# celliern/triflow

Measured on AMD Instinct MI355X. Metric: implicit time-steps/s, 1e6-node 3-var system (member-steps/s over all GPUs), higher is better.
Workload: dtype f64; 1 GPU; BASELINE config 3: M3_film, N=1000000 nodes, periodic, fixed dt=0.001, ROS2; members_per_gpu=1, parallelism=ensemble members sharded by rank, no data-path collective

## Files before the change

### include/triflow_hip.h

```cpp
#ifndef TRIFLOW_HIP_H
#define TRIFLOW_HIP_H

#include <stddef.h>
#include <stdint.h>

#ifdef __cplusplus
extern "C" {
#endif

typedef struct tf_model tf_model;
typedef struct tf_solver tf_solver;

typedef struct tf_model_spec {
    int32_t nvar;
    int32_t nh;
    int32_t npar;
    int32_t mp;
    int32_t nnz;
    int32_t seg;
    int32_t sweep_block;
    int32_t uses_x;
    uint32_t parvec_mask;
} tf_model_spec;

typedef struct tf_solver_opts {
    int32_t m1;
    int32_t m_upper;
    int32_t nstate;
    int32_t refine;
    int32_t device;
    int32_t berr_every;
    int32_t reserved;
} tf_solver_opts;

const char* tf_last_error(void);
int tf_runtime_info(int32_t* is_device_build, int32_t* device_count);
int tf_set_device(int32_t ordinal);

int tf_model_create(const tf_model_spec* spec, const void* code_object, size_t code_size,
                    tf_model** out);
int tf_model_add_alternate(tf_model* model, const void* code_object, size_t code_size,
                           uint64_t kernel_mask);
void tf_model_destroy(tf_model* model);

int tf_solver_create(tf_model* model, int64_t N, int32_t nsys, int32_t periodic,
                     const tf_solver_opts* opts, tf_solver** out);
void tf_solver_destroy(tf_solver* solver);
int tf_solver_describe(tf_solver* solver, int32_t* nlevels, int32_t* chunks ,
                       int32_t max_levels, int64_t* device_bytes);

int tf_set_state(tf_solver*, int32_t slot, int32_t first_var, int32_t nvars, const double* host);
int tf_get_state(tf_solver*, int32_t slot, int32_t first_var, int32_t nvars, double* host);
int tf_set_state_flat(tf_solver*, int32_t slot, const double* uflat );
int tf_get_state_flat(tf_solver*, int32_t slot, double* uflat);
int tf_copy_state(tf_solver*, int32_t src_slot, int32_t dst_slot);
int tf_set_helpers(tf_solver*, int32_t first, int32_t count, const double* host);
int tf_set_param_scalar(tf_solver*, int32_t k, const double* values );
int tf_set_param_vector(tf_solver*, int32_t k, const double* host );
int tf_set_dx(tf_solver*, const double* dx );
int tf_set_x(tf_solver*, const double* x );
int tf_set_dirichlet(tf_solver*, int32_t n, const int32_t* var, const int64_t* node,
                     const double* value);

int tf_set_dirichlet_values(tf_solver*, const double* before, const double* after);
int tf_poke(tf_solver*, int32_t slot, int32_t n, const int32_t* var, const int64_t* node,
            const double* value);
int tf_peek(tf_solver*, int32_t slot, int32_t n, const int32_t* var, const int64_t* node,
            double* out);

int tf_eval(tf_solver*, int32_t slot, int32_t with_j);
int tf_eval_repeat(tf_solver*, int32_t slot, int32_t with_j, int32_t reps, double* total_ms);
int tf_get_F(tf_solver*, double* F );
int tf_get_J(tf_solver*, double* Jvals );

int tf_set_csc_map(tf_solver*, const int32_t* map, int64_t n);
int tf_get_J_mapped(tf_solver*, double* out );

int tf_set_constant_jacobian(tf_solver*, int32_t on);

int tf_factor(tf_solver*, double c);
int tf_solve(tf_solver*, const double* rhs_flat , double* x_flat);
int tf_matvec(tf_solver*, const double* v_flat, double* y_flat);

int tf_step_theta(tf_solver*, int32_t src, int32_t dst, double dt, double theta);
int tf_step_row(tf_solver*, int32_t src, int32_t dst, double dt, int32_t s,
                const double* alpha, const double* gamma, const double* b,
                const double* b_pred, int32_t hook_after, double* err_out);
int tf_step_bdf2(tf_solver*, int32_t src, int32_t dst, double dt);
int tf_bdf2_reset(tf_solver*);
int tf_step_bdf2_owned(tf_solver*, int32_t src, int32_t dst, double dt, int64_t owner,
                       int32_t continuing);
int tf_bdf2_release(tf_solver*, int64_t owner);
int tf_step_bdf2_from(tf_solver*, int32_t src, int32_t dst, int32_t prev, double dt);
int tf_step_row_queued(tf_solver*, int32_t src, int32_t dst, double dt, int32_t stages,
                       const double* alpha, const double* gamma, const double* b,
                       const double* b_pred, int32_t hook_after, int32_t err_slot);
int tf_read_err(tf_solver*, int32_t err_slot, double* err_out);
enum { TF_SCHEME_THETA = 0, TF_SCHEME_ROW = 1 };
typedef struct tf_scheme {
    int32_t kind;
    int32_t stages;
    double theta;
    const double* alpha;
    const double* gamma;
    const double* b;
    int32_t hook_after;
    int32_t reserved;
} tf_scheme;
int tf_step_doubling(tf_solver*, int32_t src, int32_t dst, int32_t tmp, int32_t coarse, double dt,
                     int32_t m, int32_t nfine, const tf_scheme* scheme, int32_t ord, double* err_out);
int tf_diff_norm(tf_solver*, int32_t slot_a, int32_t slot_b, int32_t ord, double* out);

int tf_backward_error(tf_solver*, double* omega, int32_t* refined);

int tf_monitor_error(tf_solver*, double* worst);
int tf_solver_counters(tf_solver*, int64_t* factorisations, int64_t* checks, int64_t* replans);
int tf_solver_kernel_block(tf_solver*, int32_t kernel, int32_t* block);
int tf_sync(tf_solver*);

int tf_timing_enable(tf_solver*, int64_t mask);
int tf_timing_reset(tf_solver*);
int tf_timing_get(tf_solver*, int32_t kernel, double* total_ms, int64_t* launches);
int tf_debug_stamps(tf_solver*, uint64_t* out, int32_t max_levels);
int tf_kernel_count(void);
const char* tf_kernel_name(int32_t kernel);

typedef struct tf_probe tf_probe;
int tf_probe_create(tf_solver*, const void* code_object, size_t code_size, int32_t nprobe,
                    const int32_t* kinds, int32_t nconst, int32_t capacity, tf_probe** out);
void tf_probe_destroy(tf_probe* probe);
int tf_probe_set_consts(tf_probe*, const double* values , int32_t nconst);
int tf_probe_set_x(tf_probe*, const double* x );
int tf_probe_record(tf_probe*, int32_t slot);
int tf_probe_fetch(tf_probe*, double* out, int64_t max_rows, int64_t* rows);
int tf_probe_pending(tf_probe*, int64_t* rows);

typedef struct tf_record tf_record;
int tf_record_create(tf_solver*, const void* code_object, size_t code_size, int32_t nrec,
                     const int32_t* geometry, int32_t nconst, tf_record** out);
void tf_record_destroy(tf_record* record);
int tf_record_set_consts(tf_record*, const double* values , int32_t nconst);
int tf_record_set_x(tf_record*, const double* x );
int tf_record_record(tf_record*, int32_t which, int32_t slot);
int tf_record_fetch(tf_record*, int32_t which, double* out, int64_t max_rows, int64_t* rows);
int tf_record_pending(tf_record*, int32_t which, int64_t* rows);

#ifdef __cplusplus
}
#endif
#endif
```

### triflow_amd/_capi.py

```python

import ctypes as C
import os

import numpy as np

c_double_p = C.POINTER(C.c_double)
c_int32_p = C.POINTER(C.c_int32)
c_int64_p = C.POINTER(C.c_int64)


class ModelSpec(C.Structure):
    _fields_ = [("nvar", C.c_int32), ("nh", C.c_int32), ("npar", C.c_int32),
                ("mp", C.c_int32), ("nnz", C.c_int32), ("seg", C.c_int32),
                ("sweep_block", C.c_int32), ("uses_x", C.c_int32),
                ("parvec_mask", C.c_uint32)]


class SolverOpts(C.Structure):
    _fields_ = [("m1", C.c_int32), ("m_upper", C.c_int32), ("nstate", C.c_int32),
                ("refine", C.c_int32), ("device", C.c_int32), ("berr_every", C.c_int32),
                ("reserved", C.c_int32)]


class Scheme(C.Structure):
    _fields_ = [("kind", C.c_int32), ("stages", C.c_int32), ("theta", C.c_double),
                ("alpha", c_double_p), ("gamma", c_double_p), ("b", c_double_p),
                ("hook_after", C.c_int32), ("reserved", C.c_int32)]


SIGNATURES = {
    "tf_last_error": (C.c_char_p, []),
    "tf_runtime_info": (C.c_int, [c_int32_p, c_int32_p]),
    "tf_set_device": (C.c_int, [C.c_int32]),
    "tf_model_create": (C.c_int, [C.POINTER(ModelSpec), C.c_void_p, C.c_size_t,
                                  C.POINTER(C.c_void_p)]),
    "tf_model_add_alternate": (C.c_int, [C.c_void_p, C.c_void_p, C.c_size_t, C.c_uint64]),
    "tf_model_destroy": (None, [C.c_void_p]),
    "tf_solver_create": (C.c_int, [C.c_void_p, C.c_int64, C.c_int32, C.c_int32,
                                   C.POINTER(SolverOpts), C.POINTER(C.c_void_p)]),
    "tf_solver_destroy": (None, [C.c_void_p]),
    "tf_solver_describe": (C.c_int, [C.c_void_p, c_int32_p, c_int32_p, C.c_int32, c_int64_p]),
    "tf_set_state": (C.c_int, [C.c_void_p, C.c_int32, C.c_int32, C.c_int32, c_double_p]),
    "tf_get_state": (C.c_int, [C.c_void_p, C.c_int32, C.c_int32, C.c_int32, c_double_p]),
    "tf_set_state_flat": (C.c_int, [C.c_void_p, C.c_int32, c_double_p]),
    "tf_get_state_flat": (C.c_int, [C.c_void_p, C.c_int32, c_double_p]),
    "tf_copy_state": (C.c_int, [C.c_void_p, C.c_int32, C.c_int32]),
    "tf_set_helpers": (C.c_int, [C.c_void_p, C.c_int32, C.c_int32, c_double_p]),
    "tf_set_param_scalar": (C.c_int, [C.c_void_p, C.c_int32, c_double_p]),
    "tf_set_param_vector": (C.c_int, [C.c_void_p, C.c_int32, c_double_p]),
    "tf_set_dx": (C.c_int, [C.c_void_p, c_double_p]),
    "tf_set_x": (C.c_int, [C.c_void_p, c_double_p]),
    "tf_set_dirichlet": (C.c_int, [C.c_void_p, C.c_int32, c_int32_p, c_int64_p, c_double_p]),
    "tf_set_dirichlet_values": (C.c_int, [C.c_void_p, c_double_p, c_double_p]),
    "tf_poke": (C.c_int, [C.c_void_p, C.c_int32, C.c_int32, c_int32_p, c_int64_p, c_double_p]),
    "tf_peek": (C.c_int, [C.c_void_p, C.c_int32, C.c_int32, c_int32_p, c_int64_p, c_double_p]),
    "tf_eval": (C.c_int, [C.c_void_p, C.c_int32, C.c_int32]),
    "tf_eval_repeat": (C.c_int, [C.c_void_p, C.c_int32, C.c_int32, C.c_int32, c_double_p]),
    "tf_get_F": (C.c_int, [C.c_void_p, c_double_p]),
    "tf_get_J": (C.c_int, [C.c_void_p, c_double_p]),
    "tf_set_csc_map": (C.c_int, [C.c_void_p, c_int32_p, C.c_int64]),
    "tf_set_constant_jacobian": (C.c_int, [C.c_void_p, C.c_int32]),
    "tf_get_J_mapped": (C.c_int, [C.c_void_p, c_double_p]),
    "tf_factor": (C.c_int, [C.c_void_p, C.c_double]),
    "tf_solve": (C.c_int, [C.c_void_p, c_double_p, c_double_p]),
    "tf_matvec": (C.c_int, [C.c_void_p, c_double_p, c_double_p]),
    "tf_step_theta": (C.c_int, [C.c_void_p, C.c_int32, C.c_int32, C.c_double, C.c_double]),
    "tf_step_row": (C.c_int, [C.c_void_p, C.c_int32, C.c_int32, C.c_double, C.c_int32,
                              c_double_p, c_double_p, c_double_p, c_double_p, C.c_int32,
                              c_double_p]),
    "tf_step_row_queued": (C.c_int, [C.c_void_p, C.c_int32, C.c_int32, C.c_double, C.c_int32,
                                     c_double_p, c_double_p, c_double_p, c_double_p, C.c_int32, C.c_int32]),
    "tf_read_err": (C.c_int, [C.c_void_p, C.c_int32, c_double_p]),
    "tf_step_bdf2": (C.c_int, [C.c_void_p, C.c_int32, C.c_int32, C.c_double]),
    "tf_bdf2_reset": (C.c_int, [C.c_void_p]),
    "tf_step_bdf2_from": (C.c_int, [C.c_void_p, C.c_int32, C.c_int32, C.c_int32, C.c_double]),
    "tf_step_bdf2_owned": (C.c_int, [C.c_void_p, C.c_int32, C.c_int32, C.c_double, C.c_int64,
                                     C.c_int32]),
    "tf_bdf2_release": (C.c_int, [C.c_void_p, C.c_int64]),
    "tf_diff_norm": (C.c_int, [C.c_void_p, C.c_int32, C.c_int32, C.c_int32, c_double_p]),
    "tf_step_doubling": (C.c_int, [C.c_void_p, C.c_int32, C.c_int32, C.c_int32, C.c_int32, C.c_double,
                                   C.c_int32, C.c_int32, C.POINTER(Scheme), C.c_int32, c_double_p]),
    "tf_backward_error": (C.c_int, [C.c_void_p, c_double_p, c_int32_p]),
    "tf_monitor_error": (C.c_int, [C.c_void_p, c_double_p]),
    "tf_solver_counters": (C.c_int, [C.c_void_p, c_int64_p, c_int64_p, c_int64_p]),
    "tf_sync": (C.c_int, [C.c_void_p]),
    "tf_timing_enable": (C.c_int, [C.c_void_p, C.c_int64]),
    "tf_timing_reset": (C.c_int, [C.c_void_p]),
    "tf_timing_get": (C.c_int, [C.c_void_p, C.c_int32, c_double_p, c_int64_p]),
    "tf_debug_stamps": (C.c_int, [C.c_void_p, C.POINTER(C.c_uint64), C.c_int32]),
    "tf_solver_kernel_block": (C.c_int, [C.c_void_p, C.c_int32, C.POINTER(C.c_int32)]),
    "tf_kernel_count": (C.c_int, []),
    "tf_kernel_name": (C.c_char_p, [C.c_int32]),
    "tf_probe_create": (C.c_int, [C.c_void_p, C.c_void_p, C.c_size_t, C.c_int32, c_int32_p, C.c_int32,
                                  C.c_int32, C.POINTER(C.c_void_p)]),
    "tf_probe_destroy": (None, [C.c_void_p]),
    "tf_probe_set_consts": (C.c_int, [C.c_void_p, c_double_p, C.c_int32]),
    "tf_probe_set_x": (C.c_int, [C.c_void_p, c_double_p]),
    "tf_probe_record": (C.c_int, [C.c_void_p, C.c_int32]),
    "tf_probe_fetch": (C.c_int, [C.c_void_p, c_double_p, C.c_int64, c_int64_p]),
    "tf_probe_pending": (C.c_int, [C.c_void_p, c_int64_p]),
    "tf_record_create": (C.c_int, [C.c_void_p, C.c_void_p, C.c_size_t, C.c_int32, c_int32_p, C.c_int32,
                                   C.POINTER(C.c_void_p)]),
    "tf_record_destroy": (None, [C.c_void_p]),
    "tf_record_set_consts": (C.c_int, [C.c_void_p, c_double_p, C.c_int32]),
    "tf_record_set_x": (C.c_int, [C.c_void_p, c_double_p]),
    "tf_record_record": (C.c_int, [C.c_void_p, C.c_int32, C.c_int32]),
    "tf_record_fetch": (C.c_int, [C.c_void_p, C.c_int32, c_double_p, C.c_int64, c_int64_p]),
    "tf_record_pending": (C.c_int, [C.c_void_p, C.c_int32, c_int64_p]),
}


def _dptr(arr):
    return arr.ctypes.data_as(c_double_p)


def _f64(a, shape=None):
    out = np.ascontiguousarray(a, dtype=np.float64)
    if shape is not None and out.shape != tuple(shape):
        raise ValueError("expected array of shape %r, got %r" % (tuple(shape), out.shape))
    return out


class Library:

    def __init__(self, path):
        if not os.path.exists(path):
            raise RuntimeError(
                "HIP runtime library %s is missing -- build it with "
                "`python -c 'import __graft_entry__ as g; g.build()'` "
                "(there is no CPU fallback)" % path)
        self.path = path
        self.dll = C.CDLL(path)
        for name, (restype, argtypes) in SIGNATURES.items():
            fn = getattr(self.dll, name)
            fn.restype = restype
            fn.argtypes = argtypes

    def call(self, name, *args):
        rc = getattr(self.dll, name)(*args)
        if rc != 0:
            raise RuntimeError("%s: %s" % (name, self.dll.tf_last_error().decode()))

    def runtime_info(self):
        dev, cnt = C.c_int32(0), C.c_int32(0)
        self.call("tf_runtime_info", C.byref(dev), C.byref(cnt))
        return bool(dev.value), cnt.value

    def set_device(self, ordinal):
        self.call("tf_set_device", int(ordinal))

    def kernel_names(self):
        return [self.dll.tf_kernel_name(k).decode() for k in range(self.dll.tf_kernel_count())]


class DeviceModel:

    def __init__(self, lib, spec, code, alt_code=None, alt_kernels=()):
        self.lib = lib
        self.spec = dict(spec)
        cs = ModelSpec(spec["nvar"], spec["nh"], spec["npar"], spec["mp"], spec["nnz"],
                       spec["seg"], spec["sweep_block"], spec["uses_x"], spec["parvec_mask"])
        self._code = C.create_string_buffer(code, len(code)) if code else None
        handle = C.c_void_p()
        lib.call("tf_model_create", C.byref(cs),
                 C.cast(self._code, C.c_void_p) if self._code is not None else None,
                 len(code) if code else 0, C.byref(handle))
        self.handle = handle
        self._alt = None
        if alt_code and alt_kernels:
            names = lib.kernel_names()
            mask = 0
            for k in alt_kernels:
                mask |= 1 << names.index(k)
            self._alt = C.create_string_buffer(alt_code, len(alt_code))
            lib.call("tf_model_add_alternate", handle, C.cast(self._alt, C.c_void_p), len(alt_code), mask)

    def close(self):
        if self.handle:
            self.lib.dll.tf_model_destroy(self.handle)
            self.handle = None

    def __del__(self):
        try:
            self.close()
        except Exception:
            pass


class DeviceSolver:

    def __init__(self, model, N, nsys=1, periodic=False, m1=0, m_upper=0, nstate=0,
                 refine=-1, device=-1, berr_every=0):
        self.model = model
        self.lib = model.lib
        self.N, self.nsys, self.periodic = int(N), int(nsys), bool(periodic)
        self.nvar, self.nh = model.spec["nvar"], model.spec["nh"]
        self.npar, self.nnz = model.spec["npar"], model.spec["nnz"]
        m1 = m1 or int(os.environ.get("TRIFLOW_M1", "0"))
        m_upper = m_upper or int(os.environ.get("TRIFLOW_M_UPPER", "0"))
        opts = SolverOpts(m1, m_upper, nstate, refine, device, berr_every, 0)
        handle = C.c_void_p()
        self.lib.call("tf_solver_create", model.handle, self.N, self.nsys,
                      int(self.periodic), C.byref(opts), C.byref(handle))
        self.handle = handle
        self.nstate = nstate if nstate > 0 else 3
        ju = model.spec.get("j_uniform") or []
        self.constant_jacobian = bool(ju) and all(ju) and os.environ.get("TRIFLOW_REUSE_FACTOR", "1") != "0"
        if self.constant_jacobian:
            self.lib.call("tf_set_constant_jacobian", self.handle, 1)

    def close(self):
        if self.handle:
            self.lib.dll.tf_solver_destroy(self.handle)
            self.handle = None

    def __del__(self):
        try:
            self.close()
        except Exception:
            pass

    def describe(self):
        nl, nbytes = C.c_int32(0), C.c_int64(0)
        chunks = (C.c_int32 * 32)()
        self.lib.call("tf_solver_describe", self.handle, C.byref(nl), chunks, 32, C.byref(nbytes))
        return dict(levels=nl.value, chunks=list(chunks[:nl.value]), device_bytes=nbytes.value)

    def set_state(self, slot, arrays, first=0):
        a = _f64(arrays).reshape(-1, self.nsys, self.N)
        self.lib.call("tf_set_state", self.handle, slot, first, a.shape[0], _dptr(a))

    def get_state(self, slot, first=0, nvars=None):
        nvars = self.nvar - first if nvars is None else nvars
        out = np.empty((nvars, self.nsys, self.N))
        self.lib.call("tf_get_state", self.handle, slot, first, nvars, _dptr(out))
        return out

    def set_state_flat(self, slot, uflat):
        a = _f64(uflat).reshape(self.nsys, self.N * self.nvar)
        self.lib.call("tf_set_state_flat", self.handle, slot, _dptr(a))

    def get_state_flat(self, slot):
        out = np.empty((self.nsys, self.N * self.nvar))
        self.lib.call("tf_get_state_flat", self.handle, slot, _dptr(out))
        return out

    def copy_state(self, src, dst):
        self.lib.call("tf_copy_state", self.handle, src, dst)

    def set_helpers(self, arrays, first=0):
        a = _f64(arrays).reshape(-1, self.nsys, self.N)
        self.lib.call("tf_set_helpers", self.handle, first, a.shape[0], _dptr(a))

    def set_param(self, k, value):
        if (self.model.spec["parvec_mask"] >> k) & 1:
            a = _f64(np.broadcast_to(np.asarray(value, dtype=float), (self.nsys, self.N)))
            self.lib.call("tf_set_param_vector", self.handle, k, _dptr(a))
        else:
            a = _f64(np.broadcast_to(np.asarray(value, dtype=float), (self.nsys,)))
            self.lib.call("tf_set_param_scalar", self.handle, k, _dptr(a))

    def set_dx(self, dx):
        a = _f64(np.broadcast_to(np.asarray(dx, dtype=float), (self.nsys,)))
        self.lib.call("tf_set_dx", self.handle, _dptr(a))

    def set_x(self, x):
        a = _f64(np.broadcast_to(np.asarray(x, dtype=float), (self.nsys, self.N)))
        self.lib.call("tf_set_x", self.handle, _dptr(a))

    def set_dirichlet(self, entries):
        entries = list(entries)
        n = len(entries)
        var = np.array([e[0] for e in entries], dtype=np.int32)
        node = np.array([e[1] for e in entries], dtype=np.int64)
        val = np.array([e[2] for e in entries], dtype=np.float64)
        self.lib.call("tf_set_dirichlet", self.handle, n,
                      var.ctypes.data_as(c_int32_p), node.ctypes.data_as(c_int64_p), _dptr(val))

    def poke(self, slot, entries):
        entries = list(entries)
        if not entries:
            return
        var = np.array([e[0] for e in entries], dtype=np.int32)
        node = np.array([e[1] for e in entries], dtype=np.int64)
        val = np.array([e[2] for e in entries], dtype=np.float64)
        self.lib.call("tf_poke", self.handle, slot, len(entries),
                      var.ctypes.data_as(c_int32_p), node.ctypes.data_as(c_int64_p), _dptr(val))

    def peek(self, slot, var, node):
        v = np.array([var], dtype=np.int32)
        n = np.array([node], dtype=np.int64)
        out = np.empty((1, self.nsys))
        self.lib.call("tf_peek", self.handle, slot, 1, v.ctypes.data_as(c_int32_p),
                      n.ctypes.data_as(c_int64_p), _dptr(out))
        return out[0]

    def set_dirichlet_values(self, before=None, after=None):
        b = _f64(before) if before is not None else None
        a = _f64(after) if after is not None else None
        self.lib.call("tf_set_dirichlet_values", self.handle,
                      _dptr(b) if b is not None else None, _dptr(a) if a is not None else None)

    def eval(self, slot=0, with_j=False):
        self.lib.call("tf_eval", self.handle, slot, int(with_j))

    def eval_repeat(self, slot=0, with_j=True, reps=20):
        ms = C.c_double(0.0)
        self.lib.call("tf_eval_repeat", self.handle, slot, int(with_j), reps, C.byref(ms))
        return ms.value / reps

    def get_F(self):
        out = np.empty((self.nsys, self.N * self.nvar))
        self.lib.call("tf_get_F", self.handle, _dptr(out))
        return out

    def get_J(self):
        out = np.empty((self.nsys, self.N, max(self.nnz, 1)))
        self.lib.call("tf_get_J", self.handle, _dptr(out))
        return out[:, :, :self.nnz]

    def set_csc_map(self, index_list):
        m = np.ascontiguousarray(index_list, dtype=np.int32)
        self.lib.call("tf_set_csc_map", self.handle, m.ctypes.data_as(c_int32_p), m.size)
        self._csc_n = m.size

    def get_J_mapped(self):
        out = np.empty(self._csc_n)
        self.lib.call("tf_get_J_mapped", self.handle, _dptr(out))
        return out

    def factor(self, c):
        self.lib.call("tf_factor", self.handle, float(c))

    def solve(self, rhs_flat):
        rhs = _f64(rhs_flat).reshape(self.nsys, self.N * self.nvar)
        out = np.empty_like(rhs)
        self.lib.call("tf_solve", self.handle, _dptr(rhs), _dptr(out))
        return out

    def matvec(self, v_flat):
        v = _f64(v_flat).reshape(self.nsys, self.N * self.nvar)
        out = np.empty_like(v)
        self.lib.call("tf_matvec", self.handle, _dptr(v), _dptr(out))
        return out

    def step_theta(self, src, dst, dt, theta=1.0):
        self.lib.call("tf_step_theta", self.handle, src, dst, float(dt), float(theta))

    def step_row(self, src, dst, dt, alpha, gamma, b, b_pred=None, hook_after=False,
                 want_err=True):
        alpha, gamma = _f64(alpha), _f64(gamma)
        b = _f64(b)
        s = b.size
        bp = _f64(b_pred) if b_pred is not None else None
        err = C.c_double(0.0)
        self.lib.call("tf_step_row", self.handle, src, dst, float(dt), s, _dptr(alpha),
                      _dptr(gamma), _dptr(b), _dptr(bp) if bp is not None else None,
                      int(hook_after), C.byref(err) if want_err else None)
        return np.float64(err.value) if (want_err and bp is not None) else None

    def step_row_queued(self, src, dst, dt, alpha, gamma, b, b_pred, hook_after=False, err_slot=1):
        alpha, gamma, b, bp = _f64(alpha), _f64(gamma), _f64(b), _f64(b_pred)
        self.lib.call("tf_step_row_queued", self.handle, src, dst, float(dt), b.size, _dptr(alpha),
                      _dptr(gamma), _dptr(b), _dptr(bp), int(hook_after), int(err_slot))

    def read_err(self, err_slot):
        err = C.c_double(0.0)
        self.lib.call("tf_read_err", self.handle, int(err_slot), C.byref(err))
        return np.float64(err.value)

    def step_bdf2(self, src, dst, dt, owner=0, continuing=True):
        if owner:
            self.lib.call("tf_step_bdf2_owned", self.handle, src, dst, float(dt), int(owner),
                          int(bool(continuing)))
        else:
            self.lib.call("tf_step_bdf2", self.handle, src, dst, float(dt))

    def step_bdf2_from(self, src, dst, prev, dt):
        self.lib.call("tf_step_bdf2_from", self.handle, src, dst, int(prev), float(dt))

    def bdf2_release(self, owner):
        if self.handle:
            self.lib.call("tf_bdf2_release", self.handle, int(owner))

    def bdf2_reset(self):
        self.lib.call("tf_bdf2_reset", self.handle)

    def step_doubling(self, src, dst, tmp, coarse, dt, m, desc, ord=2, nfine=10):
        keep = []
        if desc["kind"] == "theta":
            sch = Scheme(0, 0, float(desc["theta"]), None, None, None, 0, 0)
        else:
            arrs = [_f64(desc[k]) for k in ("alpha", "gamma", "b")]
            keep.extend(arrs)
            sch = Scheme(1, arrs[2].size, 0.0, _dptr(arrs[0]), _dptr(arrs[1]), _dptr(arrs[2]),
                         int(bool(desc.get("hook_after", True))), 0)
        err = np.empty(self.nsys)
        self.lib.call("tf_step_doubling", self.handle, src, dst, tmp, coarse, float(dt), int(m),
                      int(nfine), C.byref(sch), 0 if ord in (0, np.inf, "inf") else int(ord), _dptr(err))
        return err

    def diff_norms(self, slot_a, slot_b, ord=2):
        out = np.empty((self.nsys, self.nvar))
        self.lib.call("tf_diff_norm", self.handle, slot_a, slot_b,
                      0 if ord in (0, np.inf, "inf") else int(ord), _dptr(out))
        return out

    def backward_error(self):
        om, flag = C.c_double(0.0), C.c_int32(0)
        self.lib.call("tf_backward_error", self.handle, C.byref(om), C.byref(flag))
        return om.value, bool(flag.value)

    def counters(self):
        f, c, r = C.c_int64(0), C.c_int64(0), C.c_int64(0)
        self.lib.call("tf_solver_counters", self.handle, C.byref(f), C.byref(c), C.byref(r))
        return dict(factorisations=f.value, checks=c.value, replans=r.value)

    def kernel_block(self, name):
        b = C.c_int32(0)
        self.lib.call("tf_solver_kernel_block", self.handle, self.lib.kernel_names().index(name), C.byref(b))
        return b.value

    def monitor_error(self):
        w = C.c_double(0.0)
        self.lib.call("tf_monitor_error", self.handle, C.byref(w))
        return w.value

    def sync(self):
        self.lib.call("tf_sync", self.handle)
        if not getattr(self, "_warned_replan", False) and self.counters()["replans"]:
            import warnings
            self._warned_replan = True
            warnings.warn("banded solver: the default partition lost accuracy on this matrix and the "
                          "factorisations go through the rescue plan (8 x longer chunks, every solve "
                          "checked): several times slower; see DESIGN.md section 4.5", RuntimeWarning,
                          stacklevel=2)

    def debug_stamps(self, levels=8):
        out = np.zeros((levels, 64), dtype=np.uint64)
        self.lib.call("tf_debug_stamps", self.handle, out.ctypes.data_as(C.POINTER(C.c_uint64)), levels)
        return out

    def timing(self, on=True, kernels=None):
        if kernels is not None:
            names = self.lib.kernel_names()
            mask = 0
            for k in kernels:
                mask |= 1 << names.index(k)
        else:
            mask = -1 if on else 0
        self.lib.call("tf_timing_enable", self.handle, mask)

    def timing_reset(self):
        self.lib.call("tf_timing_reset", self.handle)

    def timing_report(self):
        out = {}
        for k, name in enumerate(self.lib.kernel_names()):
            ms, n = C.c_double(0.0), C.c_int64(0)
            self.lib.call("tf_timing_get", self.handle, k, C.byref(ms), C.byref(n))
            if n.value:
                out[name] = (ms.value, n.value)
        return out


class DeviceProbe:

    def __init__(self, solver, code, kinds, nconst, capacity=1024):
        self.solver, self.lib = solver, solver.lib
        self.nprobe, self.nconst, self.capacity = len(kinds), int(nconst), int(capacity)
        self._code = C.create_string_buffer(code, len(code))
        k = np.ascontiguousarray(kinds, dtype=np.int32)
        handle = C.c_void_p()
        self.lib.call("tf_probe_create", solver.handle, C.cast(self._code, C.c_void_p), len(code),
                      self.nprobe, k.ctypes.data_as(c_int32_p), self.nconst, self.capacity, C.byref(handle))
        self.handle = handle

    def close(self):
        if self.handle:
            self.lib.dll.tf_probe_destroy(self.handle)
            self.handle = None

    def __del__(self):
        try:
            self.close()
        except Exception:
            pass

    def _check_open(self):
        if not self.solver.handle:
            raise RuntimeError("the solver of this probe set was closed (rows not fetched before are lost)")

    def set_consts(self, values):
        self._check_open()
        v = _f64(values).reshape(self.solver.nsys, self.nconst)
        self.lib.call("tf_probe_set_consts", self.handle, _dptr(v) if v.size else None, self.nconst)

    def set_x(self, x):
        self._check_open()
        a = _f64(np.broadcast_to(np.asarray(x, dtype=float), (self.solver.nsys, self.solver.N)))
        self.lib.call("tf_probe_set_x", self.handle, _dptr(a))

    def record(self, slot):
        self._check_open()
        self.lib.call("tf_probe_record", self.handle, int(slot))

    def pending(self):
        self._check_open()
        n = C.c_int64(0)
        self.lib.call("tf_probe_pending", self.handle, C.byref(n))
        return n.value

    def fetch(self):
        n = self.pending()
        out = np.empty((n, self.solver.nsys, self.nprobe))
        got = C.c_int64(0)
        self.lib.call("tf_probe_fetch", self.handle, _dptr(out), n, C.byref(got))
        return out[:got.value]


class DeviceRecord:

    def __init__(self, solver, code, geometry, nconst):
        self.solver, self.lib = solver, solver.lib
        self.nconst = int(nconst)
        g = np.ascontiguousarray(geometry, dtype=np.int32).reshape(-1, 6)
        self.ncols = [-(-(int(r[3]) - int(r[2])) // int(r[4])) for r in g]
        self._code = C.create_string_buffer(code, len(code))
        handle = C.c_void_p()
# ... 46 lines not shown
```

### triflow_amd/csrc/tf_args.h

```cpp
#pragma once
#include <stdint.h>

#define TF_MAX_FIELDS 16
#define TF_MAX_PARS 16
#define TF_MAX_TERMS 8

struct TfLayout {
    int nsys;
    int N;
    int P;
    int mbase;
    int rem;
    int M;
    int Ptot;
    int periodic;
    int64_t plane;
};

struct TfSweepArgs {
    TfLayout L;
    const double* fields;
    const double* helpers;
    const double* parvec;
    const double* parsca;
    const double* dx;
    const double* xcoord;
    double* F;
    double* Jv;
    int with_j;
    int nterms;
    const double* kx[TF_MAX_TERMS];
    double kc[TF_MAX_TERMS];
    double fscale;
    double* theta_rhs;
    double theta, theta_dt;
    double* bdf_rhs;
    const double* bdf_prev;
    double* bdf_prev_out;
    double bdf_c0, bdf_c1;
    int bdf_two_step;
    double* stage_rhs;
    double gc[TF_MAX_TERMS];
    double cF, cA;
};

struct TfSpmvArgs {
    TfLayout L;
    const double* parsca;
    const double* dx;
    const double* Jv;
    const double* v;
    double* y;
    double scale;
    int absval;
    int nterms;
    const double* vx[TF_MAX_TERMS];
    double vc[TF_MAX_TERMS];
    const double* addF;
    double cF, cA;
};

struct TfNormArgs {
    TfLayout L;
    const double* a;
    const double* b;
    double* partial;
    int nblocks;
    int ord;
    const int* status;
    const double* mon;
};

struct TfBerrArgs {
    TfLayout L;
    const double* parsca;
    const double* dx;
    const double* Jv;
    const double* x;
    const double* rhs;
    double c;
    double* red;
    int one_node;
    int reserved_;
    const double* xbase;
};

struct TfStageMonArgs { TfSweepArgs s; TfBerrArgs b; };

struct TfVecArgs {
    int64_t n;
    int nterms;
    int op;
    double* out;
    const double* base;
    const double* x[TF_MAX_TERMS];
    double c[TF_MAX_TERMS];
    double* red;
    double c2[TF_MAX_TERMS];
};

struct TfPermArgs {
    TfLayout L;
    const double* src;
    double* dst;
    int ncomp;
    int mode;
};

struct TfGatherArgs {
    TfLayout L;
    const double* Jv;
    const int* map;
    double* out;
    int64_t n;
    int nnz;
};

struct TfDirichletArgs {
    TfLayout L;
    double* fields;
    int n;
    const int* var;
    const int* node;
    const double* value;
};

#define TF_POKE_MAX 8
struct TfPokeArgs {
    TfLayout L;
    double* fields;
    int n;
    int var[TF_POKE_MAX];
    int node[TF_POKE_MAX];
    double value[TF_POKE_MAX];
};

struct TfLevelArgs {
    TfLayout L;
    const double* Jv;
    const double* parsca;
    const double* dx;
    double c;
    const double* Ablk;
    const double* rhs;
    double* x;
    double* Ut;
    double* Et;
    double* yt;
    double* Dinv;
    double* Unup;
    double* tips_dn;
    double* tips_up;
    TfLayout Lnext;
    double* Anext;
    double* rhsnext;
    const double* xnext;
    int* status;
    int lu_cols;
    int next_aos;
    int cr_rhs;
    double* crf;
    double* zt;
    unsigned* perm;
    int fold_top;
    int respike;
    int twist;
    int ylds_rows;
    int fuse_asm;
    double* upd_out;
    const double* upd_base;
    const double* upd_k0;
    double upd_c0, upd_c1;
    int upd_n;
    double* topAinv;
    double* topx;
    unsigned long long* stamps;
};

struct TfTinyArgs {
    TfLayout L;
    const double* Jv;
    const double* parsca;
    const double* dx;
    double c;
    double* lu;
    int* piv;
    const double* rhs;
    double* x;
    int* status;
};

struct TfTailArgs {
    TfLevelArgs lv[2];
};

struct TfScalarArgs {
    TfLevelArgs lv[3];
    unsigned* counter;
};

struct TfTopArgs {
    int nsys;
    const double* A;
    const double* rhs;
    double* Ainv;
    double* x;
    int* status;
    int aos;
};

#define TF_RESPIKE_MODEL(mp, nvar) ((mp) * (nvar) * (nvar) >= 8)
#define TF_RESPIKE_MIN_NODES 750000
#define TF_TWIST_MAX_CHUNKS 65536

#ifndef TF_L1_SPLIT_LDS
#define TF_L1_SPLIT_LDS (40 * 1024)
#endif
#define TF_L1_SPLIT_MODEL(mp, nvar) ((nvar) >= 2 && 2 * (1 + (mp)) * (nvar) * (nvar) * 64 * 8 <= TF_L1_SPLIT_LDS)

#define TF_STAGE_SEG 8

#define TF_CR_MAXLEN 16
#define TF_CRS_MAXLEN 256
#define TF_CRS_TOPLEN(b) ((b) == 1 ? 512 : 256)

#define TF_PROBE_SUM 0
#define TF_PROBE_MEAN 1
#define TF_PROBE_INTEGRAL 2
#define TF_PROBE_MAX 3
#define TF_PROBE_MIN 4
#define TF_PROBE_ARGMAX 5
#define TF_PROBE_ARGMIN 6
#define TF_PROBE_KINDS 7
#define TF_PROBE_SEG 8
struct TfProbeArgs {
    TfLayout L;
    const double* fields;
    const double* helpers;
    const double* parvec;
    const double* parsca;
    const double* dx;
    const double* xcoord;
    const double* hc;
    double* partial;
    double* ends;
    int nblk;
    int nseg;
    int capacity;
    int* cursor;
    double* ring;
};

#define TF_REC_SAMPLE 0
#define TF_REC_MAX 1
#define TF_REC_MIN 2
#define TF_REC_MEAN 3
#define TF_REC_BLOCK 256
struct TfRecordArgs {
    TfLayout L;
    const double* fields;
    const double* helpers;
    const double* parvec;
    const double* parsca;
    const double* dx;
    const double* xcoord;
    const double* hc;
    int which;
    int pool;
    int start, stop, step;
    int ncols;
    int split;
    int part;
    int nblk;
    int capacity;
    int* cursor;
    double* ring;
};

enum TfKernel {
    TFK_SWEEP_F = 0, TFK_SWEEP_FJ, TFK_SPMV, TFK_VEC, TFK_VEC_MAXABS, TFK_PERM, TFK_DIRICHLET,
    TFK_L1_FACTOR, TFK_L1_SOLVE, TFK_L1_ASM_MAT, TFK_L1_ASM_RHS, TFK_L1_BACKSUB,
    TFK_BT_LU, TFK_BT_SPIKE, TFK_BT_RHS, TFK_BT_ASM_MAT, TFK_BT_ASM_RHS, TFK_BT_BACKSUB,
    TFK_TOP_FACTOR, TFK_TOP_SOLVE, TFK_BERR, TFK_DIFFNORM, TFK_L1_FACTOR_RHS, TFK_SWEEP_F_STAGE,
    TFK_CR_FACTOR, TFK_CR_FWD, TFK_CR_BWD, TFK_POKE, TFK_SWEEP_FJ_THETA, TFK_SWEEP_FJ_BDF2, TFK_GATHER,
    TFK_SWEEP_F_STAGE_RHS, TFK_L1_FWD2, TFK_L1_BACKSUB_U, TFK_CR_TAIL, TFK_L1_FWD2_BACKSUB, TFK_TINY_FACTOR, TFK_TINY_SOLVE,
    TFK_S_FWD, TFK_S_BWD, TFK_SWEEP_F_STAGE_RHS_N, TFK_L1_SOLVE_CR, TFK_L1_FWD2_BACKSUB_CR, TFK_SWEEP_F_STAGE_RHS_MON,
    TFK_PROBE_PARTIAL, TFK_PROBE_FINAL,
    TFK_RECORD, TFK_COUNT
};
#define TF_KERNEL_NAMES { \
    "tfk_sweep_f", "tfk_sweep_fj", "tfk_spmv", "tfk_vec", "tfk_vec_maxabs", "tfk_perm", "tfk_dirichlet", \
    "tfk_l1_factor", "tfk_l1_solve", "tfk_l1_asm_mat", "tfk_l1_asm_rhs", "tfk_l1_backsub", \
    "tfk_bt_lu", "tfk_bt_spike", "tfk_bt_rhs", "tfk_bt_asm_mat", "tfk_bt_asm_rhs", "tfk_bt_backsub", \
    "tfk_top_factor", "tfk_top_solve", "tfk_berr", "tfk_diffnorm", "tfk_l1_factor_rhs", "tfk_sweep_f_stage", \
    "tfk_cr_factor", "tfk_cr_fwd", "tfk_cr_bwd", "tfk_poke", "tfk_sweep_fj_theta", "tfk_sweep_fj_bdf2", \
    "tfk_gather", "tfk_sweep_f_stage_rhs", "tfk_l1_fwd2", "tfk_l1_backsub_u", "tfk_cr_tail", \
    "tfk_l1_fwd2_backsub", "tfk_tiny_factor", "tfk_tiny_solve", "tfk_s_fwd", "tfk_s_bwd", "tfk_sweep_f_stage_rhs_n", \
    "tfk_l1_solve_cr", "tfk_l1_fwd2_backsub_cr", "tfk_sweep_f_stage_rhs_mon", \
    "tfk_probe_partial", "tfk_probe_final" }
#define TF_KERNEL_NAMES_RECORD { "tfk_record" }
static inline const char* tf_kernel_entry(int kernel) {
    static const char* const base[] = TF_KERNEL_NAMES;
    static const char* const rec[] = TF_KERNEL_NAMES_RECORD;
    static_assert(sizeof(base) / sizeof(base[0]) == TFK_RECORD, "TF_KERNEL_NAMES and TfKernel differ");
    static_assert(sizeof(rec) / sizeof(rec[0]) == TFK_COUNT - TFK_RECORD, "TF_KERNEL_NAMES_RECORD and TfKernel differ");
    if (kernel < 0 || kernel >= TFK_COUNT) return "";
    return kernel < TFK_RECORD ? base[kernel] : rec[kernel - TFK_RECORD];
}
```

### triflow_amd/csrc/tf_backend_hip.cpp

```cpp
#include "tf_backend.h"
#include "tf_args.h"

#include <hip/hip_runtime.h>
#include <hip/hip_ext.h>

#include <algorithm>
#include <cstdio>
#include <cstdlib>
#include <cstring>
#include <map>
#include <thread>
#include <stdexcept>
#include <string>

namespace tfb {

static void check(hipError_t err, const char* what) {
    if (err != hipSuccess)
        throw std::runtime_error(std::string("HIP error in ") + what + ": " + hipGetErrorString(err));
}
#define TF_HIP(call) check((call), #call)

struct Module { hipModule_t mod; hipFunction_t fn[TFK_COUNT]; hipModule_t alt = nullptr; };
struct Stream { hipStream_t s; };
struct Event { hipEvent_t e; };

bool is_device_build() { return true; }
int coop_group(int b) { return b <= 2 ? 1 : (b <= 8 ? 8 : (b <= 16 ? 16 : 1)); }

bool cyclic_reduction(int b) {
    const char* mode = getenv("TRIFLOW_REDUCED");
    if (mode && std::string(mode) == "walk") return false;
    return b >= 1 && b <= 8;
}

int device_count() {
    int n = 0;
    if (hipGetDeviceCount(&n) != hipSuccess) return 0;
    return n;
}

void set_device(int ordinal) { TF_HIP(hipSetDevice(ordinal)); }

void* dev_alloc(size_t bytes) {
    void* p = nullptr;
    if (bytes == 0) bytes = 8;
    TF_HIP(hipMalloc(&p, bytes));
    TF_HIP(hipMemset(p, 0, bytes));
    TF_HIP(hipDeviceSynchronize());
    return p;
}
void dev_free(void* p) { if (p) (void)hipFree(p); }
void memset0(void* p, size_t bytes, Stream* s) { TF_HIP(hipMemsetAsync(p, 0, bytes, s->s)); }
namespace {
constexpr size_t kStageChunk = 8u << 20;
constexpr size_t kStageMin = 4u << 20;
struct Bounce {
    void* buf[2] = {nullptr, nullptr};
    hipEvent_t ev[2];
    bool ok = false;
    Bounce() {
        if (hipHostMalloc(&buf[0], kStageChunk, hipHostMallocDefault) != hipSuccess) return;
        if (hipHostMalloc(&buf[1], kStageChunk, hipHostMallocDefault) != hipSuccess) return;
        if (hipEventCreateWithFlags(&ev[0], hipEventDisableTiming) != hipSuccess) return;
        if (hipEventCreateWithFlags(&ev[1], hipEventDisableTiming) != hipSuccess) return;
        ok = true;
    }
};
struct BounceSet {
    std::map<int, Bounce*> by_device;
    ~BounceSet() {
        for (auto& kv : by_device) {
            Bounce* b = kv.second;
            if (b->ok) { (void)hipEventDestroy(b->ev[0]); (void)hipEventDestroy(b->ev[1]); }
            if (b->buf[0]) (void)hipHostFree(b->buf[0]);
            if (b->buf[1]) (void)hipHostFree(b->buf[1]);
            delete b;
        }
    }
};
Bounce& bounce() {
    static thread_local BounceSet set;
    int dev = 0;
    (void)hipGetDevice(&dev);
    Bounce*& b = set.by_device[dev];
    if (!b) b = new Bounce();
    return *b;
}
void parallel_copy(void* dst, const void* src, size_t n) {
    constexpr int NT = 4;
    if (n < (1u << 20)) { std::memcpy(dst, src, n); return; }
    std::thread th[NT - 1];
    const size_t part = (n / NT + 63) & ~(size_t)63;
    for (int t = 1; t < NT; ++t) {
        const size_t lo = std::min(n, part * t), hi = std::min(n, part * (t + 1));
        th[t - 1] = std::thread([=] { if (hi > lo) std::memcpy((char*)dst + lo, (const char*)src + lo, hi - lo); });
    }
    std::memcpy(dst, src, std::min(n, part));
    for (int t = 1; t < NT; ++t) th[t - 1].join();
}
}
void h2d(void* dst, const void* src, size_t bytes, Stream* s) {
    Bounce& b = bounce();
    if (bytes < kStageMin || !b.ok) {
        TF_HIP(hipMemcpyAsync(dst, src, bytes, hipMemcpyHostToDevice, s->s));
        TF_HIP(hipStreamSynchronize(s->s));
        return;
    }
    size_t off = 0;
    for (int k = 0; off < bytes; ++k) {
        const int i = k & 1;
        const size_t n = std::min(kStageChunk, bytes - off);
        if (k >= 2) TF_HIP(hipEventSynchronize(b.ev[i]));
        parallel_copy(b.buf[i], (const char*)src + off, n);
        TF_HIP(hipMemcpyAsync((char*)dst + off, b.buf[i], n, hipMemcpyHostToDevice, s->s));
        TF_HIP(hipEventRecord(b.ev[i], s->s));
        off += n;
    }
    TF_HIP(hipStreamSynchronize(s->s));
}
void d2h(void* dst, const void* src, size_t bytes, Stream* s) {
    Bounce& b = bounce();
    if (bytes < kStageMin || !b.ok) {
        TF_HIP(hipMemcpyAsync(dst, src, bytes, hipMemcpyDeviceToHost, s->s));
        TF_HIP(hipStreamSynchronize(s->s));
        return;
    }
    size_t off = 0, done = 0;
    int k = 0;
    for (; off < bytes; ++k) {
        const int i = k & 1;
        const size_t n = std::min(kStageChunk, bytes - off);
        if (k >= 2) {
            TF_HIP(hipEventSynchronize(b.ev[i]));
            const size_t m = std::min(kStageChunk, bytes - done);
            parallel_copy((char*)dst + done, b.buf[i], m);
            done += m;
        }
        TF_HIP(hipMemcpyAsync(b.buf[i], (const char*)src + off, n, hipMemcpyDeviceToHost, s->s));
        TF_HIP(hipEventRecord(b.ev[i], s->s));
        off += n;
    }
    for (int j = (k >= 2 ? k - 2 : 0); j < k; ++j) {
        const int i = j & 1;
        TF_HIP(hipEventSynchronize(b.ev[i]));
        const size_t m = std::min(kStageChunk, bytes - done);
        parallel_copy((char*)dst + done, b.buf[i], m);
        done += m;
    }
}
void d2d(void* dst, const void* src, size_t bytes, Stream* s) {
    TF_HIP(hipMemcpyAsync(dst, src, bytes, hipMemcpyDeviceToDevice, s->s));
}

Module* module_load(const void* image, size_t) {
    Module* m = new Module();
    hipError_t err = hipModuleLoadData(&m->mod, image);
    if (err != hipSuccess) {
        delete m;
        check(err, "hipModuleLoadData (is the code object built for this GPU, gfx950?)");
    }
    for (int k = 0; k < TFK_COUNT; ++k) {
        err = hipModuleGetFunction(&m->fn[k], m->mod, tf_kernel_entry(k));
        if (err != hipSuccess) {
            (void)hipModuleUnload(m->mod);
            delete m;
            throw std::runtime_error(std::string("kernel missing from code object: ") + tf_kernel_entry(k));
        }
    }
    if (const char* alt = getenv("TF_ALT_HSACO")) {
        const char* mask_s = getenv("TF_ALT_MASK");
        unsigned long mask = mask_s ? strtoul(mask_s, nullptr, 0) : 0;
        FILE* f = fopen(alt, "rb");
        if (f && mask) {
            fseek(f, 0, SEEK_END); long n = ftell(f); fseek(f, 0, SEEK_SET);
            std::string img(n, '\0');
            if (fread(&img[0], 1, n, f) == (size_t)n) {
                hipModule_t am;
                if (hipModuleLoadData(&am, img.data()) == hipSuccess)
                    for (int k = 0; k < TFK_COUNT; ++k)
                        if ((mask >> k) & 1ul) (void)hipModuleGetFunction(&m->fn[k], am, tf_kernel_entry(k));
            }
        }
        if (f) fclose(f);
    }
    return m;
}
void module_add_alternate(Module* m, const void* image, size_t, uint64_t mask) {
    if (!m || !mask) return;
    if (m->alt) throw std::runtime_error("module_add_alternate: one alternate build per model");
    check(hipModuleLoadData(&m->alt, image), "hipModuleLoadData (alternate build)");
    for (int k = 0; k < TFK_COUNT; ++k)
        if ((mask >> k) & 1ull) {
            if (hipModuleGetFunction(&m->fn[k], m->alt, tf_kernel_entry(k)) != hipSuccess)
                throw std::runtime_error(std::string("kernel missing from the alternate code object: ") + tf_kernel_entry(k));
        }
}
void module_unload(Module* m) {
    if (!m) return;
    if (m->alt) (void)hipModuleUnload(m->alt);
    (void)hipModuleUnload(m->mod);
    delete m;
}

Stream* stream_create() {
    Stream* s = new Stream();
    TF_HIP(hipStreamCreateWithFlags(&s->s, hipStreamNonBlocking));
    return s;
}
void stream_destroy(Stream* s) { if (s) { (void)hipStreamDestroy(s->s); delete s; } }
void stream_sync(Stream* s) { TF_HIP(hipStreamSynchronize(s->s)); }

unsigned kernel_block(Module* m, int kernel) {
    int v = 0;
    TF_HIP(hipFuncGetAttribute(&v, HIP_FUNC_ATTRIBUTE_MAX_THREADS_PER_BLOCK, m->fn[kernel]));
    return (unsigned)v;
}

void launch(Module* m, int kernel, unsigned gx, unsigned gy, unsigned block,
            const void* args, size_t arg_bytes, Stream* s, unsigned lds_bytes) {
    size_t size = arg_bytes;
    void* config[] = {HIP_LAUNCH_PARAM_BUFFER_POINTER, const_cast<void*>(args),
                      HIP_LAUNCH_PARAM_BUFFER_SIZE, &size, HIP_LAUNCH_PARAM_END};
    TF_HIP(hipModuleLaunchKernel(m->fn[kernel], gx, gy, 1, block, 1, 1, lds_bytes, s->s, nullptr, config));
}

void launch_timed(Module* m, int kernel, unsigned gx, unsigned gy, unsigned block,
                  const void* args, size_t arg_bytes, Stream* s, Event* start, Event* stop,
                  unsigned lds_bytes) {
    size_t size = arg_bytes;
    void* config[] = {HIP_LAUNCH_PARAM_BUFFER_POINTER, const_cast<void*>(args),
                      HIP_LAUNCH_PARAM_BUFFER_SIZE, &size, HIP_LAUNCH_PARAM_END};
    TF_HIP(hipExtModuleLaunchKernel(m->fn[kernel], gx * block, gy, 1, block, 1, 1, lds_bytes, s->s,
                                    nullptr, config, start->e, stop->e, 0));
}

struct Graph { hipGraph_t graph; hipGraphExec_t exec; };
bool graphs_supported() { return true; }
void capture_begin(Stream* s) { TF_HIP(hipStreamBeginCapture(s->s, hipStreamCaptureModeThreadLocal)); }
Graph* capture_end(Stream* s) {
    hipGraph_t graph = nullptr;
    TF_HIP(hipStreamEndCapture(s->s, &graph));
    hipGraphExec_t exec = nullptr;
    hipError_t err = hipGraphInstantiate(&exec, graph, nullptr, nullptr, 0);
    if (err != hipSuccess) { (void)hipGraphDestroy(graph); check(err, "hipGraphInstantiate"); }
    return new Graph{graph, exec};
}
void capture_abort(Stream* s) {
    hipGraph_t graph = nullptr;
    (void)hipStreamEndCapture(s->s, &graph);
    if (graph) (void)hipGraphDestroy(graph);
}
void graph_launch(Graph* g, Stream* s) { TF_HIP(hipGraphLaunch(g->exec, s->s)); }
void graph_destroy(Graph* g) {
    if (!g) return;
    (void)hipGraphExecDestroy(g->exec);
    (void)hipGraphDestroy(g->graph);
    delete g;
}

struct Mailbox { char* host = nullptr; hipEvent_t ev; };
Mailbox* mailbox_create() {
    Mailbox* m = new Mailbox();
    TF_HIP(hipHostMalloc((void**)&m->host, 64, hipHostMallocDefault));
    std::memset(m->host, 0, 64);
    TF_HIP(hipEventCreateWithFlags(&m->ev, hipEventDisableTiming));
    return m;
}
void mailbox_destroy(Mailbox* m) {
    if (!m) return;
    (void)hipEventDestroy(m->ev);
    (void)hipHostFree(m->host);
    delete m;
}
void mailbox_post(Mailbox* m, int at, const void* dev_src, size_t bytes, Stream* s) {
    TF_HIP(hipMemcpyAsync(m->host + at, dev_src, bytes, hipMemcpyDeviceToHost, s->s));
}
void mailbox_mark(Mailbox* m, Stream* s) { TF_HIP(hipEventRecord(m->ev, s->s)); }
void mailbox_wait(Mailbox* m, void* dst, size_t bytes) {
    TF_HIP(hipEventSynchronize(m->ev));
    std::memcpy(dst, m->host, bytes);
}

Event* event_create() {
    Event* e = new Event();
    TF_HIP(hipEventCreate(&e->e));
    return e;
}
void event_destroy(Event* e) { if (e) { (void)hipEventDestroy(e->e); delete e; } }
void event_record(Event* e, Stream* s) { TF_HIP(hipEventRecord(e->e, s->s)); }
float event_elapsed_ms(Event* a, Event* b) {
    float ms = 0.f;
    TF_HIP(hipEventElapsedTime(&ms, a->e, b->e));
    return ms;
}

void* host_alloc(size_t bytes) {
    void* p = nullptr;
    TF_HIP(hipHostMalloc(&p, bytes ? bytes : 8, hipHostMallocDefault));
    return p;
}
void host_free(void* p) { if (p) (void)hipHostFree(p); }
void d2h_async(void* dst, const void* src, size_t bytes, Stream* s) {
    TF_HIP(hipMemcpyAsync(dst, src, bytes, hipMemcpyDeviceToHost, s->s));
}
void stream_wait_event(Stream* s, Event* e) { TF_HIP(hipStreamWaitEvent(s->s, e->e, 0)); }
void event_sync(Event* e) { TF_HIP(hipEventSynchronize(e->e)); }

}
```

### triflow_amd/csrc/tf_coop_hip.h

```cpp
#pragma once
#include "tf_crs.h"

template <int BB> struct TfCoop {
    static constexpr int G = BB <= 2 ? 1 : (BB <= 8 ? 8 : (BB <= 16 ? 16 : 1));
    static constexpr int NGRP = G > 1 ? 64 / G : 64;
};

template <int BB>
__device__ __forceinline__ void tfk_bt_lu_coop(const TfLevelArgs& a, int dir) {
    typedef TfTips<BB, 1> Tip;
    constexpr int G = TfCoop<BB>::G, NGRP = TfCoop<BB>::NGRP;
    const TfLayout& L = a.L;
    const int grp = threadIdx.x / G, g = threadIdx.x % G;
    const int pg = blockIdx.x * NGRP + grp;
    const bool lane_on = pg < L.Ptot && g < BB;
    const int e = lane_on ? pg / L.P : 0, p = lane_on ? pg - e * L.P : 0;
    const int len = tf_len(L, p), mI = len - 1, start = tf_start(L, p);
    const int di = dir > 0 ? 0 : 1;
    const int behind = dir > 0 ? 0 : 2, ahead = dir > 0 ? 2 : 0;

    __shared__ double sUn[NGRP][BB][BB];
    __shared__ double sAh[NGRP][BB][BB];
    __shared__ double sAll[2][NGRP][G][2 * BB + 1];
    __shared__ double sE[NGRP][BB][BB + 1];
// ... 322 lines not shown
            double sub = 0.0, dia = 0.0, sup = 0.0;
#pragma unroll
            for (int k = 0; k < BB; ++k) {
                sub = tf_fma(-H[k], tdn(Tip::V(0, 0, k, c)), sub);
                dia = tf_fma(-H[k], tdn(Tip::W(0, 0, k, c)), dia);
            }
            dia += D[c];
            if (has_next) {
#pragma unroll
                for (int k = 0; k < BB; ++k) {
                    dia = tf_fma(-K[k], tup(Tip::V(0, 0, k, c)), dia);
                    sup = tf_fma(-K[k], tup(Tip::W(0, 0, k, c)), sup);
                }
            }
            a.Anext[tf_next_A(a, e, p, s2, 0, g, c, BB)] = sub;
            a.Anext[tf_next_A(a, e, p, s2, 1, g, c, BB)] = dia;
            a.Anext[tf_next_A(a, e, p, s2, 2, g, c, BB)] = sup;
        }
    }
}

template <int BB> struct TfCr {
    static constexpr int MAXLEN = TF_CR_MAXLEN;
    static constexpr int NPOS = MAXLEN + 1;
    static constexpr int G = 8, NGRP = 8;
};

template <int BB, int G>
__device__ __forceinline__ int tf_gj_coop(double (&S)[BB], double (&INV)[BB], bool on, int g,
                                          double* xch, bool& ok) {
    constexpr int RS = 2 * BB + 1;
    int myk = -1;
#pragma unroll
    for (int c = 0; c < BB; ++c) INV[c] = c == g ? 1.0 : 0.0;
    auto publish = [&](int kk) {
        double* dst = xch + ((kk & 1) * G + g) * RS;
#pragma unroll
        for (int c = 0; c < BB; ++c) { dst[c] = S[c]; dst[BB + c] = INV[c]; }
        dst[2 * BB] = (on && myk < 0) ? tf_abs(S[kk]) : -1.0;
    };
    publish(0);
    __syncthreads();
#pragma unroll
    for (int kk = 0; kk < BB; ++kk) {
        const double* buf = xch + (kk & 1) * G * RS;
        int piv = 0;
        double best = -2.0;
#pragma unroll
        for (int r = 0; r < BB; ++r) {
            const double v = buf[r * RS + 2 * BB];
            if (v > best) { best = v; piv = r; }
        }
        const double* prow = buf + piv * RS;
        const double pv = prow[kk];
        if (on) ok = ok && (pv != 0.0) && tf_finite(pv);
        const double rp = 1.0 / pv;
        const bool mine = g == piv;
        if (mine) myk = kk;
        const double f2 = mine ? 0.0 : -S[kk] * rp;
#pragma unroll
        for (int c = 0; c < BB; ++c) {
            S[c] = tf_fma(f2, prow[c], S[c]);
            INV[c] = tf_fma(f2, prow[BB + c], INV[c]);
        }
        if (mine) {
#pragma unroll
            for (int c = 0; c < BB; ++c) { S[c] *= rp; INV[c] *= rp; }
        }
        if (kk + 1 < BB) publish(kk + 1);
        __syncthreads();
    }
    return myk;
}


template <int BB>
__device__ __forceinline__ void tf_load_row(const double* p, double (&dst)[BB]) {
    if constexpr (BB % 2 == 0) {
        const double2* q = reinterpret_cast<const double2*>(__builtin_assume_aligned(p, 16));
#pragma unroll
        for (int m = 0; m < BB / 2; ++m) {
            const double2 v = q[m];
            dst[2 * m] = v.x;
            dst[2 * m + 1] = v.y;
        }
    } else {
#pragma unroll
        for (int m = 0; m < BB; ++m) dst[m] = p[m];
    }
}

__device__ __forceinline__ void tf_wave_sync() {
    __builtin_amdgcn_fence(__ATOMIC_RELEASE, "wavefront");
    __builtin_amdgcn_wave_barrier();
    __builtin_amdgcn_fence(__ATOMIC_ACQUIRE, "wavefront");
}
template <int BB> struct TfCrSolveLds {
    static constexpr int NPOS = TF_CR_MAXLEN + 1;
    double sYr[NPOS * 2 * BB], sY[NPOS][BB], sZ[NPOS][BB];
};

template <int BB> struct TfCrIo {
    const double* ys;
    const double* crf0;
    double* next_own;
    double* next_prev;
    double* xmirror;
    bool has_mirror;
    const double* xn_own;
    const double* xn_prev;
    bool has_xprev;
    __device__ __forceinline__ TfCrIo(const TfLevelArgs& a, const TfCrChunk<BB>& ch) {
        ys = a.rhs + (ch.nbase + ch.start) * 2 * BB;
        crf0 = a.crf + (ch.nbase + ch.start) * 5 * BB * BB;
        next_own = a.rhsnext ? a.rhsnext + ((int64_t)ch.e * a.Lnext.N + ch.p) * 2 * BB : nullptr;
        next_prev = a.rhsnext ? a.rhsnext + ((int64_t)ch.e * a.Lnext.N + ch.pprev) * 2 * BB + BB : nullptr;
        xmirror = nullptr; has_mirror = false;
        xn_own = a.xnext ? a.xnext + ((int64_t)ch.e * a.Lnext.N + ch.p) * BB : nullptr;
        xn_prev = a.xnext ? a.xnext + ((int64_t)ch.e * a.Lnext.N + ch.pprev) * BB : nullptr;
        has_xprev = ch.has_prev;
    }
};

template <int BB> struct TfCrFwdRows { double Di[4][BB], Lb[4][BB], Ua[4][BB]; };
template <int BB>
__device__ __forceinline__ void tfk_cr_fwd_load(const TfCrChunk<BB>& ch, int tid, const TfCrIo<BB>& io, TfCrFwdRows<BB>& rows) {
    constexpr int G = TfCr<BB>::G, B2 = BB * BB, MAXR = 4;
    const int grp = tid / G, g = tid % G;
    const bool row_on = g < BB;
    const int mI = ch.mI;
#pragma unroll
    for (int r = 0; r < MAXR; ++r) {
        const int s = 1 << r;
        const int nA = ((mI >> r) + 1) >> 1, nB = mI >> (r + 1), nq = mI >> r;
        const bool onA = s <= mI && grp < nA && row_on;
        const bool onB = s <= mI && grp <= nB && row_on;
        const bool ends = grp == nB;
        const int aa = 2 * s * (grp + 1);
        const bool vL = onB && (ends ? (nq & 1) != 0 : true);
        const bool vR = onB && (ends ? true : aa + s <= mI);
        const int k = s * (2 * grp + 1), kL = ends ? nq * s : aa - s, kR = ends ? s : aa + s;
        const double* rk = io.crf0 + ((onA ? k : 1) - 1) * 5 * B2 + g * BB;
        const double* rl = io.crf0 + ((vL ? kL : 1) - 1) * 5 * B2 + 4 * B2 + g * BB;
        const double* rr = io.crf0 + ((vR ? kR : 1) - 1) * 5 * B2 + 3 * B2 + g * BB;
        tf_load_row<BB>(rk, rows.Di[r]);
        tf_load_row<BB>(rl, rows.Lb[r]);
        tf_load_row<BB>(rr, rows.Ua[r]);
    }
}
#define TF_CR_NYS(b) ((TF_CR_MAXLEN * 2 * (b) + 63) / 64)
template <int BB>
__device__ __forceinline__ void tfk_cr_fwd_load_ys(const TfCrChunk<BB>& ch, int tid, const TfCrIo<BB>& io, double (&ysv)[TF_CR_NYS(BB)]) {
#pragma unroll
    for (int q = 0; q < TF_CR_NYS(BB); ++q) ysv[q] = tid + 64 * q < ch.len * 2 * BB ? io.ys[tid + 64 * q] : 0.0;
}

template <int BB, bool KEEPZ = false, bool PRE = false>
__device__ __forceinline__ void tfk_cr_fwd_chunk(const TfLevelArgs& a, const TfCrChunk<BB>& ch, int tid,
                                                 TfCrSolveLds<BB>& sh, const TfCrIo<BB>& io,
                                                 double* zkeep = nullptr, const TfCrFwdRows<BB>* pre = nullptr,
                                                 const double* ysv = nullptr) {
    typedef TfCr<BB> C;
    constexpr int G = C::G, B2 = BB * BB, MAXR = 4;
    static_assert(C::MAXLEN <= 16, "round count");
    const TfLayout& L = a.L;
    const int grp = tid / G, g = tid % G;
    const bool row_on = g < BB;
    const int mI = ch.mI, pe = ch.pe, len = ch.len;
    double (&sY)[TfCrSolveLds<BB>::NPOS][BB] = sh.sY;
    double (&sZ)[TfCrSolveLds<BB>::NPOS][BB] = sh.sZ;
    double* sYr = sh.sYr;

    double* const zt0 = a.zt + (ch.nbase + ch.start - 1) * BB + (row_on ? g : 0);
    tf_wave_sync();
    TfCrFwdRows<BB> own;
    if constexpr (PRE) {
#pragma unroll
        for (int q = 0; q < TF_CR_NYS(BB); ++q)
            if (tid + 64 * q < len * 2 * BB) sYr[2 * BB + tid + 64 * q] = ysv[q];
    } else {
        for (int i = tid; i < len * 2 * BB; i += 64) sYr[2 * BB + i] = io.ys[i];
        tfk_cr_fwd_load<BB>(ch, tid, io, own);
    }
    const TfCrFwdRows<BB>& rw = PRE ? *pre : own;
    const double (&Di)[4][BB] = rw.Di;
    const double (&Lb)[4][BB] = rw.Lb;
    const double (&Ua)[4][BB] = rw.Ua;
    tf_wave_sync();
    if (PRE && (ch.p & 3) == 0) TF_STAMP(a, 42);
    for (int i = tid; i < (len + 1) * BB; i += 64) {
        const int pos = i / BB, r = i - pos * BB;
        sY[pos][r] = pos > 0 ? sYr[pos * 2 * BB + r] + sYr[pos * 2 * BB + BB + r] : 0.0;
    }
    tf_wave_sync();
#pragma unroll
    for (int r = 0; r < MAXR; ++r) {
        const int s = 1 << r;
        if (s <= mI) {
            const int nA = ((mI >> r) + 1) >> 1, nB = mI >> (r + 1), nq = mI >> r;
            if (grp < nA && row_on) {
                const int k = s * (2 * grp + 1);
                double z = 0.0;
#pragma unroll
                for (int m = 0; m < BB; ++m) z = tf_fma(Di[r][m], sY[k][m], z);
                sZ[k][g] = z;
                zt0[k * BB] = z;
                if (KEEPZ) zkeep[r] = z;
            }
            tf_wave_sync();
            if (grp <= nB && row_on) {
                const bool ends = grp == nB;
                const int aa = 2 * s * (grp + 1);
                const int aL = ends ? pe : aa, aU = ends ? 0 : aa;
                const bool vL = ends ? (nq & 1) != 0 : true;
                const bool vR = ends ? true : aa + s <= mI;
                const int kL = vL ? (ends ? nq * s : aa - s) : 1, kR = vR ? (ends ? s : aa + s) : 1;
                double yl = 0.0, yu = 0.0;
#pragma unroll
                for (int m = 0; m < BB; ++m) {
                    yl = tf_fma(-Lb[r][m], sZ[kL][m], yl);
                    yu = tf_fma(-Ua[r][m], sZ[kR][m], yu);
                }
                if (vL) sY[aL][g] += yl;
                if (vR) sY[aU][g] += yu;
            }
            tf_wave_sync();
        }
    }
    if (PRE && (ch.p & 3) == 0) TF_STAMP(a, 43);
    if (a.fold_top) {
        double x = 0.0;
        if (row_on && grp == 0) {
            const int nsys = L.Ptot;
#pragma unroll
            for (int c = 0; c < BB; ++c)
                x = tf_fma(a.topAinv[(int64_t)(g * BB + c) * nsys + ch.e], sY[pe][c] + sY[0][c], x);
        }
        tf_wave_sync();
        if (row_on && grp == 0) {
            a.topx[(int64_t)ch.e * BB + g] = x;
            a.x[(ch.nbase + ch.node(pe)) * BB + g] = x;
            if (io.has_mirror) io.xmirror[(pe - 1) * BB + g] = x;
            sY[pe][g] = x;
            sY[0][g] = ch.has_prev ? x : 0.0;
        }
        tf_wave_sync();
#pragma unroll
        for (int r = MAXR - 1; r >= 0; --r) {
            const int s = 1 << r;
            if (s <= mI) {
                const int nA = ((mI >> r) + 1) >> 1;
                if (grp < nA && row_on) {
                    const int k = s * (2 * grp + 1);
                    const int kl = k - s, kr = k + s <= mI ? k + s : pe;
                    const double* rec = io.crf0 + (k - 1) * 5 * B2 + g * BB;
                    double xk = sZ[k][g];
#pragma unroll
                    for (int m = 0; m < BB; ++m) {
                        xk = tf_fma(-rec[1 * B2 + m], sY[kl][m], xk);
                        xk = tf_fma(-rec[2 * B2 + m], sY[kr][m], xk);
                    }
                    sY[k][g] = xk;
                    a.x[(ch.nbase + ch.node(k)) * BB + g] = xk;
                    if (io.has_mirror) io.xmirror[(k - 1) * BB + g] = xk;
                }
                tf_wave_sync();
            }
        }
    } else if (row_on && grp < 2) {
        if (grp == 0) io.next_own[g] = sY[pe][g]; else io.next_prev[g] = sY[0][g];
    }
}

template <int BB> struct TfCrBwdRows { double Er[4][BB], Fr[4][BB], zk[4]; };

template <int BB>
__device__ __forceinline__ void tfk_cr_bwd_load(const TfLevelArgs& a, const TfCrChunk<BB>& ch, int tid,
                                                const TfCrIo<BB>& io, TfCrBwdRows<BB>& rows, bool load_z) {
    constexpr int G = TfCr<BB>::G, B2 = BB * BB, MAXR = 4;
    const int grp = tid / G, g = tid % G;
    const bool row_on = g < BB;
    const int mI = ch.mI;
#pragma unroll
    for (int r = 0; r < MAXR; ++r) {
        const int s = 1 << r;
        const int nA = ((mI >> r) + 1) >> 1;
        const bool on = s <= mI && grp < nA && row_on;
        const int k = on ? s * (2 * grp + 1) : 1;
        const double* rec = io.crf0 + (k - 1) * 5 * B2 + g * BB;
        tf_load_row<BB>(rec + 1 * B2, rows.Er[r]);
        tf_load_row<BB>(rec + 2 * B2, rows.Fr[r]);
        if (load_z) rows.zk[r] = a.zt[(ch.nbase + ch.node(k)) * BB + (row_on ? g : 0)];
    }
}

template <int BB>
__device__ __forceinline__ double tfk_cr_bwd_sep(int tid, const TfCrIo<BB>& io) {
    constexpr int G = TfCr<BB>::G;
    const int grp = tid / G, g = tid % G;
    if (g < BB && grp == 0) return io.xn_own[g];
    if (g < BB && grp == 1 && io.has_xprev) return io.xn_prev[g];
    return 0.0;
}
template <int BB, bool USE_EF = false, bool PREX = false>
__device__ __forceinline__ void tfk_cr_bwd_run(const TfLevelArgs& a, const TfCrChunk<BB>& ch, int tid,
                                               TfCrSolveLds<BB>& sh, const TfCrIo<BB>& io,
                                               const TfCrBwdRows<BB>& rows, const double* ef = nullptr, double xsep = 0.0) {
    constexpr int G = TfCr<BB>::G, MAXR = 4, B2 = BB * BB;
    const int grp = tid / G, g = tid % G;
    const bool row_on = g < BB;
    const int mI = ch.mI, pe = ch.pe;
    double (&sX)[TfCrSolveLds<BB>::NPOS][BB] = sh.sY;
    double* const x0 = a.x + (ch.nbase + ch.start - 1) * BB + (row_on ? g : 0);
    tf_wave_sync();
    if (row_on && grp == 0) {
        const double xs = PREX ? xsep : io.xn_own[g];
        sX[pe][g] = xs;
        x0[pe * BB] = xs;
    }
    if (row_on && grp == 1) sX[0][g] = PREX ? xsep : (io.has_xprev ? io.xn_prev[g] : 0.0);
    tf_wave_sync();
#pragma unroll
    for (int r = MAXR - 1; r >= 0; --r) {
        const int s = 1 << r;
        if (s <= mI) {
            const int nA = ((mI >> r) + 1) >> 1;
            if (grp < nA && row_on) {
                const int k = s * (2 * grp + 1);
                const int kl = k - s, kr = k + s <= mI ? k + s : pe;
                double xk = rows.zk[r];
                if (USE_EF) {
                    const double* er = ef + (k - 1) * 2 * B2 + g * BB;
#pragma unroll
                    for (int m = 0; m < BB; ++m) {
                        xk = tf_fma(-er[m], sX[kl][m], xk);
                        xk = tf_fma(-er[B2 + m], sX[kr][m], xk);
                    }
                } else {
#pragma unroll
                    for (int m = 0; m < BB; ++m) {
                        xk = tf_fma(-rows.Er[r][m], sX[kl][m], xk);
                        xk = tf_fma(-rows.Fr[r][m], sX[kr][m], xk);
                    }
                }
                sX[k][g] = xk;
                x0[k * BB] = xk;
            }
            tf_wave_sync();
        }
    }
}

template <int BB>
__device__ __forceinline__ void tfk_cr_fwd_coop(const TfLevelArgs& a) {
    __shared__ TfCrSolveLds<BB> sh;
    const TfCrChunk<BB> ch(a.L, (int)blockIdx.x);
    tfk_cr_fwd_chunk<BB>(a, ch, (int)threadIdx.x, sh, TfCrIo<BB>(a, ch));
}
template <int BB>
__device__ __forceinline__ void tfk_cr_bwd_coop(const TfLevelArgs& a) {
    __shared__ TfCrSolveLds<BB> sh;
    const TfCrChunk<BB> ch(a.L, (int)blockIdx.x);
    const TfCrIo<BB> io(a, ch);
    TfCrBwdRows<BB> rows;
    tfk_cr_bwd_load<BB>(a, ch, (int)threadIdx.x, io, rows, true);
    tfk_cr_bwd_run<BB>(a, ch, (int)threadIdx.x, sh, io, rows);
}

#define TF_CR_TAIL_WAVES 8
#define TF_CR_TAIL_MAXB 6
template <int BB>
__device__ __forceinline__ void tfk_cr_tail_coop(const TfTailArgs& t) {
    constexpr int B2 = BB * BB, NW = TF_CR_TAIL_WAVES, MAXLEN = TF_CR_MAXLEN;
    __shared__ TfCrSolveLds<BB> sh[NW];
    __shared__ double sEF[NW][MAXLEN * 2 * B2];
    __shared__ double sCrfTop[NW * 5 * B2];
    __shared__ double sRhsTop[NW * 2 * BB];
    __shared__ double sXTop[NW * BB];
    const int w = __builtin_amdgcn_readfirstlane((int)threadIdx.x >> 6), lane = (int)threadIdx.x & 63, e = (int)blockIdx.x;
    const TfLevelArgs& la = t.lv[0];
    const TfLevelArgs& lb = t.lv[1];
    const int P = la.L.P;
    const TfCrChunk<BB> chb(lb.L, e);
    const TfCrChunk<BB> ch(la.L, e * P + (w < P ? w : 0));
    const bool mine = w < P;
    TF_STAMP(la, 50);
    constexpr int NTOP = (NW * 5 * B2 + 64 * NW - 1) / (64 * NW);
    double topv[NTOP];
    {
        const double* src = lb.crf + chb.nbase * 5 * B2;
#pragma unroll
        for (int q = 0; q < NTOP; ++q) {
            const int i = (int)threadIdx.x + 64 * NW * q, lim = P * 5 * B2 - 1;
            topv[q] = src[i < lim ? i : lim];
        }
    }
    TfCrIo<BB> io(la, ch);
    constexpr int NEF = (MAXLEN * 2 * B2 + 63) / 64;
    double ef[NEF];
#pragma unroll
    for (int q = 0; q < NEF; ++q) {
        const int i = lane + 64 * q;
        const int nd = i / (2 * B2), o = i - nd * 2 * B2;
        const int ndc = nd < ch.mI ? nd : (ch.mI > 0 ? ch.mI - 1 : 0);
        ef[q] = io.crf0[ndc * 5 * B2 + B2 + o];
    }
    TfCrBwdRows<BB> rows;
#pragma unroll
    for (int r = 0; r < 4; ++r) rows.zk[r] = 0.0;
    TF_STAMP(la, 51);
    if (mine) {
        io.next_own = sRhsTop + ch.p * 2 * BB;
        io.next_prev = sRhsTop + ch.pprev * 2 * BB + BB;
        tfk_cr_fwd_chunk<BB, true>(la, ch, lane, sh[w], io, rows.zk);
    }
    TF_STAMP(la, 52);
#pragma unroll
    for (int q = 0; q < NEF; ++q)
        if (lane + 64 * q < MAXLEN * 2 * B2) sEF[w][lane + 64 * q] = ef[q];
#pragma unroll
    for (int q = 0; q < NTOP; ++q) {
        const int i = (int)threadIdx.x + 64 * NW * q;
        if (i < NW * 5 * B2) sCrfTop[i] = topv[q];
    }
    __syncthreads();
    TF_STAMP(la, 53);
    if (w == 0) {
        TfCrIo<BB> iob(lb, chb);
        iob.ys = sRhsTop;
        iob.crf0 = sCrfTop;
        iob.xmirror = sXTop; iob.has_mirror = true;
        tfk_cr_fwd_chunk<BB>(lb, chb, lane, sh[0], iob);
    }
    TF_STAMP(la, 54);
    __syncthreads();
    TF_STAMP(la, 55);
    if (mine) {
        io.xn_own = sXTop + ch.p * BB;
        io.xn_prev = sXTop + ch.pprev * BB;
        tfk_cr_bwd_run<BB, true>(la, ch, lane, sh[w], io, rows, sEF[w]);
    }
    TF_STAMP(la, 56);
}

template <int BB>
__device__ __forceinline__ void tfk_top_factor_coop(const TfTopArgs& a) {
    constexpr int G = 8, NGRP = 8;
    const int grp = threadIdx.x / G, g = threadIdx.x % G;
    const int e = blockIdx.x * NGRP + grp;
    const bool on = e < a.nsys && g < BB;
    const int es = e < a.nsys ? e : 0, gq = g < BB ? g : 0;
    __shared__ double sX[NGRP * 2 * G * (2 * BB + 1)];
    double S[BB], INV[BB];
#pragma unroll
    for (int c = 0; c < BB; ++c) {
        if (a.aos) {
            const double* rec = a.A + (int64_t)es * 4 * BB * BB + gq * BB + c;
            S[c] = rec[0] + rec[BB * BB] + rec[2 * BB * BB] + rec[3 * BB * BB];
        } else {
            S[c] = a.A[(int64_t)((0 * BB + gq) * BB + c) * a.nsys + es]
                 + a.A[(int64_t)((1 * BB + gq) * BB + c) * a.nsys + es]
                 + a.A[(int64_t)((2 * BB + gq) * BB + c) * a.nsys + es];
        }
    }
    bool ok = true;
    const int myk = tf_gj_coop<BB, G>(S, INV, on, g, sX + grp * 2 * G * (2 * BB + 1), ok);
    if (on) {
#pragma unroll
        for (int c = 0; c < BB; ++c) a.Ainv[(int64_t)(myk * BB + c) * a.nsys + e] = INV[c];
        if (!ok) *a.status = 1;
    }
}
```

### triflow_amd/csrc/tf_cr3_hip.h

```cpp
#pragma once

template <int BB> struct TfCr3 {
    static constexpr int MAXLEN = TF_CR_MAXLEN, NPOS = MAXLEN + 1;
    static constexpr int oL = 0, oDL = BB, oU = 2 * BB, oYL = 3 * BB, oDR = 3 * BB + 1, oYR = 4 * BB + 1,
                         oZ = 4 * BB + 2;
    static constexpr int RS = (4 * BB + 3) | 1;
    static constexpr int PS = BB * RS;
    static constexpr int NC = 4 * BB + 1;
    static constexpr bool DUP = NC <= 32;
    static_assert(NC <= 64, "a wavefront holds the augmented columns");
};

__device__ __forceinline__ void tf_st_u(double* ubase, unsigned off8, double v) {
    *(double*)((char*)ubase + off8) = v;
}

template <int BB, int K>
__device__ __forceinline__ void tf_gj3_step(double (&val)[BB], int c, bool& grow) {
    constexpr int PL = BB + K;
    const double pv = tf_readlane_f64(val[K], PL);
    const double rp = tf_rcp_newton(pv);
    if constexpr (K + 1 < BB) {
        double mx = 0.0;
#pragma unroll
        for (int i = K + 1; i < BB; ++i) mx = __builtin_fmax(mx, tf_abs(val[i]));
        if (c == PL && !(mx <= TF_GJ_GROWTH * tf_abs(val[K]))) grow = true;
    }
    const double pr = val[K] * rp;
#pragma unroll
    for (int i = 0; i < BB; ++i) {
        if (i == K) continue;
        const double m = tf_readlane_f64(val[i], PL);
        val[i] = tf_fma(-m, pr, val[i]);
    }
    val[K] = pr;
    if constexpr (K + 1 < BB) tf_gj3_step<BB, K + 1>(val, c, grow);
}

template <int BB>
__device__ __forceinline__ void tfk_cr_factor_v4(const TfLevelArgs& a) {
    typedef TfCr3<BB> C;
    constexpr int NPOS = C::NPOS, B2 = BB * BB, REC = 4 * B2, NT_MIN = 256;
    constexpr int RS = C::RS, PS = C::PS, NC = C::NC;
    constexpr int oL = C::oL, oDL = C::oDL, oU = C::oU, oYL = C::oYL, oDR = C::oDR, oYR = C::oYR, oZ = C::oZ;
    constexpr int NO = 2 * BB + 1;
    constexpr int NQ = (2 * B2 + 63) / 64;
    const int NT = blockDim.x, nw = NT >> 6;
    const TfLayout& L = a.L;
    const TfCrChunk<BB> ch(L, (int)blockIdx.x);
    const int tid = threadIdx.x, w = __builtin_amdgcn_readfirstlane(tid >> 6), lane = tid & 63;
    constexpr bool DUP = C::DUP;
    const int half = DUP ? lane >> 5 : 0, c = DUP ? lane & 31 : lane;
    const int mI = ch.mI, pe = ch.pe, len = ch.len;
    const bool with_rhs = a.cr_rhs != 0;

    __shared__ double sRow[NPOS * PS];
    __shared__ unsigned sPerm[NPOS + 1];
    auto row = [&](int pos, int r) { return sRow + pos * PS + r * RS; };
    unsigned* const perm = a.perm + ch.nbase + ch.start;
    if (tid < len) sPerm[tid + 1] = perm[tid];
    unsigned* const perm_top = a.perm + (int64_t)L.nsys * L.N + ch.e;
    if (a.fold_top && tid == 64) sPerm[0] = *perm_top;

    const bool cL = c < BB, cD = c >= BB && c < 2 * BB, cU = c >= 2 * BB && c < 3 * BB, cY = c == 3 * BB,
               cI = c > 3 * BB && c < NC;
    const int off1 = cL ? oL + c : (cD ? oDL + c - BB : (cU ? oU + c - 2 * BB : (cY ? oYL : oZ)));
    const int off2 = cD ? oDR + c - BB : (cY ? oYR : oZ);
    const int idc = cI ? c - 3 * BB - 1 : -1;
    const bool keepE = half == 0 && (cL || cU), keepZ = half == 0 && cY;
    const bool grec = half == 0 && (cL || cU || cI);
    const unsigned goff = (unsigned)((cI ? idc : (cL ? B2 + c : 2 * B2 + c - 2 * BB)) * 8);
    const bool pvalid = cL || cU || cY;
    auto pacc_of = [&](int sd) { return sd == 0 ? (cL || cY) : (cU || cY); };
    auto pslot_of = [&](int sd) { return sd == 0 ? (cL ? oDR + c : (cU ? oU + c - 2 * BB : oYR))
                                                 : (cL ? oL + c : (cU ? oDL + c - 2 * BB : oYL)); };
    const int pslot0 = pslot_of(DUP ? half : 0), pslot1 = pslot_of(1);
    const bool pacc0 = pacc_of(DUP ? half : 0), pacc1 = pacc_of(1);
    const int opoff0 = (DUP ? half : 0) ? oL : oU;
    int crel[NQ];
    bool cside[NQ], cok[NQ];
#pragma unroll
    for (int q = 0; q < NQ; ++q) {
        const int e = lane + 64 * q, sd = e >= B2 ? 1 : 0, j = e - sd * B2;
        cok[q] = e < 2 * B2;
        cside[q] = sd != 0;
        crel[q] = cok[q] ? (j / BB) * RS + (sd ? oL : oU) + j % BB : 0;
    }

    TF_STAMP_REAL(a, 30);
    TF_STAMP(a, 0);
    {
        const double* src = a.Ablk + (ch.nbase + ch.start) * REC;
        const int n3 = len * 3 * B2;
        constexpr int NIT = (C::MAXLEN * 3 * B2 + NT_MIN - 1) / NT_MIN;
        double v[NIT], v2[NIT];
#pragma unroll
        for (int it = 0; it < NIT; ++it) {
            const int i = it * NT + tid;
            const int nd = i / (3 * B2), rem = i - nd * 3 * B2, blk = rem / B2, rc = rem - blk * B2;
            v[it] = i < n3 ? src[nd * REC + blk * B2 + rc] : 0.0;
            v2[it] = (i < n3 && blk == 1) ? src[nd * REC + 3 * B2 + rc] : 0.0;
        }
        const double* prev = a.Ablk + (ch.nbase + ch.gprev) * REC + 2 * B2;
        double p0 = 0.0, y0 = 0.0;
        if (tid < B2 && ch.has_prev) p0 = prev[tid];
        const double* ys = a.rhs + (ch.nbase + ch.start) * 2 * BB;
        if (with_rhs && tid < len * BB) y0 = ys[(tid / BB) * 2 * BB + tid % BB] + ys[(tid / BB) * 2 * BB + BB + tid % BB];
        for (int i = tid; i < (len + 1) * BB * (RS - 3 * BB); i += NT) {
            const int pr = i / (RS - 3 * BB), o = i - pr * (RS - 3 * BB);
            sRow[(pr / BB) * PS + (pr % BB) * RS + 3 * BB + o] = 0.0;
        }
        if (tid < 3 * B2) {
            const int blk = tid / B2, rc = tid - blk * B2, r = rc / BB, cc = rc - r * BB;
            row(0, r)[blk * BB + cc] = 0.0;
        }
#pragma unroll
        for (int it = 0; it < NIT; ++it) {
            const int i = it * NT + tid;
            const int nd = i / (3 * B2), rem = i - nd * 3 * B2, blk = rem / B2, rc = rem - blk * B2;
            const int r = rc / BB, cc = rc - r * BB;
            if (i < n3) row(nd + 1, r)[blk * BB + cc] = v[it] + v2[it];
        }
        __syncthreads();
        if (tid < B2) row(0, tid / BB)[oU + tid % BB] = p0;
        if (tid < len * BB) row(tid / BB + 1, tid % BB)[oYL] = y0;
        if (!L.periodic) {
            if (ch.start == 0 && tid < B2) row(1, tid / BB)[oL + tid % BB] = 0.0;
            if (ch.start + len == L.N && tid >= 64 && tid < 64 + B2) row(pe, (tid - 64) / BB)[oU + (tid - 64) % BB] = 0.0;
        }
    }
    __syncthreads();

    bool ok = true;
    TF_STAMP(a, 1);
    int stamp_i = 2;
    for (int r = 0; (1 << r) <= mI; ++r) {
        const int s = 1 << r;
        const int nA = ((mI >> r) + 1) >> 1;
        for (int t = w; t < nA; t += nw) {
            const int k = s * (2 * t + 1);
            const int ia = k - s, ib = k + s <= mI ? k + s : pe;
            const double* rk = row(k, 0);
            double* ra = row(ia, 0);
            double* rb = row(ib, 0);
            double* nb = (DUP && half) ? rb : ra;
            if (r == 1) TF_STAMP(a, 44);
            double old[BB], old1[DUP ? 1 : BB], cp[NQ];
#pragma unroll
            for (int i = 0; i < BB; ++i) old[i] = nb[i * RS + pslot0];
            if constexpr (!DUP) {
#pragma unroll
                for (int i = 0; i < BB; ++i) old1[i] = rb[i * RS + pslot1];
            }
#pragma unroll
            for (int q = 0; q < NQ; ++q) cp[q] = (cside[q] ? rb : ra)[crel[q]];
            unsigned code = (unsigned)__builtin_amdgcn_readfirstlane((int)sPerm[k]);
            double val[BB];
            bool done = false;
#pragma unroll 1
            for (int attempt = 0; attempt < 2 && !done; ++attempt) {
#pragma unroll
                for (int i = 0; i < BB; ++i) {
                    const int src = (int)(((code >> (3 * i)) & 7u) ^ (unsigned)i);
                    const double* rr = rk + src * RS;
                    const double v = rr[off1] + rr[off2];
                    val[i] = idc == src ? 1.0 : v;
                }
                bool grow = false;
                tf_gj3_step<BB, 0>(val, c, grow);
                double chk = 0.0;
#pragma unroll
                for (int i = 0; i < BB; ++i) chk += val[i] - val[i];
                if (c < NC && !(chk == 0.0)) grow = true;
                done = __builtin_amdgcn_ballot_w64(grow) == 0ull;
                TF_COUNT(a, 41);
                if (!done) {
                    if (attempt == 1) { ok = false; break; }
                    TF_COUNT(a, 40);
                    constexpr int NJ = (NC + 7) / 8;
                    const int g = lane & 7, h = lane >> 3;
                    double sv[NJ];
#pragma unroll
                    for (int j = 0; j < NJ; ++j) {
                        const int cc = h + 8 * j;
                        const double* rr = rk + (g < BB ? g : 0) * RS;
                        double v = 0.0;
                        if (g < BB) {
                            if (cc < BB) v = rr[oL + cc];
                            else if (cc < 2 * BB) v = rr[oDL + cc - BB] + rr[oDR + cc - BB];
                            else if (cc < 3 * BB) v = rr[oU + cc - 2 * BB];
                            else if (cc == 3 * BB) v = rr[oYL] + rr[oYR];
                            else if (cc < NC) v = cc - 3 * BB - 1 == g ? 1.0 : 0.0;
                        }
                        sv[j] = v;
                    }
                    const int myk = tf_gj_wave<BB, NC, BB>(sv, g, h, ok);
                    unsigned bits = 0;
                    if (g < BB && h == 0) {
                        if (myk >= 0) bits = ((unsigned)(g ^ myk)) << (3 * myk); else ok = false;
                    }
                    code = (unsigned)__builtin_amdgcn_readfirstlane((int)tf_group8_or(bits));
                    if (lane == 0) perm[k - 1] = code;
                }
            }
            if (r == 1) TF_STAMP(a, 45);
            {
                double* rec = a.crf + (ch.nbase + ch.node(k)) * 5 * B2;
                if (grec) {
#pragma unroll
                    for (int i = 0; i < BB; ++i) tf_st_u(rec, goff + (unsigned)(i * BB * 8), val[i]);
                }
#pragma unroll
                for (int q = 0; q < NQ; ++q)
                    if (cok[q]) tf_st_u(rec, (unsigned)((3 * B2 + lane + 64 * q) * 8), cp[q]);
                double* rkw = row(k, 0);
                if (keepZ || (keepE && a.fold_top)) {
#pragma unroll
                    for (int i = 0; i < BB; ++i) rkw[i * RS + off1] = val[i];
                }
            }
            if (r == 1) TF_STAMP(a, 46);
            auto update = [&](double* nbp, int opoff, int pslot, bool pacc, const double* oldv) {
                const double* opb = nbp + opoff;
                double out[BB];
#pragma unroll
                for (int i = 0; i < BB; ++i) {
                    double acc = 0.0;
#pragma unroll
                    for (int m = 0; m < BB; ++m) acc = tf_fma(-opb[i * RS + m], val[m], acc);
                    out[i] = acc;
                }
                if (pvalid) {
#pragma unroll
                    for (int i = 0; i < BB; ++i) nbp[i * RS + pslot] = (pacc ? oldv[i] : 0.0) + out[i];
                }
            };
            update(nb, opoff0, pslot0, pacc0, old);
            if (r == 1) TF_STAMP(a, 47);
            if constexpr (!DUP) update(rb, oL, pslot1, pacc1, old1);
            if (r == 1) TF_STAMP(a, 48);
        }
        TF_STAMP(a, stamp_i); ++stamp_i;
        __syncthreads();
        TF_STAMP(a, stamp_i); ++stamp_i;
    }

    if (with_rhs) {
        double* zt = a.zt + (ch.nbase + ch.start) * BB;
        for (int i = tid; i < mI * BB; i += NT) zt[i] = row(i / BB + 1, i % BB)[oYL];
    }
    for (int i = tid; i < 2 * BB * NO; i += NT) {
        const int side = i / (BB * NO), rem = i - side * BB * NO, r = rem / NO, o = rem - r * NO;
        const int nn = side == 0 ? ch.p : ch.pprev;
        double* rec = a.Anext + ((int64_t)ch.e * a.Lnext.N + nn) * REC;
        double* rr = a.rhsnext + ((int64_t)ch.e * a.Lnext.N + nn) * 2 * BB;
        const double* rs = row(side == 0 ? pe : 0, r);
        if (o < BB) rec[(side == 0 ? 0 : 2) * B2 + r * BB + o] = rs[(side == 0 ? oL : oU) + o];
        else if (o < 2 * BB) rec[(side == 0 ? 1 : 3) * B2 + r * BB + o - BB] = rs[oDL + o - BB] + rs[oDR + o - BB];
        else if (with_rhs) rr[(side == 0 ? 0 : BB) + r] = rs[oYL] + rs[oYR];
    }
    TF_STAMP(a, 20);
    if (a.fold_top) {
        __syncthreads();
        constexpr int NCT = 2 * BB + 1, NJT = (NCT + 7) / 8;
        const int g = lane & 7, h = lane >> 3;
        if (w == 0) {
            const double* r0 = row(0, 0);
            const double* rp = row(pe, 0);
            double val[NJT];
            unsigned code = sPerm[0];
            const unsigned code0 = code;
            const int myk = tf_gj_node<BB, NCT, 0>(val, g, h, code, ok, [&](int rr, int cc) {
                const int o = rr * RS;
                return rr < 0 ? 0.0 : (cc < BB ? rp[o + oL + cc] + (rp[o + oDL + cc] + rp[o + oDR + cc]) + r0[o + oU + cc]
                                                     + (r0[o + oDL + cc] + r0[o + oDR + cc])
                       : (cc == BB ? (rp[o + oYL] + rp[o + oYR]) + (r0[o + oYL] + r0[o + oYR])
                                   : ((cc < NCT && cc - BB - 1 == rr) ? 1.0 : 0.0))); });
            if (code != code0 && lane == 0) *perm_top = code;
            if (g < BB) {
                const int nsys = L.Ptot;
#pragma unroll
                for (int j = 0; j < NJT; ++j) {
                    const int cc = h + 8 * j;
                    if (cc > BB && cc < NCT) a.topAinv[(int64_t)(myk * BB + cc - BB - 1) * nsys + ch.e] = val[j];
                    if (cc == BB && with_rhs) {
                        const double x = val[j];
                        a.topx[(int64_t)ch.e * BB + myk] = x;
                        a.x[(ch.nbase + ch.node(pe)) * BB + myk] = x;
                        row(pe, myk)[oYL] = x;
                        row(0, myk)[oYL] = ch.has_prev ? x : 0.0;
                    }
                }
            }
        }
        if (with_rhs) {
            __syncthreads();
            int r = 0;
            while ((2 << r) <= mI) ++r;
            for (; r >= 0; --r) {
                const int s = 1 << r;
                const int nA = ((mI >> r) + 1) >> 1;
                for (int t = w; t < nA; t += nw) {
                    if (!(h == 0 && g < BB)) continue;
                    const int k = s * (2 * t + 1);
                    const int kl = k - s, kr = k + s <= mI ? k + s : pe;
                    double* rk = row(k, g);
                    double xk = rk[oYL];
#pragma unroll
                    for (int m = 0; m < BB; ++m) {
                        xk = tf_fma(-rk[oL + m], row(kl, m)[oYL], xk);
                        xk = tf_fma(-rk[oU + m], row(kr, m)[oYL], xk);
                    }
                    rk[oYL] = xk;
                    a.x[(ch.nbase + ch.node(k)) * BB + g] = xk;
                }
                __syncthreads();
            }
        }
    }
    if (!ok && lane == 0) *a.status = 1;
    TF_STAMP(a, 21);
    TF_STAMP_REAL(a, 31);
}
```

### triflow_amd/csrc/tf_entry_hip.h

```cpp
#pragma once

#include "tf_coop_hip.h"
#include "tf_cr2_hip.h"
#include "tf_cr3_hip.h"
#include "tf_probe.h"
#include "tf_record.h"

#define TF_GID ((int)(blockIdx.x * blockDim.x + threadIdx.x))

#define TF_ASM_HALF (2 * TF_B2 * TF_B2)
#define TF_ASM_SW (TF_ASM_HALF | 1)
#define TF_FUSE_ASM_OK (TF_ASM_SW * 64 * 8 <= 40 * 1024)
#ifndef TF_L1_SPLIT
#define TF_L1_SPLIT 1
#endif
#define TF_L1_SPLIT_ON (TF_L1_SPLIT && TF_L1_SPLIT_MODEL(TF_MP, TF_NVAR))
#define TF_L1_FACTOR_BLOCK (TF_L1_SPLIT_ON ? 128 : 64)
#define TF_L1_XCH (TF_L1_SPLIT_ON ? 2 * (1 + TF_MP) * TF_NVAR * TF_NVAR * 64 : 1)
#define TF_L1_STAGE (TF_FUSE_ASM_OK ? 64 * TF_ASM_SW : 1)
template <bool WITH_RHS>
__device__ __forceinline__ void tfk_l1_factor_any(const TfLevelArgs& a) {
    __shared__ double stage[TF_L1_STAGE > TF_L1_XCH ? TF_L1_STAGE : TF_L1_XCH];
    __shared__ int srec[64];
    const int lane = threadIdx.x & 63, role = threadIdx.x >> 6, pg = blockIdx.x * 64 + lane;
// ... 42 lines not shown
__global__ void __launch_bounds__(TF_SWEEP_BLOCK) tfk_sweep_f_stage_rhs(TfSweepArgs a) {
    if (a.nterms == 1) tfk_sweep_body<false, true, false, false, true, TF_STAGE_SEG, 1>(a, TF_GID, blockIdx.y);
    else tfk_sweep_body<false, true, false, false, true, TF_STAGE_SEG>(a, TF_GID, blockIdx.y);
}
__global__ void __launch_bounds__(TF_SWEEP_BLOCK) tfk_sweep_f_stage_rhs_n(TfSweepArgs a) {
    switch (a.nterms) {
    case 2: tfk_sweep_body<false, true, false, false, true, TF_STAGE_SEG, 2>(a, TF_GID, blockIdx.y); break;
    case 3: tfk_sweep_body<false, true, false, false, true, TF_STAGE_SEG, 3>(a, TF_GID, blockIdx.y); break;
    case 4: tfk_sweep_body<false, true, false, false, true, TF_STAGE_SEG, 4>(a, TF_GID, blockIdx.y); break;
    case 5: tfk_sweep_body<false, true, false, false, true, TF_STAGE_SEG, 5>(a, TF_GID, blockIdx.y); break;
    default: tfk_sweep_body<false, true, false, false, true, TF_STAGE_SEG>(a, TF_GID, blockIdx.y);
    }
}
__global__ void TF_SWEEP_ATTR __launch_bounds__(TF_SWEEP_BLOCK) tfk_sweep_fj(TfSweepArgs a) {
    tfk_sweep_body<true>(a, TF_GID, blockIdx.y);
}
__global__ void TF_SWEEP_ATTR __launch_bounds__(TF_SWEEP_BLOCK) tfk_sweep_fj_theta(TfSweepArgs a) {
    tfk_sweep_body<true, false, true>(a, TF_GID, blockIdx.y);
}
__global__ void TF_SWEEP_ATTR __launch_bounds__(TF_SWEEP_BLOCK) tfk_sweep_fj_bdf2(TfSweepArgs a) {
    tfk_sweep_body<true, false, false, true>(a, TF_GID, blockIdx.y);
}
__global__ void __launch_bounds__(TF_SWEEP_BLOCK) tfk_spmv(TfSpmvArgs a) {
    tfk_spmv_body(a, TF_GID, blockIdx.y);
}
__device__ __forceinline__ void tf_raise_max(unsigned long long* red, unsigned long long bits) {
    if (bits > __atomic_load_n(red, __ATOMIC_RELAXED)) atomicMax(red, bits);
}

__global__ void __launch_bounds__(256) tfk_vec(TfVecArgs a) {
    const int64_t stride = (int64_t)gridDim.x * blockDim.x;
    for (int64_t i = TF_GID; i < a.n; i += stride) tfk_vec_elem(a, i);
}

__global__ void __launch_bounds__(256) tfk_vec_maxabs(TfVecArgs a) {
    const int64_t stride = (int64_t)gridDim.x * blockDim.x;
    double m = 0.0;
    for (int64_t i = TF_GID; i < a.n; i += stride) {
        const double v = a.op == TF_VEC_MAXRATIO ? tf_vec_ratio(a, i) : (a.op == TF_VEC_SUM_ERR ? tf_vec_sum_err(a, i) : tf_vec_err(a, i));
        m = (v > m || v != v) ? v : m;
    }
    unsigned long long bits = (unsigned long long)__double_as_longlong(m);
    if (m != m) bits = 0x7ff8000000000000ull;
#pragma unroll
    for (int off = 32; off > 0; off >>= 1) {
        const unsigned long long o = __shfl_xor(bits, off, 64);
        bits = o > bits ? o : bits;
    }
    __shared__ unsigned long long part[4];
    const int lane = threadIdx.x & 63, wave = threadIdx.x >> 6;
    if (lane == 0) part[wave] = bits;
    __syncthreads();
    if (threadIdx.x == 0) {
        for (int w = 1; w < (int)(blockDim.x >> 6); ++w) bits = part[w] > bits ? part[w] : bits;
        tf_raise_max((unsigned long long*)a.red, bits);
    }
}

__device__ __forceinline__ void tf_berr_reduce(const TfBerrArgs& a, double m) {
    unsigned long long bits = (unsigned long long)__double_as_longlong(m);
    if (m != m) bits = 0x7ff8000000000000ull;
#pragma unroll
    for (int off = 32; off > 0; off >>= 1) {
        const unsigned long long o = __shfl_xor(bits, off, 64);
        bits = o > bits ? o : bits;
    }
    if ((threadIdx.x & 63) == 0) tf_raise_max((unsigned long long*)a.red, bits);
}
__global__ void __launch_bounds__(TF_SWEEP_BLOCK) tfk_berr(TfBerrArgs a) {
    tf_berr_reduce(a, tfk_berr_body(a, TF_GID, blockIdx.y));
}
__global__ void __launch_bounds__(TF_SWEEP_BLOCK) tfk_sweep_f_stage_rhs_mon(TfStageMonArgs a) {
    if (blockIdx.y + 1 == gridDim.y) { tf_berr_reduce(a.b, tfk_berr_body(a.b, TF_GID, 0)); return; }
    tfk_sweep_body<false, true, false, false, true, TF_STAGE_SEG, 1>(a.s, TF_GID, blockIdx.y);
}

__global__ void __launch_bounds__(256) tfk_diffnorm(TfNormArgs a) {
    double acc = tfk_diffnorm_partial(a, blockIdx.y, blockIdx.x, threadIdx.x, blockDim.x);
#pragma unroll
    for (int off = 32; off > 0; off >>= 1) {
        const double o = __shfl_xor(acc, off, 64);
        acc = a.ord == 2 ? acc + o : (o > acc ? o : acc);
    }
    __shared__ double part[4];
    if ((threadIdx.x & 63) == 0) part[threadIdx.x >> 6] = acc;
    __syncthreads();
    if (threadIdx.x == 0) {
        for (int w = 1; w < (int)(blockDim.x >> 6); ++w)
            acc = a.ord == 2 ? acc + part[w] : (part[w] > acc ? part[w] : acc);
        a.partial[(int64_t)blockIdx.y * a.nblocks + blockIdx.x] = acc;
        if (a.status && blockIdx.x == 0 && blockIdx.y == 0) {
            double* tail = a.partial + (int64_t)gridDim.y * a.nblocks;
            unsigned long long bits = (unsigned)*a.status;
            tail[0] = __longlong_as_double((long long)bits);
            tail[1] = *a.mon;
        }
    }
}

__device__ __forceinline__ TfProbeAcc tf_probe_wave(int kind, TfProbeAcc r) {
#pragma unroll
    for (int off = 32; off > 0; off >>= 1) {
        const TfProbeAcc o{__shfl_xor(r.v, off, 64), __shfl_xor(r.i, off, 64)};
        r = tf_probe_combine(kind, r, o);
    }
    return r;
}
__global__ void __launch_bounds__(256) tfk_probe_partial(TfProbeArgs a) {
    if constexpr (TF_NPROBE > 0) {
        const int e = blockIdx.x / a.nblk, blk = blockIdx.x - e * a.nblk, sg = blockIdx.y;
        const int p = blk * 256 + threadIdx.x;
        const int lane = threadIdx.x & 63, wave = threadIdx.x >> 6;
        TfProbeAcc acc[TF_NPROBE_A];
        if (p < a.L.P) tf_probe_walk(a, e, p, sg, acc);
        else {
#pragma unroll
            for (int k = 0; k < TF_NPROBE; ++k) acc[k] = tf_probe_identity(tf_probe_kind[k]);
        }
        __shared__ double lv[4][TF_NPROBE_A], li[4][TF_NPROBE_A];
#pragma unroll
        for (int k = 0; k < TF_NPROBE; ++k) {
            const TfProbeAcc r = tf_probe_wave(tf_probe_kind[k], acc[k]);
            if (lane == 0) { lv[wave][k] = r.v; li[wave][k] = r.i; }
        }
        __syncthreads();
        if (threadIdx.x < TF_NPROBE) {
            const int k = threadIdx.x, kind = tf_probe_kind[k];
            TfProbeAcc r{lv[0][k], li[0][k]};
            for (int w = 1; w < 4; ++w) r = tf_probe_combine(kind, r, TfProbeAcc{lv[w][k], li[w][k]});
            double* out = a.partial + (((int64_t)e * TF_NPROBE + k) * a.nseg * a.nblk + sg * a.nblk + blk) * 2;
            out[0] = r.v;
            out[1] = r.i;
        }
    }
}
__global__ void __launch_bounds__(256) tfk_probe_final(TfProbeArgs a) {
    if constexpr (TF_NPROBE > 0) {
        const int e = blockIdx.x, lane = threadIdx.x & 63, wave = threadIdx.x >> 6;
        const TfLayout& L = a.L;
        const int row = *(volatile int*)&a.cursor[0];
        const int nb = a.nblk * a.nseg;
        for (int k = wave; k < TF_NPROBE; k += 4) {
            const int kind = tf_probe_kind[k];
            const double* part = a.partial + ((int64_t)e * TF_NPROBE + k) * nb * 2;
            TfProbeAcc r = tf_probe_identity(kind);
            for (int b0 = lane; b0 < nb; b0 += 64 * 8) {
                TfProbeAcc v[8];
#pragma unroll
                for (int j = 0; j < 8; ++j) {
                    const int b = b0 + 64 * j;
                    v[j] = b < nb ? TfProbeAcc{part[2 * b], part[2 * b + 1]} : tf_probe_identity(kind);
                }
#pragma unroll
                for (int j = 0; j < 8; ++j)
                    if (b0 + 64 * j < nb) r = tf_probe_combine(kind, r, v[j]);
            }
            r = tf_probe_wave(kind, r);
            if (lane == 0) {
                double xnode = 0.0;
                if ((kind == TF_PROBE_ARGMAX || kind == TF_PROBE_ARGMIN) && r.i >= 0.0 && r.i < (double)L.N) {
                    int p, i;
                    tf_locate(L, (int)r.i, p, i);
                    xnode = a.xcoord[tf_idx(L, e * L.P + p, i)];
                }
                const double* end = a.ends + ((int64_t)e * TF_NPROBE + k) * 2;
                const double f0 = kind == TF_PROBE_INTEGRAL ? end[0] : 0.0;
                const double fN1 = kind == TF_PROBE_INTEGRAL ? end[1] : 0.0;
                const double val = tf_probe_finish(kind, r, L.N, L.periodic, a.dx[e], f0, fN1, xnode);
                if (row < a.capacity) a.ring[((int64_t)row * L.nsys + e) * TF_NPROBE + k] = val;
            }
        }
        __syncthreads();
        if (threadIdx.x == 0) {
            __threadfence();
            if (atomicAdd(&a.cursor[1], 1) == L.nsys - 1) {
                atomicExch(&a.cursor[1], 0);
                atomicExch(&a.cursor[0], row < a.capacity ? row + 1 : row);
            }
        }
    }
}

__global__ void __launch_bounds__(256) tfk_perm(TfPermArgs a) {
    tfk_perm_elem(a, (int64_t)blockIdx.x * blockDim.x + threadIdx.x);
}
__global__ void __launch_bounds__(256) tfk_gather(TfGatherArgs a) {
    tfk_gather_elem(a, (int64_t)blockIdx.x * blockDim.x + threadIdx.x);
}
__global__ void __launch_bounds__(64) tfk_dirichlet(TfDirichletArgs a) {
    tfk_dirichlet_elem(a, TF_GID);
}
__global__ void __launch_bounds__(64) tfk_poke(TfPokeArgs a) {
    tfk_poke_elem(a, TF_GID);
}

#define TF_L1_ATTR
#if TF_L1_SPLIT_ON
#define TF_L1_FACTOR_ATTR __attribute__((amdgpu_waves_per_eu(2)))
#else
#define TF_L1_FACTOR_ATTR
#endif
__global__ void TF_L1_FACTOR_ATTR __launch_bounds__(TF_L1_FACTOR_BLOCK) tfk_l1_factor(TfLevelArgs a) { tfk_l1_factor_any<false>(a); }
__global__ void TF_L1_FACTOR_ATTR __launch_bounds__(TF_L1_FACTOR_BLOCK) tfk_l1_factor_rhs(TfLevelArgs a) { tfk_l1_factor_any<true>(a); }
__global__ void __launch_bounds__(64) tfk_l1_solve(TfLevelArgs a) {
    TF_WGTRACE(a, 2, 0);
    if (blockIdx.y == 0) tfk_chunk_body<TfRowsL1, +1, false, false, true>(a, TF_GID);
    else tfk_chunk_body<TfRowsL1, -1, false, false, false>(a, TF_GID);
    TF_WGTRACE(a, 2, 1);
}
__global__ void __launch_bounds__(64) tfk_l1_fwd2(TfLevelArgs a) {
    if constexpr (TF_RESPIKE_MODEL(TF_MP, TF_NVAR)) {
        if (blockIdx.y == 0) tfk_chunk_body<TfRowsL1, +1, false, false, true, true>(a, TF_GID);
        else tfk_chunk_body<TfRowsL1, -1, false, false, true, true>(a, TF_GID);
    }
}
__global__ void TF_L1_ATTR __launch_bounds__(128) tfk_l1_fwd2_backsub(TfLevelArgs a) {
    if constexpr (TF_RESPIKE_MODEL(TF_MP, TF_NVAR)) {
        extern __shared__ double tf_dyn_lds[];
        TF_WGTRACE(a, 1, 0);
        const int lane = threadIdx.x & 63, dir = threadIdx.x >> 6, pg = blockIdx.x * 64 + lane;
        double* ydn = tf_dyn_lds + lane;
        double* yup = tf_dyn_lds + (size_t)a.ylds_rows * TF_NVAR * 64 + lane;
        if (dir == 0) tfk_chunk_body<TfRowsL1, +1, false, false, true, true, true>(a, pg, ydn);
        else tfk_chunk_body<TfRowsL1, -1, false, false, true, true, true>(a, pg, yup);
        __syncthreads();
        TF_STAMP(a, 3);
        tfk_backsub_twist_body<TfRowsL1, true>(a, pg, dir, ydn, yup);
        TF_STAMP(a, 8);
        TF_WGTRACE(a, 1, 1);
    }
}
__global__ void __launch_bounds__(64 * TF_MP) tfk_l1_asm_mat(TfLevelArgs a) {
    constexpr int NREC = 3 * TF_B2 * TF_B2, SW = NREC | 1;
    const int lane = threadIdx.x & 63, pg = blockIdx.x * 64 + lane;
    const int tsel = blockDim.x > 64 ? (int)(threadIdx.x >> 6) : -1;
    if constexpr (SW * 64 * 8 <= 64 * 1024) {
        if (a.next_aos) {
            __shared__ double stage[64 * SW];
            tfk_asm_body<TfRowsL1, true>(a, pg, stage + lane * SW, tsel);
            __syncthreads();
            const int pg0 = blockIdx.x * 64;
            const int nrec = a.L.Ptot - pg0 < 64 ? a.L.Ptot - pg0 : 64;
            double* dst = a.Anext + (int64_t)pg0 * 4 * TF_B2 * TF_B2;
            for (int idx = threadIdx.x; idx < nrec * NREC; idx += blockDim.x) {
                const int t = idx / NREC, off = idx - t * NREC;
                dst[(int64_t)t * 4 * TF_B2 * TF_B2 + off] = stage[t * SW + off];
            }
            return;
        }
    }
    tfk_asm_body<TfRowsL1, true>(a, pg, nullptr, tsel);
}
__global__ void __launch_bounds__(64 * TF_MP) tfk_l1_asm_rhs(TfLevelArgs a) {
    tfk_asm_body<TfRowsL1, false>(a, blockIdx.x * 64 + (threadIdx.x & 63), nullptr,
                                  blockDim.x > 64 ? (int)(threadIdx.x >> 6) : -1);
}
__global__ void TF_L1_ATTR __launch_bounds__(64) tfk_l1_backsub(TfLevelArgs a) { tfk_backsub_body<TfRowsL1, true>(a, TF_GID); }
__global__ void TF_L1_ATTR __launch_bounds__(64) tfk_l1_backsub_u(TfLevelArgs a) {
    if constexpr (TF_RESPIKE_MODEL(TF_MP, TF_NVAR)) tfk_backsub_twist_body<TfRowsL1>(a, TF_GID, (int)blockIdx.y);
}

typedef TfRowsBT<TF_B2> TfRowsUp;
__global__ void __launch_bounds__(64) tfk_bt_lu(TfLevelArgs a) {
    if constexpr (TfCoop<TF_B2>::G > 1) tfk_bt_lu_coop<TF_B2>(a, blockIdx.y == 0 ? +1 : -1);
    else tfk_bt_lu_body<TF_B2>(a, TF_GID, blockIdx.y == 0 ? +1 : -1);
}
__global__ void __launch_bounds__(64) tfk_bt_spike(TfLevelArgs a) {
    if constexpr (TfCoop<TF_B2>::G > 1)
        tfk_bt_col_coop<TF_B2>(a, (blockIdx.y & 1) == 0 ? +1 : -1, blockIdx.y >> 1);
    else tfk_bt_col_body<TF_B2>(a, TF_GID, (blockIdx.y & 1) == 0 ? +1 : -1, blockIdx.y >> 1);
}
__global__ void __launch_bounds__(64) tfk_bt_rhs(TfLevelArgs a) {
    if constexpr (TfCoop<TF_B2>::G > 1) tfk_bt_col_coop<TF_B2>(a, blockIdx.y == 0 ? +1 : -1, TF_B2);
    else tfk_bt_col_body<TF_B2>(a, TF_GID, blockIdx.y == 0 ? +1 : -1, TF_B2);
}
__global__ void __launch_bounds__(64) tfk_bt_asm_mat(TfLevelArgs a) {
    if constexpr (TfCoop<TF_B2>::G > 1) tfk_bt_asm_coop<TF_B2, true>(a);
    else tfk_asm_body<TfRowsUp, true>(a, TF_GID);
}
__global__ void __launch_bounds__(64) tfk_bt_asm_rhs(TfLevelArgs a) {
    if constexpr (TfCoop<TF_B2>::G > 1) tfk_bt_asm_coop<TF_B2, false>(a);
    else tfk_asm_body<TfRowsUp, false>(a, TF_GID);
}
__global__ void __launch_bounds__(64) tfk_bt_backsub(TfLevelArgs a) {
    if constexpr (TfCoop<TF_B2>::G > 1) tfk_bt_backsub_coop<TF_B2>(a);
    else tfk_backsub_body<TfRowsUp>(a, TF_GID);
}
__global__ void __launch_bounds__(64) tfk_top_factor(TfTopArgs a) {
    if constexpr (TfCoop<TF_B2>::G == 8) tfk_top_factor_coop<TF_B2>(a);
    else tfk_top_body<TF_B2, true>(a, TF_GID);
}
__global__ void __launch_bounds__(64) tfk_top_solve(TfTopArgs a) { tfk_top_body<TF_B2, false>(a, TF_GID); }
__global__ void __launch_bounds__(64) tfk_tiny_factor(TfTinyArgs a) { tfk_tiny_factor_body(a, TF_GID); }
__global__ void __launch_bounds__(64) tfk_tiny_solve(TfTinyArgs a) { tfk_tiny_solve_body(a, TF_GID); }

#define TF_CR_BLOCK (TF_B2 <= 2 ? 256 : 64)
#define TF_CR_FACTOR_BLOCK (TF_B2 <= 2 ? 256 : 512)
#ifndef TF_CR_FACTOR_WAVES
#define TF_CR_FACTOR_WAVES (TF_B2 >= 8 ? 2 : 4)
#endif
__global__ void __attribute__((amdgpu_waves_per_eu(TF_CR_FACTOR_WAVES))) __launch_bounds__(TF_CR_FACTOR_BLOCK)
tfk_cr_factor(TfLevelArgs a) {
    if constexpr (TF_B2 <= 2) tfk_crs_factor<TF_B2, 256>(a, (int)blockIdx.x, (int)threadIdx.x);
    else if constexpr (TF_B2 <= 8) tfk_cr_factor_v4<TF_B2>(a);
}
__global__ void __launch_bounds__(TF_CR_BLOCK) tfk_cr_fwd(TfLevelArgs a) {
    if constexpr (TF_B2 <= 2) tfk_crs_fwd<TF_B2, 256>(a, (int)blockIdx.x, (int)threadIdx.x);
    else if constexpr (TF_B2 <= 8) tfk_cr_fwd_coop<TF_B2>(a);
}
__global__ void __launch_bounds__(TF_CR_BLOCK) tfk_cr_bwd(TfLevelArgs a) {
    if constexpr (TF_B2 <= 2) tfk_crs_bwd<TF_B2, 256>(a, (int)blockIdx.x, (int)threadIdx.x);
    else if constexpr (TF_B2 <= 8) tfk_cr_bwd_coop<TF_B2>(a);
}
__device__ __forceinline__ void tf_own4(const TfLayout& L2, int blk, int& e, int& q0, int& nq, int& c0, int& cnt) {
    const int qps = (L2.P + 3) / 4;
    e = blk / qps;
    q0 = (blk - e * qps) * 4;
    nq = L2.P - q0 < 4 ? L2.P - q0 : 4;
    c0 = tf_start(L2, q0);
    cnt = tf_start(L2, q0 + nq - 1) + tf_len(L2, q0 + nq - 1) - c0;
}
__global__ void TF_L1_ATTR __launch_bounds__(128) tfk_l1_solve_cr(TfTailArgs t) {
    if constexpr (TF_B2 >= 3 && TF_B2 <= 6) {
        const TfLevelArgs& l1 = t.lv[0];
        const TfLevelArgs& l2 = t.lv[1];
        __shared__ TfCrSolveLds<TF_B2> sh[2];
        const int lane = threadIdx.x & 63, w = __builtin_amdgcn_readfirstlane((int)threadIdx.x >> 6);
        int e, q0, nq, c0, cnt;
        tf_own4(l2.L, (int)blockIdx.x, e, q0, nq, c0, cnt);
        const int P1 = l1.L.P;
        const TfCrChunk<TF_B2> cha(l2.L, e * l2.L.P + q0 + (w < nq ? w : 0));
        const TfCrChunk<TF_B2> chb(l2.L, e * l2.L.P + q0 + (w + 2 < nq ? w + 2 : 0));
        const TfCrIo<TF_B2> ioa(l2, cha), iob(l2, chb);
        TfCrFwdRows<TF_B2> ra, rb;
        TF_STAMP(l2, 57);
        tfk_cr_fwd_load<TF_B2>(cha, lane, ioa, ra);
        if (lane < cnt) {
            if (w == 0) tfk_chunk_body<TfRowsL1, +1, false, false, true>(l1, e * P1 + c0 + lane);
            else {
                int c = c0 + lane + 1;
                if (c == P1) c = l1.L.periodic ? 0 : -1;
                if (c >= 0) tfk_chunk_body<TfRowsL1, -1, false, false, false>(l1, e * P1 + c);
            }
        }
        TF_STAMP(l2, 58);
        __builtin_amdgcn_fence(__ATOMIC_RELEASE, "workgroup");
        __syncthreads();
        __builtin_amdgcn_fence(__ATOMIC_ACQUIRE, "workgroup");
        TF_STAMP(l2, 59);
        double ya[TF_CR_NYS(TF_B2)], yb[TF_CR_NYS(TF_B2)];
        tfk_cr_fwd_load_ys<TF_B2>(cha, lane, ioa, ya);
        tfk_cr_fwd_load_ys<TF_B2>(chb, lane, iob, yb);
        tfk_cr_fwd_load<TF_B2>(chb, lane, iob, rb);
        if (w < nq) tfk_cr_fwd_chunk<TF_B2, false, true>(l2, cha, lane, sh[w], ioa, nullptr, &ra, ya);
        TF_STAMP(l2, 60);
        if (w + 2 < nq) tfk_cr_fwd_chunk<TF_B2, false, true>(l2, chb, lane, sh[w], iob, nullptr, &rb, yb);
        TF_STAMP(l2, 61);
    }
}
__global__ void TF_L1_ATTR __launch_bounds__(128) tfk_l1_fwd2_backsub_cr(TfTailArgs t) {
    if constexpr (TF_RESPIKE_MODEL(TF_MP, TF_NVAR) && TF_B2 >= 3 && TF_B2 <= 6) {
        extern __shared__ double tf_dyn_lds[];
        const TfLevelArgs& a = t.lv[0];
        const TfLevelArgs& l2 = t.lv[1];
        __shared__ TfCrSolveLds<TF_B2> sh[2];
        const int lane = threadIdx.x & 63, dir = __builtin_amdgcn_readfirstlane((int)threadIdx.x >> 6);
        int e, q0, nq, c0, cnt;
        tf_own4(l2.L, (int)blockIdx.x, e, q0, nq, c0, cnt);
        const TfCrChunk<TF_B2> cha(l2.L, e * l2.L.P + q0 + (dir < nq ? dir : 0));
        const TfCrChunk<TF_B2> chb(l2.L, e * l2.L.P + q0 + (dir + 2 < nq ? dir + 2 : 0));
        const TfCrIo<TF_B2> ioa(l2, cha), iob(l2, chb);
        TfCrBwdRows<TF_B2> ra, rb;
        TF_STAMP(l2, 62);
        tfk_cr_bwd_load<TF_B2>(l2, cha, lane, ioa, ra, true);
        const double xa = tfk_cr_bwd_sep<TF_B2>(lane, ioa);
        tfk_cr_bwd_load<TF_B2>(l2, chb, lane, iob, rb, true);
        const double xb = tfk_cr_bwd_sep<TF_B2>(lane, iob);
        if (dir < nq) {
            if (dir == 0 && cha.has_prev && lane >= TfCr<TF_B2>::G && lane < TfCr<TF_B2>::G + TF_B2)
                l2.x[(cha.nbase + cha.gprev) * TF_B2 + lane - TfCr<TF_B2>::G] = xa;
            tfk_cr_bwd_run<TF_B2, false, true>(l2, cha, lane, sh[dir], ioa, ra, nullptr, xa);
        }
        if (dir + 2 < nq) tfk_cr_bwd_run<TF_B2, false, true>(l2, chb, lane, sh[dir], iob, rb, nullptr, xb);
        TF_STAMP(l2, 63);
        __builtin_amdgcn_fence(__ATOMIC_RELEASE, "workgroup");
        __syncthreads();
        __builtin_amdgcn_fence(__ATOMIC_ACQUIRE, "workgroup");
        const int pg = lane < cnt ? e * a.L.P + c0 + lane : a.L.Ptot;
        double* ydn = tf_dyn_lds + lane;
        double* yup = tf_dyn_lds + (size_t)a.ylds_rows * TF_NVAR * 64 + lane;
        if (dir == 0) tfk_chunk_body<TfRowsL1, +1, false, false, true, true, true>(a, pg, ydn);
        else tfk_chunk_body<TfRowsL1, -1, false, false, true, true, true>(a, pg, yup);
        __syncthreads();
        tfk_backsub_twist_body<TfRowsL1, true>(a, pg, dir, ydn, yup);
    }
}

__global__ void __launch_bounds__(512) tfk_s_fwd(TfScalarArgs t) {
    if constexpr (TF_B2 <= 2) {
        const TfLevelArgs& l1 = t.lv[0];
        const TfLevelArgs& l2 = t.lv[1];
        const int tid = threadIdx.x;
        const TfCrChunk<TF_B2> ch(l2.L, (int)blockIdx.x);
        const int P1 = l1.L.P;
        __shared__ double sF2[(TF_CRS_MAXLEN + 1) * 5 * TF_B2 * TF_B2], sF3[TfCrs<TF_B2>::FSIZE];
        TF_STAMP(l2, 57);
        TF_STAMP_REAL(l2, 30);
        TfCrsStaged<TF_B2, 512, TF_CRS_MAXLEN> rF2;
        TfCrsStaged<TF_B2, 512, TF_CRS_TOPLEN(TF_B2)> rF3;
        tfk_crs_stage_request<TF_B2, 512>(l2, (int)blockIdx.x, tid, rF2);
        tfk_crs_stage_request<TF_B2, 512>(t.lv[2], ch.e, tid, rF3);
        double topv[TF_B2 * TF_B2];
#pragma unroll
        for (int i = 0; i < TF_B2 * TF_B2; ++i) topv[i] = tid == 0 ? t.lv[2].topAinv[(int64_t)i * t.lv[2].L.Ptot + ch.e] : 0.0;
        TF_STAMP(l2, 58);
        __shared__ double sRhs[TF_CRS_MAXLEN * 2 * TF_B2];
        TfLevelArgs l1w = l1;
        l1w.rhsnext = (double*)sRhs - ((int64_t)ch.e * l1.Lnext.N + ch.start) * 2 * TF_B2;
        if (tid < 256) {
            if (tid < ch.len) tfk_chunk_body<TfRowsL1, +1, false, false, true>(l1w, ch.e * P1 + ch.start + tid);
        } else if (tid - 256 < ch.len) {
            int c = ch.start + tid - 256 + 1;
            if (c == P1) c = l1.L.periodic ? 0 : -1;
            if (c >= 0) tfk_chunk_body<TfRowsL1, -1, false, false, false>(l1w, ch.e * P1 + c);
            else if (TF_B2 > 0) {
#pragma unroll
                for (int r = 0; r < TF_B2; ++r) sRhs[(tid - 256) * 2 * TF_B2 + TF_B2 + r] = 0.0;
            }
        }
        tfk_crs_stage_put<TF_B2, 512>(l2, (int)blockIdx.x, tid, rF2, sF2);
        tfk_crs_stage_put<TF_B2, 512>(t.lv[2], ch.e, tid, rF3, sF3);
        TF_STAMP(l2, 59);
        __syncthreads();
        TF_STAMP(l2, 60);
        tfk_crs_fwd<TF_B2, 512, true, true>(l2, (int)blockIdx.x, tid, sF2, sRhs);
        TF_STAMP(l2, 61);
        __shared__ int last;
        if (tid < 64) {
            asm volatile("s_waitcnt vmcnt(0)" ::: "memory");
            if (tid == 0) {
                const unsigned seen = __hip_atomic_fetch_add(t.counter + ch.e, 1u, __ATOMIC_RELAXED, __HIP_MEMORY_SCOPE_AGENT);
                const int is_last = seen == (unsigned)l2.L.P - 1u;
                if (is_last) __hip_atomic_store(t.counter + ch.e, 0u, __ATOMIC_RELAXED, __HIP_MEMORY_SCOPE_AGENT);
                last = is_last;
            }
        }
        __syncthreads();
        TF_STAMP(l2, 62);
        TF_STAMP_IF(l2, 55, last);
        TF_STAMP_REAL_IF(l2, 32, last);
        if (last) tfk_crs_fwd<TF_B2, 512, true, false, true, true>(t.lv[2], ch.e, tid, sF3, nullptr, topv);
        TF_STAMP_IF(l2, 56, last);
        TF_STAMP_REAL_IF(l2, 31, last);
    }
}
__global__ void __launch_bounds__(512) tfk_s_bwd(TfScalarArgs t) {
    if constexpr (TF_B2 <= 2) {
        const TfLevelArgs& l1 = t.lv[0];
        const TfLevelArgs& l2 = t.lv[1];
        const int tid = threadIdx.x;
        const TfCrChunk<TF_B2> ch(l2.L, (int)blockIdx.x);
        TF_STAMP(l2, 50);
        tfk_crs_bwd<TF_B2, 512>(l2, (int)blockIdx.x, tid, true);
        TF_STAMP(l2, 51);
        __builtin_amdgcn_fence(__ATOMIC_RELEASE, "workgroup");
        __syncthreads();
        __builtin_amdgcn_fence(__ATOMIC_ACQUIRE, "workgroup");
        TF_STAMP(l2, 52);
        if (tid < ch.len) tfk_backsub_body<TfRowsL1, true>(l1, ch.e * l1.L.P + ch.start + tid);
        TF_STAMP(l2, 53);
    }
}
__global__ void __launch_bounds__(64 * TF_CR_TAIL_WAVES) tfk_cr_tail(TfTailArgs t) {
    if constexpr (TF_B2 >= 3 && TF_B2 <= TF_CR_TAIL_MAXB) tfk_cr_tail_coop<TF_B2>(t);
}

}
```

### triflow_amd/csrc/tf_rt_diag.cpp

```cpp
#include "tf_solver.h"

extern "C" {

int tf_backward_error(tf_solver* s, double* omega, int32_t* refined) {
    TF_API_BEGIN
    require(s, "null solver");
    if (omega) *omega = s->last_omega;
    if (refined) *refined = s->fact_needs_refine ? 1 : 0;
    TF_API_END
}

int tf_debug_stamps(tf_solver* s, uint64_t* out, int32_t max_levels) {
    TF_API_BEGIN
    require(s && out, "null argument");
    const size_t regions = std::max<size_t>(std::max<size_t>(s->levels.size(), 1), (size_t)std::max(max_levels, 0));
    const size_t need = 64 * regions;
    if (s->stamp_buf.n < need) { s->drop_graphs(); s->stamp_buf.alloc(need, s->bytes); return 0; }
    const size_t n = 64 * std::min<size_t>(s->stamp_buf.n / 64, (size_t)std::max(max_levels, 0));
    tfb::d2h(out, s->stamp_buf.p, n * sizeof(uint64_t), s->stream);
    TF_API_END
}

int tf_monitor_error(tf_solver* s, double* worst) {
    TF_API_BEGIN
    require(s && worst, "null argument");
    *worst = 0.0;
    if (s->monitored) tfb::d2h(worst, s->red.p + 4, sizeof(double), s->stream);
    TF_API_END
}

int tf_solver_counters(tf_solver* s, int64_t* factorisations, int64_t* checks, int64_t* replans) {
    TF_API_BEGIN
    require(s, "null solver");
    if (factorisations) *factorisations = s->n_factor;
    if (checks) *checks = s->n_checks;
    if (replans) *replans = s->n_replans;
    TF_API_END
}

int tf_solver_kernel_block(tf_solver* s, int32_t kernel, int32_t* block) {
    TF_API_BEGIN
    require(s && block, "null argument");
    require(kernel >= 0 && kernel < TFK_COUNT, "no such kernel");
    *block = (int32_t)tfb::kernel_block(s->model->module, kernel);
    TF_API_END
}

int tf_sync(tf_solver* s) {
    TF_API_BEGIN
    require(s, "null solver");
    tfb::stream_sync(s->stream);
    s->check_status();
    TF_API_END
}

int tf_timing_enable(tf_solver* s, int64_t on) {
    TF_API_BEGIN
    require(s, "null solver");
    s->collect_timing();
    s->timing = on < 0 ? ~0ull : (uint64_t)on;
    TF_API_END
}
int tf_timing_reset(tf_solver* s) {
    TF_API_BEGIN
    require(s, "null solver");
    s->collect_timing();
    for (int k = 0; k < TFK_COUNT; ++k) { s->time_ms[k] = 0; s->time_n[k] = 0; }
    TF_API_END
}
int tf_timing_get(tf_solver* s, int32_t kernel, double* total_ms, int64_t* launches) {
    TF_API_BEGIN
    require(s, "null solver");
    require(kernel >= 0 && kernel < TFK_COUNT, "tf_timing_get: kernel index");
    s->collect_timing();
    if (total_ms) *total_ms = s->time_ms[kernel];
    if (launches) *launches = s->time_n[kernel];
    TF_API_END
}

}
```

### triflow_amd/csrc/tf_rt_plan.cpp

```cpp
#include "tf_solver.h"

namespace tfrt { thread_local std::string g_last_error; }

extern "C" {

const char* tf_last_error(void) { return g_last_error.c_str(); }

int tf_runtime_info(int32_t* is_device_build, int32_t* device_count) {
    TF_API_BEGIN
    if (is_device_build) *is_device_build = tfb::is_device_build() ? 1 : 0;
    if (device_count) *device_count = tfb::device_count();
    TF_API_END
}

int tf_set_device(int32_t ordinal) {
    TF_API_BEGIN
    tfb::set_device(ordinal);
    TF_API_END
}

int tf_kernel_count(void) { return TFK_COUNT; }
const char* tf_kernel_name(int32_t kernel) {
    return tf_kernel_entry(kernel);
}

int tf_model_create(const tf_model_spec* spec, const void* code, size_t size, tf_model** out) {
    TF_API_BEGIN
    require(spec && out, "tf_model_create: null argument");
    require(spec->nvar >= 1 && spec->nvar + spec->nh <= TF_MAX_FIELDS, "tf_model_create: bad field count");
    require(spec->npar >= 0 && spec->npar <= TF_MAX_PARS, "tf_model_create: bad parameter count");
    require(spec->mp >= 1 && spec->seg >= 1 && spec->sweep_block >= 64, "tf_model_create: bad stencil constants");
    std::unique_ptr<tf_model> m(new tf_model());
    m->spec = *spec;
    m->module = tfb::module_load(code, size);
    *out = m.release();
    TF_API_END
}

int tf_model_add_alternate(tf_model* model, const void* code, size_t size, uint64_t kernel_mask) {
    TF_API_BEGIN
    require(model && code, "tf_model_add_alternate: null argument");
    tfb::module_add_alternate(model->module, code, size, kernel_mask);
    TF_API_END
}

void tf_model_destroy(tf_model* model) { delete model; }

}
namespace {
tf_solver* make_solver(tf_model* model, int64_t N, int32_t nsys, int32_t periodic,
                       const tf_solver_opts* opts, tfb::Stream* shared) {
    require(model != nullptr, "tf_solver_create: null argument");
    const tf_model_spec& sp = model->spec;
    require(nsys >= 1, "tf_solver_create: nsys must be >= 1");
    require(N >= (periodic ? sp.mp : 1), "tf_solver_create: a periodic grid needs at least mp nodes");
    require(N * (int64_t)nsys < (int64_t)1 << 31, "tf_solver_create: too many nodes for 32-bit chunk indices");
    std::unique_ptr<tf_solver> s(new tf_solver());
    s->model = model; s->spec = sp; s->N = N; s->nsys = nsys; s->periodic = periodic ? 1 : 0;
    int m1 = opts && opts->m1 > 0 ? opts->m1 : 0;
    int mup = opts && opts->m_upper > 0 ? opts->m_upper : 6;
    s->nstate = opts && opts->nstate > 0 ? opts->nstate : 3;
    s->refine = opts ? opts->refine : -1;
    if (opts && opts->berr_every > 0) { s->berr_every = s->berr_cur = opts->berr_every; s->berr_adaptive = false; }
    if (opts && opts->device >= 0) tfb::set_device(opts->device);
    mup = std::max(mup, 2);
    if (shared) { s->stream = shared; s->owns_stream = false; }
    else s->stream = tfb::stream_create();
    if (const char* v = getenv("TRIFLOW_REPLAN")) s->replan_on = atoi(v) != 0;
    s->graphs_on = tfb::graphs_supported() && (int64_t)N * nsys <= 50000;
    if (const char* v = getenv("TRIFLOW_GRAPHS")) s->graphs_on = tfb::graphs_supported() && atoi(v) != 0;
    if (const char* v = getenv("TRIFLOW_FUSE_STAGE")) s->fuse_stage = atoi(v) != 0;
    if (const char* v = getenv("TRIFLOW_S_FUSE")) s->s_fuse = atoi(v) != 0;
    if (const char* v = getenv("TRIFLOW_L1CR_FUSE")) s->l1cr_fuse = atoi(v) != 0;
    if (const char* v = getenv("TRIFLOW_L1_FUSE_BACKSUB")) s->l1_fuse_backsub = atoi(v) != 0;
    if (const char* v = getenv("TRIFLOW_L1_FUSE_ASM")) s->l1_fuse_asm = atoi(v) != 0;
    if (const char* v = getenv("TRIFLOW_FUSE_UPDATE")) s->upd_fuse = atoi(v) != 0;
    if (const char* v = getenv("TRIFLOW_HOOK_IN_PLACE")) s->hook_in_place = atoi(v) != 0;
    s->l1_respike = TF_RESPIKE_MODEL(sp.mp, sp.nvar) && (int64_t)N * nsys >= TF_RESPIKE_MIN_NODES;
    if (const char* v = getenv("TRIFLOW_L1_TWIST")) s->l1_twist = atoi(v) != 0 ? 1 : 0;
    if (const char* v = getenv("TRIFLOW_L1_RESPIKE"))
        s->l1_respike = TF_RESPIKE_MODEL(sp.mp, sp.nvar) && atoi(v) != 0;

    const int b2 = sp.mp * sp.nvar;
    s->use_cr = tfb::cyclic_reduction(b2);
    if (m1 == 0) {
        const int64_t total = (int64_t)N * nsys;
        m1 = 32;
        const bool dispersive_capable = sp.nvar == 1 && sp.mp >= 2;
        if (s->use_cr && !dispersive_capable)
            m1 = total <= 30000 ? 4 : (total <= 200000 ? 8 : (total <= 600000 ? 16 : 32));
        if (s->use_cr && !dispersive_capable && b2 <= 2 && total > 600000) {
            m1 = 16;
            while (N / m1 > TF_CRS_MAXLEN * TF_CRS_TOPLEN(b2)) m1 *= 2;
        }
    }
    m1 = std::max(m1, 2 * sp.mp);
    s->m1_used = m1; s->mup_used = mup;
    s->tiny = N < 2 * sp.mp + 1;
    {
        const int cr_cap = b2 <= 2 ? TF_CRS_MAXLEN : TF_CR_MAXLEN;
        const int cr_len = opts && opts->m_upper > 0 ? std::min(std::max(opts->m_upper, 2), cr_cap) : cr_cap;
        int64_t cr_max_nodes = (int64_t)1 << 40;
        if (const char* v = getenv("TRIFLOW_CR_MAX_NODES")) cr_max_nodes = atoll(v);
        int n = (int)N, B = sp.nvar, MP = sp.mp, m = m1;
        bool first = true;
        while (true) {
            const bool cr = !first && s->use_cr && (int64_t)n * nsys <= cr_max_nodes;
            int P = std::max(1, n / m);
            if (cr) P = (n + cr_len - 1) / cr_len;
            if (cr && b2 <= 2 && cr_len == cr_cap && n <= TF_CRS_TOPLEN(b2)) P = 1;
            std::unique_ptr<Level> lv(new Level());
            lv->L = make_layout(nsys, n, P, s->periodic);
            lv->B = B; lv->MP = MP; lv->cr = cr;
            s->levels.push_back(std::move(lv));
            if (P == 1) break;
            n = P; B = b2; MP = 1; m = mup; first = false;
        }
        s->top.L = make_layout(nsys, 1, 1, s->periodic);
        s->top.B = b2; s->top.MP = 1;
    }
    s->L1 = s->levels[0]->L;
    const int64_t plane = s->L1.plane;
    require(plane < ((int64_t)1 << 29), "tf_solver_create: more than 2^29 nodes per solver (a plane is addressed with 32-bit byte offsets)");

    int64_t& tot = s->bytes;
    for (int i = 0; i < s->nstate; ++i) {
        s->state.emplace_back(new DevBuf());
        s->state.back()->alloc((size_t)sp.nvar * plane, tot);
    }
    s->helpers.alloc((size_t)sp.nh * plane, tot);
    if (sp.parvec_mask) s->parvec.alloc((size_t)sp.npar * plane, tot); else s->parvec.alloc(1, tot);
    s->parsca.alloc((size_t)std::max(sp.npar, 1) * nsys, tot);
    s->dx.alloc(nsys, tot);
    if (sp.uses_x) s->xcoord.alloc(plane, tot); else s->xcoord.alloc(1, tot);
    s->F.alloc((size_t)sp.nvar * plane, tot);
    s->Jv.alloc((size_t)std::max(sp.nnz, 1) * plane, tot);
    DevBuf* work[] = {&s->Wstage, &s->Wsum, &s->Wjv, &s->Wrhs, &s->Wres, &s->Wdel};
    for (DevBuf* w : work) w->alloc((size_t)sp.nvar * plane, tot);
    for (int i = 0; i < TF_MAX_TERMS; ++i) s->K[i].alloc(i < 6 ? (size_t)sp.nvar * plane : 1, tot);
    s->red.alloc(8, tot);
    s->status = (int*)tfb::dev_alloc(sizeof(int));
    if (b2 <= 2) s->sfuse_counter = (unsigned*)tfb::dev_alloc((size_t)nsys * sizeof(unsigned));
    for (size_t l = 0; l < s->levels.size(); ++l) s->levels[l]->alloc(l, nsys, s->l1_respike, tot);
    s->top.alloc_top(b2, nsys, tot);
    s->topAinv.alloc((size_t)b2 * b2 * nsys, tot);
    if (s->tiny) {
        const size_t n = (size_t)N * sp.nvar;
        s->tiny_lu.alloc(n * n * nsys, tot);
        s->tiny_piv = (int*)tfb::dev_alloc(n * nsys * sizeof(int));
    }
    return s.release();
}
}

tf_solver* tf_solver::ensure_fallback() {
    if (fallback) return fallback;
    tf_solver_opts o;
    std::memset(&o, 0, sizeof(o));
    o.m1 = (int32_t)std::min<int64_t>(N, std::max<int64_t>(64, 8 * (int64_t)m1_used));
    o.m_upper = 0; o.nstate = 1; o.refine = -1; o.device = -1;
    o.berr_every = 1;
    fallback = make_solver(model, N, nsys, periodic, &o, stream);
    fallback->refine_trigger = 1e-14;
    bytes += fallback->bytes;
    return fallback;
}

extern "C" {
int tf_solver_create(tf_model* model, int64_t N, int32_t nsys, int32_t periodic,
                     const tf_solver_opts* opts, tf_solver** out) {
    TF_API_BEGIN
    require(model && out, "tf_solver_create: null argument");
    *out = make_solver(model, N, nsys, periodic, opts, nullptr);
    TF_API_END
}

void tf_solver_destroy(tf_solver* solver) {
    if (!solver) return;
    try { tfb::stream_sync(solver->stream); } catch (...) {}
    delete solver;
}

int tf_solver_describe(tf_solver* s, int32_t* nlevels, int32_t* chunks, int32_t max_levels,
                       int64_t* device_bytes) {
    TF_API_BEGIN
    require(s, "null solver");
    if (nlevels) *nlevels = (int32_t)s->levels.size();
    if (chunks)
        for (size_t l = 0; l < s->levels.size() && (int)l < max_levels; ++l) chunks[l] = s->levels[l]->L.P;
    if (device_bytes) *device_bytes = s->bytes;
    TF_API_END
}
}
```

### triflow_amd/csrc/tf_solver.h

```cpp
#pragma once
#include "../../include/triflow_hip.h"
#include "tf_args.h"
#include "tf_backend.h"

#include <algorithm>
#include <cmath>
#include <cstdio>
#include <cstdlib>
#include <cstring>
#include <map>
#include <memory>
#include <stdexcept>
#include <string>
#include <vector>

namespace tfrt {

extern thread_local std::string g_last_error;

#define TF_API_BEGIN try {
#define TF_API_END                                               \
    return 0;                                                    \
    }                                                            \
    catch (const std::exception& ex) { g_last_error = ex.what(); return 1; } \
    catch (...) { g_last_error = "unknown error"; return 1; }

inline void require(bool cond, const char* msg) {
    if (!cond) throw std::invalid_argument(msg);
}

inline TfLayout make_layout(int nsys, int N, int P, int periodic) {
    TfLayout L;
    L.nsys = nsys; L.N = N; L.P = P;
    L.mbase = N / P; L.rem = N % P;
    L.M = L.mbase + (L.rem > 0 ? 1 : 0);
    L.Ptot = nsys * P;
    L.periodic = periodic;
    L.plane = (int64_t)L.M * L.Ptot;
    return L;
}

struct DevBuf {
    double* p = nullptr;
    size_t n = 0;
    void alloc(size_t count, int64_t& total) {
        release();
        n = count;
        p = (double*)tfb::dev_alloc(std::max<size_t>(count, 1) * sizeof(double));
        total += (int64_t)(std::max<size_t>(count, 1) * sizeof(double));
    }
    void release() { if (p) tfb::dev_free(p); p = nullptr; n = 0; }
    void swap(DevBuf& o) { std::swap(p, o.p); std::swap(n, o.n); }
    ~DevBuf() { release(); }
    DevBuf() = default;
    DevBuf(const DevBuf&) = delete;
    DevBuf& operator=(const DevBuf&) = delete;
};

struct Level {
    TfLayout L;
    int B = 0, MP = 0;
    bool cr = false;
    DevBuf Ablk, rhs, x, Ut, Et, yt, tips_dn, tips_up, Dinv, Unup;
    DevBuf crf, zt;
    unsigned* perm = nullptr;
    ~Level() { if (perm) tfb::dev_free(perm); }
    Level() = default;
    Level(const Level&) = delete;
    Level& operator=(const Level&) = delete;
    void swap(Level& o) {
        std::swap(L, o.L); std::swap(B, o.B); std::swap(MP, o.MP); std::swap(cr, o.cr); std::swap(perm, o.perm);
        DevBuf* mine[] = {&Ablk, &rhs, &x, &Ut, &Et, &yt, &tips_dn, &tips_up, &Dinv, &Unup, &crf, &zt};
        DevBuf* theirs[] = {&o.Ablk, &o.rhs, &o.x, &o.Ut, &o.Et, &o.yt, &o.tips_dn, &o.tips_up, &o.Dinv, &o.Unup, &o.crf, &o.zt};
        for (int i = 0; i < 12; ++i) mine[i]->swap(*theirs[i]);
    }
    void alloc(size_t l, int nsys, bool l1_respike, int64_t& tot) {
        const int64_t pl = L.plane;
        if (cr) {
            const size_t nodes = (size_t)L.N * nsys;
            Ablk.alloc(nodes * 4 * B * B, tot);
            rhs.alloc(nodes * 2 * B, tot);
            x.alloc(nodes * B, tot);
            crf.alloc(nodes * 5 * B * B, tot);
            zt.alloc(nodes * B, tot);
            perm = (unsigned*)tfb::dev_alloc((nodes + nsys) * sizeof(unsigned));
            tot += (int64_t)((nodes + nsys) * sizeof(unsigned));
            return;
        }
        const int UW = (l == 0 && B == 1) ? 2 * MP : MP;
        Ut.alloc((size_t)UW * B * B * pl, tot);
        if (l == 0 && l1_respike) Et.alloc(1, tot);
        else Et.alloc((size_t)MP * B * B * pl, tot);
        yt.alloc((size_t)B * pl, tot);
        const size_t tipsz = (size_t)(MP * B + 2 * MP * MP * B * B) * L.Ptot;
        tips_dn.alloc(tipsz, tot);
        tips_up.alloc(tipsz, tot);
        if (l > 0) {
            Ablk.alloc((size_t)3 * B * B * pl, tot);
            Dinv.alloc((size_t)2 * B * B * pl, tot);
            Unup.alloc((size_t)B * B * pl, tot);
            rhs.alloc((size_t)B * pl, tot);
            x.alloc((size_t)B * pl, tot);
        }
    }
    void alloc_top(int b2, int nsys, int64_t& tot) {
        Ablk.alloc((size_t)4 * b2 * b2 * nsys, tot);
        rhs.alloc((size_t)2 * b2 * nsys, tot);
        x.alloc((size_t)b2 * nsys, tot);
    }
};

}
using namespace tfrt;

enum {
    TF_VEC_SUM = 0, TF_VEC_LIN2 = 1, TF_VEC_THETA_RHS = 2, TF_VEC_MAXABS = 3, TF_VEC_COPY = 4,
    TF_VEC_BDF2_RHS = 5, TF_VEC_ADD = 6, TF_VEC_RESID = 7, TF_VEC_MAXRATIO = 8, TF_VEC_SUM_ERR = 9
};

struct tf_model {
    tf_model_spec spec;
    tfb::Module* module = nullptr;
    ~tf_model() { tfb::module_unload(module); }
};

struct tf_solver {
    tf_model* model = nullptr;
    tf_model_spec spec;
    int64_t N = 0;
    int nsys = 1, periodic = 0, nstate = 3, refine = 0;
    TfLayout L1;
    bool use_cr = false;
    unsigned cr_block() const { return top.B <= 2 ? 256u : 64u; }
    unsigned cr_factor_block(int64_t chunks) const {
        if (top.B <= 2) return 256u;
        const char* v = getenv("TRIFLOW_CR_FACTOR_BLOCK");
        if (v) return atoi(v) >= 512 ? 512u : 256u;
        return chunks > 1024 ? 256u : 512u;
    }
    bool fold_top() const { return levels.size() > 1 && levels.back()->cr; }
    bool level_cr(size_t l) const { return l < levels.size() && levels[l]->cr; }
    bool next_aos(size_t l) const { return l + 1 < levels.size() ? levels[l + 1]->cr : levels.back()->cr; }
    tfb::Stream* stream = nullptr;
    int64_t bytes = 0;

    std::vector<std::unique_ptr<DevBuf>> state;
    DevBuf helpers, parvec, parsca, dx, xcoord;
    DevBuf F, Jv, Wstage, Wsum, Wjv, Wrhs, Wres, Wdel, K[TF_MAX_TERMS];
    DevBuf staging, normbuf;
    DevBuf red;
    int* status = nullptr;
    tfb::Mailbox* err_box[4] = {nullptr, nullptr, nullptr, nullptr};
    std::vector<std::unique_ptr<Level>> levels;
    Level top;
    DevBuf topAinv;
    double factor_c = 0.0;
    bool have_factor = false, have_jac = false;
    std::vector<std::unique_ptr<Level>> levels_alt;
    Level top_alt;
    DevBuf topAinv_alt;
    bool alt_allocated = false;
    int slot_id = 0;
    struct SlotMeta {
        double factor_c = 0.0, cf_c = 0.0;
        bool have_factor = false, cf_valid = false, fact_checked = false, fact_needs_refine = false,
             check_now = true, delegated = false;
        uint64_t cf_ver = 0;
        int sweeps_needed = 0;
    } meta_alt;
    bool fact_checked = false, fact_needs_refine = false;
    double last_omega = 0.0, refine_trigger = 1e-11, monitor_omega = 0.0;
    int berr_every = 8;
    int berr_cur = 8, berr_max = 64;
    bool berr_adaptive = true;
    int64_t n_factor = 0, n_checks = 0, n_replans = 0;
    bool check_now = true;
    struct Checked { double c; int sweeps; int64_t at; bool replan; };
    std::vector<Checked> checked;
    Checked* checked_like(double c) {
        for (auto& e : checked)
            if (std::fabs(c - e.c) <= 0.1 * std::fabs(e.c)) return &e;
        return nullptr;
    }

    int ndir = 0;
    int *dir_var = nullptr, *dir_node = nullptr;
    DevBuf dir_val, dir_val_post;

    DevBuf stamp_buf;
    int* csc_map = nullptr;
    int64_t csc_n = 0;
    char* poke_buf = nullptr;
    size_t poke_bytes = 0;

    struct BdfHist { DevBuf Uprev; bool have_prev = false; double dt_prev = 0.0; };
    BdfHist bdf0;
    std::map<int64_t, std::unique_ptr<BdfHist>> bdf_owned;

    enum LaunchMode { TF_EAGER = 0, TF_CAPTURE, TF_DRY };
    LaunchMode mode = TF_EAGER;
    bool graphs_on = false;
    struct GraphEntry { tfb::Graph* graph; int64_t used; };
    std::map<std::string, GraphEntry> graphs;
    int64_t graph_clock = 0, graph_replays = 0;
    void drop_graphs() {
        if (!graphs.empty()) { try { tfb::stream_sync(stream); } catch (...) {} }
        for (auto& kv : graphs) tfb::graph_destroy(kv.second.graph);
        graphs.clear();
    }
    std::map<std::string, int64_t> seen_once;
    template <class Fn> void run_graphed(const std::string& key, bool graphable, Fn fn) {
        if (!graphs_on || !graphable || timing != 0) { fn(); return; }
        auto it = graphs.find(key);
        if (it == graphs.end()) {
            auto seen = seen_once.find(key);
            if (seen == seen_once.end()) {
                if (seen_once.size() >= 64) seen_once.clear();
                seen_once.emplace(key, ++graph_clock);
                fn();
                return;
            }
            seen_once.erase(seen);
            tfb::capture_begin(stream);
            mode = TF_CAPTURE;
            try { fn(); } catch (...) { mode = TF_EAGER; tfb::capture_abort(stream); throw; }
            mode = TF_EAGER;
            tfb::Graph* g = tfb::capture_end(stream);
            if (graphs.size() >= 8) {
                auto victim = graphs.begin();
                for (auto jt = graphs.begin(); jt != graphs.end(); ++jt)
                    if (jt->second.used < victim->second.used) victim = jt;
                tfb::stream_sync(stream);
                tfb::graph_destroy(victim->second.graph);
                graphs.erase(victim);
            }
            it = graphs.emplace(key, GraphEntry{g, 0}).first;
        } else {
            mode = TF_DRY;
            try { fn(); } catch (...) { mode = TF_EAGER; throw; }
            mode = TF_EAGER;
            ++graph_replays;
        }
        it->second.used = ++graph_clock;
        tfb::graph_launch(it->second.graph, stream);
    }
    bool step_graphable(double c) {
        if (const Checked* like = checked_like(c); like && like->replan) return false;
        if (reuse_ok(c)) return refine != -1 || fact_checked;
        if (alt_ok(c)) return refine != -1 || meta_alt.fact_checked;
        return !check_due(c);
    }
    void prepare_step(double c) { if (wants_alt(c)) ensure_alt(); }
    bool check_due(double c) {
        if (refine != -1) return false;
        const Checked* like = checked_like(c);
        return n_factor + 1 <= 4 || !like || n_factor + 1 - like->at >= berr_cur;
    }
    int sweeps_for(double c) { const Checked* like = checked_like(c); return like ? like->sweeps : -1; }
    void zero(void* p, size_t nbytes) { if (mode != TF_DRY) tfb::memset0(p, nbytes, stream); }
    void copy(void* dst, const void* src, size_t nbytes) { if (mode != TF_DRY) tfb::d2d(dst, src, nbytes, stream); }

    uint64_t timing = 0;
    struct Stamp { int kernel; tfb::Event *a, *b; };
    std::vector<Stamp> stamps;
    std::vector<tfb::Event*> event_pool;
    double time_ms[TFK_COUNT] = {0};
    int64_t time_n[TFK_COUNT] = {0};

    ~tf_solver() {
        for (auto& st : stamps) { tfb::event_destroy(st.a); tfb::event_destroy(st.b); }
        for (auto* e : event_pool) tfb::event_destroy(e);
        drop_graphs();
        if (poke_buf) tfb::dev_free(poke_buf);
        if (csc_map) tfb::dev_free(csc_map);
        if (status) tfb::dev_free(status);
        if (sfuse_counter) tfb::dev_free(sfuse_counter);
        for (auto* m : err_box) tfb::mailbox_destroy(m);
        if (dir_var) tfb::dev_free(dir_var);
        if (dir_node) tfb::dev_free(dir_node);
        delete fallback;
        if (tiny_piv) tfb::dev_free(tiny_piv);
        if (owns_stream) tfb::stream_destroy(stream);
    }

    int64_t plane() const { return L1.plane; }
    int64_t vecn() const { return (int64_t)spec.nvar * L1.plane; }
    double* st(int slot) {
        if (slot < 0 || slot >= nstate) throw std::invalid_argument("state slot out of range");
        return state[slot]->p;
    }

    tfb::Event* get_event() {
        if (!event_pool.empty()) { auto* e = event_pool.back(); event_pool.pop_back(); return e; }
        return tfb::event_create();
    }
    void launch(int kernel, unsigned gx, unsigned gy, unsigned block, const void* args, size_t sz,
                unsigned lds_bytes = 0) {
        if (mode == TF_DRY) return;
        if ((timing >> kernel) & 1ull) {
            Stamp stp{kernel, get_event(), get_event()};
            tfb::launch_timed(model->module, kernel, gx, gy, block, args, sz, stream, stp.a, stp.b, lds_bytes);
            stamps.push_back(stp);
        } else {
            tfb::launch(model->module, kernel, gx, gy, block, args, sz, stream, lds_bytes);
        }
    }
    void collect_timing() {
        if (stamps.empty()) return;
        tfb::stream_sync(stream);
        for (auto& stp : stamps) {
            time_ms[stp.kernel] += tfb::event_elapsed_ms(stp.a, stp.b);
            time_n[stp.kernel] += 1;
            event_pool.push_back(stp.a);
            event_pool.push_back(stp.b);
        }
        stamps.clear();
    }
    static unsigned cdiv(int64_t a, int64_t b) { return (unsigned)((a + b - 1) / b); }
    unsigned sweep_gx() const {
        const unsigned gx = cdiv(L1.Ptot, spec.sweep_block);
        return gx > 8 ? (gx + 7u) / 8u * 8u : gx;
    }

    void vec(int op, double* out, const double* base, int nterms, const double* const* xs, const double* cs, int64_t n = -1, int red_slot = 0, const double* cs2 = nullptr);

    void perm(int mode, const double* src, double* dst, int ncomp);
    void ensure_staging(size_t count);
    void upload_planes(const double* host, double* planes, int ncomp);
    void download_planes(const double* planes, double* host, int ncomp);
    void upload_aos(const double* host, double* planes, int ncomp);
    void download_aos(const double* planes, double* host, int ncomp);

    void apply_dirichlet(double* fields, bool post = false);

    void sweep(const double* fields, bool with_j, int nterms = 0, const double* const* kx = nullptr, const double* kc = nullptr, double fscale = 1.0, double* Fout = nullptr);
    void sweep_bdf2(const double* fields, bool two_step, double c0, double c1, double* rhs, const double* prev, double* prev_out);
    void sweep_theta(const double* fields, double dt, double theta, double* rhs);
    void spmv(const double* v, double* y, double scale, bool absval = false);

    bool fuse_stage = true;
    bool jconst = false, cf_valid = false, reused = false;
    double cf_c = 0.0;
    uint64_t par_ver = 0, cf_ver = 0;
    static bool same_c(double a, double b) { return a == b || std::fabs(a - b) <= 1e-15 * std::fabs(b); }
    bool reuse_ok(double c) const { return jconst && cf_valid && have_jac && same_c(cf_c, c) && cf_ver == par_ver; }
    bool alt_ok(double c) const;
    bool wants_alt(double c) const;
    bool two_slots = true;
    void ensure_alt();
    void swap_slots();
    std::string slot_key(double c) const;
    bool l1_respike = false;
    int l1_twist = -1;
    bool l1_fuse_asm = true;
    bool fuse_asm_ok() const;
    unsigned l1_factor_block_ = 0;
    unsigned l1_factor_block();
    bool tiny = false;
    DevBuf tiny_lu;
    int* tiny_piv = nullptr;
    TfTinyArgs tiny_args(const double* rhs1, double* x1);
    bool l1_fuse_backsub = true;
    void stage_rhs(const double* Uin, int nterms, const double* const* ks, const double* ac, const double* gc, double dt, double* y,
                   const TfBerrArgs* probe = nullptr);
    void spmv_stage(int nterms, const double* const* vx, const double* vc, const double* Fp, double cF, double cA, double* y);

    std::vector<std::vector<double>> slot_hook;
    std::vector<double> dir_h, dir_post_h;
    bool hook_in_place = true;
    void slot_written(int slot) { if (slot >= 0 && (size_t)slot < slot_hook.size()) slot_hook[slot].clear(); }
    void mark_hooked(int slot, bool post = true);
    bool input_is_hooked(int src) const;
    const double* stage_input(int src, double* U);

    unsigned asm_block() const { return tfb::is_device_build() ? 64u * (unsigned)spec.mp : 64u; }
    Level& next_of(size_t l) { return l + 1 < levels.size() ? *levels[l + 1] : top; }
    unsigned l1_twist_lds(TfLevelArgs& a) const;
    TfLevelArgs level_args(size_t l, const double* rhs1, double* x1);
    TfTopArgs top_args();
    void factor(double c, const double* rhs1 = nullptr, double* x1 = nullptr);
    void factor_step(double c, const double* rhs1, double* x1);
    struct Update { double* out; const double* base; const double* k0; double c0, c1; int n; };
    Update upd_req{};
    bool upd_req_on = false, upd_done = false;
    bool upd_fuse = true;
    void request_update(double* out, const double* base, const double* k0, double c0, double c1, int n);
    bool take_update_done() { const bool d = upd_done; upd_done = false; upd_req_on = false; return d; }
    bool update_allowed() const;
    void backsub_chain(const double* rhs1, double* x1, int skip);
    bool s_fuse = true;
    unsigned* sfuse_counter = nullptr;
    bool l1cr_fuse = true;
    bool l1cr_ok() const;
    bool scalar_fused_ok() const;
    TfScalarArgs scalar_args(const double* rhs1, double* x1);
    bool cr_tail = true;
    bool tail_ok() const;
    void solve_once(const double* rhs1, double* x1);
    void refine_sweep(const double* rhs1, double* x1);
    double backward_error(const double* rhs1, const double* x1);
    unsigned mon_phase = 0;
    bool sampled_monitor_due() const;
    void monitor_sampled(const double* rhs1, const double* x1, const double* xbase);
    TfBerrArgs probe_args(const double* rhs1, const double* x1, const double* xbase);
    void solve(const double* rhs1, double* x1);
    int sweeps_needed = 0;
    bool unstable = false;

    tf_solver* fallback = nullptr;
    bool owns_stream = true;
    int m1_used = 0, mup_used = 0;
    bool delegated = false;
    bool replan_on = true;
    bool can_replan() const { return replan_on && refine == -1 && !tiny && !levels.empty() && levels[0]->L.P > 1; }
    tf_solver* ensure_fallback();
    void transfer_to(tf_solver* dst, const double* src_planes, double* dst_planes, int ncomp);
    double fb_c = 0.0;
    uint64_t fb_ver = 0;
    bool fb_valid = false;
    bool fb_touched = false;
    void delegate_factor(double c);
    void delegate_solve(const double* rhs1, double* x1);
    void polish(const double* rhs1, double* x1);

    bool monitored = false;
    void check_status(const int* have_flag = nullptr, const double* have_worst = nullptr);
};
```

### triflow_amd/csrc/tf_solver_linear.cpp

```cpp
#include "tf_solver.h"

unsigned tf_solver::l1_twist_lds(TfLevelArgs& a) const {
    if (!(l1_respike && a.twist && l1_fuse_backsub && tfb::is_device_build())) return 0;
    auto half = [&](int mI) { return (spec.mp * spec.nvar <= 6 && mI >= 4 * spec.mp) ? (mI + 1) / 2 : mI; };
    const int mI_max = a.L.M - spec.mp;
    a.ylds_rows = std::max(half(mI_max), a.L.rem > 0 ? half(mI_max - 1) : 0);
    const size_t lds = (size_t)2 * a.ylds_rows * spec.nvar * 64 * sizeof(double);
    return lds <= 80u * 1024u ? (unsigned)lds : 0u;
}

TfLevelArgs tf_solver::level_args(size_t l, const double* rhs1, double* x1) {
    Level& lv = *levels[l];
    Level& nx = next_of(l);
    TfLevelArgs a;
    std::memset(&a, 0, sizeof(a));
    a.L = lv.L; a.Jv = Jv.p; a.parsca = parsca.p; a.dx = dx.p; a.c = factor_c; a.Ablk = lv.Ablk.p;
    a.rhs = l == 0 ? rhs1 : lv.rhs.p;
    a.x = l == 0 ? x1 : lv.x.p;
    a.Ut = lv.Ut.p; a.Et = lv.Et.p; a.yt = lv.yt.p; a.Dinv = lv.Dinv.p; a.Unup = lv.Unup.p;
    a.tips_dn = lv.tips_dn.p; a.tips_up = lv.tips_up.p;
    a.Lnext = nx.L; a.Anext = nx.Ablk.p; a.rhsnext = nx.rhs.p; a.xnext = nx.x.p;
    a.status = status;
    a.next_aos = next_aos(l) ? 1 : 0; a.crf = lv.crf.p; a.zt = lv.zt.p; a.perm = lv.perm;
    a.fold_top = fold_top() && l + 1 == levels.size() ? 1 : 0;
    a.respike = l == 0 && l1_respike ? 1 : 0;
    a.fuse_asm = l == 0 && fuse_asm_ok() ? 1 : 0;
    a.twist = a.respike && (l1_twist < 0 ? lv.L.Ptot <= TF_TWIST_MAX_CHUNKS : l1_twist > 0) ? 1 : 0;
    if (a.respike && l1_twist < 0 && !a.twist) { a.twist = 1; if (!l1_twist_lds(a)) a.twist = 0; }
    a.topAinv = topAinv.p; a.topx = top.x.p;
    a.stamps = stamp_buf.n ? (unsigned long long*)stamp_buf.p + 64 * l : nullptr;
    return a;
}

TfTopArgs tf_solver::top_args() {
    TfTopArgs t;
    t.nsys = nsys; t.A = top.Ablk.p; t.rhs = top.rhs.p; t.Ainv = topAinv.p; t.x = top.x.p; t.status = status;
    t.aos = levels.back()->cr ? 1 : 0;
    return t;
}

void tf_solver::factor(double c, const double* rhs1, double* x1) {
    if (!have_jac) throw std::runtime_error("tf_factor: no Jacobian evaluated yet (call tf_eval with_j=1)");
    factor_c = c;
    delegated = false;
    if (const Checked* like0 = checked_like(c); like0 && like0->replan && can_replan()) {
        ++n_factor;
        have_factor = true; cf_valid = jconst; cf_c = c; cf_ver = par_ver;
        check_now = false; fact_checked = true; sweeps_needed = 0;
        delegate_factor(c);
        if (rhs1) delegate_solve(rhs1, x1);
        return;
    }
    const bool fused = rhs1 != nullptr && !tiny;
    if (tiny) {
        TfTinyArgs t = tiny_args(nullptr, nullptr);
        launch(TFK_TINY_FACTOR, cdiv(nsys, 64), 1, 64, &t, sizeof(t));
    }
    for (size_t l = 0; l < levels.size() && !tiny; ++l) {
        TfLevelArgs a = level_args(l, rhs1, x1);
        if (!fused) a.rhs = nullptr;
        unsigned gx = cdiv(a.L.Ptot, 64);
        if (l == 0) launch(fused ? TFK_L1_FACTOR_RHS : TFK_L1_FACTOR, gx, 2, l1_factor_block(), &a, sizeof(a));
        else if (levels[l]->cr) {
            a.cr_rhs = fused ? 1 : 0;
            launch(TFK_CR_FACTOR, (unsigned)a.L.Ptot, 1, cr_factor_block(a.L.Ptot), &a, sizeof(a));
            continue;
        } else {
            const int G = tfb::coop_group(levels[l]->B);
            const unsigned gc = cdiv((int64_t)a.L.Ptot * G, 64);
            const int ncols = levels[l]->B + (fused ? 1 : 0);
            a.lu_cols = G > 1 ? ncols : 0;
            launch(TFK_BT_LU, gc, 2, 64, &a, sizeof(a));
            if (G == 1) launch(TFK_BT_SPIKE, gc, 2 * (unsigned)ncols, 64, &a, sizeof(a));
        }
        if (l == 0) { if (!a.fuse_asm) launch(TFK_L1_ASM_MAT, gx, 1, asm_block(), &a, sizeof(a)); }
        else launch(TFK_BT_ASM_MAT, cdiv((int64_t)a.L.Ptot * tfb::coop_group(levels[l]->B), 64), 1, 64, &a, sizeof(a));
    }
    if (!fold_top() && !tiny) { TfTopArgs t = top_args(); launch(TFK_TOP_FACTOR, cdiv((int64_t)nsys * (tfb::coop_group(top.B) == 8 ? 8 : 1), 64), 1, 64, &t, sizeof(t)); }
    have_factor = true;
    ++n_factor;
    cf_valid = jconst; cf_c = c; cf_ver = par_ver;
    const Checked* like = checked_like(c);
    check_now = refine == -1 && (n_factor <= 4 || !like || n_factor - like->at >= berr_cur);
    if (check_now) { fact_checked = false; fact_needs_refine = false; sweeps_needed = 0; }
    else if (like) { sweeps_needed = like->sweeps; fact_needs_refine = sweeps_needed > 0; }
    if (rhs1 == nullptr) return;
    if (!fused) { solve(rhs1, x1); return; }
    if (!fold_top()) { TfTopArgs t = top_args(); launch(TFK_TOP_SOLVE, cdiv(nsys, 64), 1, 64, &t, sizeof(t)); }
    backsub_chain(rhs1, x1, fold_top() ? 1 : 0);
    polish(rhs1, x1);
}

void tf_solver::factor_step(double c, const double* rhs1, double* x1) {
    reused = reuse_ok(c);
    if (!reused && alt_ok(c)) { swap_slots(); reused = true; }
    else if (wants_alt(c)) { ensure_alt(); swap_slots(); }
    if (!reused) { factor(c, rhs1, x1); return; }
    have_factor = true;
    solve(rhs1, x1);
}

void tf_solver::request_update(double* out, const double* base, const double* k0, double c0, double c1, int n) {
    upd_req = Update{out, base, k0, c0, c1, n};
    upd_req_on = upd_fuse;
    upd_done = false;
}

bool tf_solver::update_allowed() const {
    return !delegated && !tiny && refine <= 0 && (refine != -1 || (fact_checked && sweeps_needed == 0));
}

void tf_solver::backsub_chain(const double* rhs1, double* x1, int skip) {
    if (skip == 1 && scalar_fused_ok()) {
        TfScalarArgs t = scalar_args(rhs1, x1);
        upd_req_on = false;
        launch(TFK_S_BWD, (unsigned)t.lv[1].L.Ptot, 1, 512, &t, sizeof(t));
        return;
    }
    bool l2_in_l1 = false;
    if (l1cr_ok() && levels.size() - (size_t)skip >= 2) {
        TfLevelArgs a0 = level_args(0, rhs1, x1);
        const unsigned lds0 = l1_twist_lds(a0);
        l2_in_l1 = lds0 > 0 && lds0 <= 64u * 1024u;
    }
    for (size_t l = levels.size() - (size_t)skip; l-- > 0;) {
        if (l == 1 && l2_in_l1) continue;
        TfLevelArgs a = level_args(l, rhs1, x1);
        if (l == 0) {
            const unsigned gy = a.twist ? 2u : 1u;
            const bool take = upd_req_on && update_allowed();
            upd_req_on = false;
            if (const unsigned lds = l1_twist_lds(a)) {
                if (take) {
                    a.upd_out = upd_req.out; a.upd_base = upd_req.base; a.upd_k0 = upd_req.k0;
                    a.upd_c0 = upd_req.c0; a.upd_c1 = upd_req.c1; a.upd_n = upd_req.n;
                    upd_done = true;
                }
                if (l2_in_l1) {
                    TfTailArgs t;
                    t.lv[0] = a;
                    t.lv[1] = level_args(1, rhs1, x1);
                    launch(TFK_L1_FWD2_BACKSUB_CR, (unsigned)nsys * cdiv(t.lv[1].L.P, 4), 1, 128, &t, sizeof(t), lds);
                    continue;
                }
                launch(TFK_L1_FWD2_BACKSUB, cdiv(a.L.Ptot, 64), 1, 128, &a, sizeof(a), lds);
                continue;
            }
            if (l1_respike) launch(TFK_L1_FWD2, cdiv(a.L.Ptot, 64), gy, 64, &a, sizeof(a));
            launch(l1_respike ? TFK_L1_BACKSUB_U : TFK_L1_BACKSUB, cdiv(a.L.Ptot, 64), gy, 64, &a, sizeof(a));
        }
        else if (levels[l]->cr) launch(TFK_CR_BWD, (unsigned)a.L.Ptot, 1, cr_block(), &a, sizeof(a));
        else launch(TFK_BT_BACKSUB, cdiv((int64_t)a.L.Ptot * tfb::coop_group(levels[l]->B), 64), 1, 64, &a, sizeof(a));
    }
}

bool tf_solver::l1cr_ok() const {
    return l1cr_fuse && tfb::is_device_build() && !tiny && top.B >= 3 && top.B <= 6 && levels.size() >= 4 &&
           levels[1]->cr && levels[2]->cr && fuse_asm_ok();
}

bool tf_solver::scalar_fused_ok() const {
    return s_fuse && tfb::is_device_build() && !tiny && top.B <= 2 && levels.size() == 3 && levels[1]->cr &&
           levels[2]->cr && levels[2]->L.P == 1 && fold_top() && fuse_asm_ok() && !l1_respike;
}

TfScalarArgs tf_solver::scalar_args(const double* rhs1, double* x1) {
    TfScalarArgs t;
    for (size_t l = 0; l < 3; ++l) t.lv[l] = level_args(l, rhs1, x1);
    if (!sfuse_counter) sfuse_counter = (unsigned*)tfb::dev_alloc((size_t)nsys * sizeof(unsigned));
    t.counter = sfuse_counter;
    return t;
}

bool tf_solver::tail_ok() const {
    const size_t n = levels.size();
    return cr_tail && tfb::is_device_build() && n >= 3 && top.B >= 3 && top.B <= 6 && levels[n - 1]->cr && levels[n - 2]->cr &&
           levels[n - 1]->L.P == 1 && levels[n - 2]->L.P <= 8;
}

void tf_solver::solve_once(const double* rhs1, double* x1) {
    if (tiny) {
        TfTinyArgs t = tiny_args(rhs1, x1);
        launch(TFK_TINY_SOLVE, cdiv(nsys, 64), 1, 64, &t, sizeof(t));
        return;
    }
    if (scalar_fused_ok()) {
        TfScalarArgs t = scalar_args(rhs1, x1);
        launch(TFK_S_FWD, (unsigned)t.lv[1].L.Ptot, 1, 512, &t, sizeof(t));
        backsub_chain(rhs1, x1, 1);
        return;
    }
    const bool tail = tail_ok();
    for (size_t l = 0; l < levels.size(); ++l) {
        if (tail && l + 2 == levels.size()) {
            TfTailArgs t;
            t.lv[0] = level_args(l, rhs1, x1);
            t.lv[1] = level_args(l + 1, rhs1, x1);
            launch(TFK_CR_TAIL, (unsigned)nsys, 1, 64u * 8u, &t, sizeof(t));
            backsub_chain(rhs1, x1, 2);
            return;
        }
        if (l == 0 && l1cr_ok()) {
            TfTailArgs t;
            t.lv[0] = level_args(0, rhs1, x1);
            t.lv[1] = level_args(1, rhs1, x1);
            launch(TFK_L1_SOLVE_CR, (unsigned)nsys * cdiv(t.lv[1].L.P, 4), 1, 128, &t, sizeof(t));
            l = 1;
            continue;
        }
        TfLevelArgs a = level_args(l, rhs1, x1);
        unsigned gx = cdiv(a.L.Ptot, 64);
        if (l == 0) launch(TFK_L1_SOLVE, gx, 2, 64, &a, sizeof(a));
        else if (levels[l]->cr) { launch(TFK_CR_FWD, (unsigned)a.L.Ptot, 1, cr_block(), &a, sizeof(a)); continue; }
        else launch(TFK_BT_RHS, cdiv((int64_t)a.L.Ptot * tfb::coop_group(levels[l]->B), 64), 2, 64, &a, sizeof(a));
        if (l == 0) { if (!a.fuse_asm) launch(TFK_L1_ASM_RHS, gx, 1, asm_block(), &a, sizeof(a)); }
        else launch(TFK_BT_ASM_RHS, cdiv((int64_t)a.L.Ptot * tfb::coop_group(levels[l]->B), 64), 1, 64, &a, sizeof(a));
    }
    if (!fold_top()) { TfTopArgs t = top_args(); launch(TFK_TOP_SOLVE, cdiv(nsys, 64), 1, 64, &t, sizeof(t)); }
    backsub_chain(rhs1, x1, fold_top() ? 1 : 0);
}

void tf_solver::refine_sweep(const double* rhs1, double* x1) {
    spmv(x1, Wjv.p, factor_c);
    const double* xs[3] = {rhs1, x1, Wjv.p};
    vec(TF_VEC_RESID, Wres.p, nullptr, 3, xs, nullptr);
    solve_once(Wres.p, Wdel.p);
    const double* ys[2] = {x1, Wdel.p};
    vec(TF_VEC_ADD, x1, nullptr, 2, ys, nullptr);
}

double tf_solver::backward_error(const double* rhs1, const double* x1) {
    ++n_checks;
    tfb::memset0(red.p, sizeof(double), stream);
    TfBerrArgs a;
    std::memset(&a, 0, sizeof(a));
    a.L = L1; a.Jv = Jv.p; a.x = x1; a.rhs = rhs1; a.c = factor_c; a.red = red.p;
    a.parsca = parsca.p; a.dx = dx.p; a.one_node = -1;
    unsigned gx = sweep_gx(), gy = cdiv(L1.M, spec.seg);
    launch(TFK_BERR, gx, gy, spec.sweep_block, &a, sizeof(a));
    double h = 0;
    tfb::d2h(&h, red.p, sizeof(h), stream);
    return h;
}

bool tf_solver::sampled_monitor_due() const {
    return refine < 0 && !reused && !delegated && !tiny && have_factor && !(refine == -1 && check_now);
}

TfBerrArgs tf_solver::probe_args(const double* rhs1, const double* x1, const double* xbase) {
    TfBerrArgs a;
    std::memset(&a, 0, sizeof(a));
    a.L = L1; a.Jv = Jv.p; a.x = x1; a.rhs = rhs1; a.c = factor_c; a.red = red.p + 4;
    a.parsca = parsca.p; a.dx = dx.p; a.xbase = xbase;
    a.one_node = (int)((mon_phase++ * 13u) % 4096u);
    monitored = true;
    return a;
}

void tf_solver::monitor_sampled(const double* rhs1, const double* x1, const double* xbase) {
    TfBerrArgs a = probe_args(rhs1, x1, xbase);
    launch(TFK_BERR, sweep_gx(), 1, spec.sweep_block, &a, sizeof(a));
}

void tf_solver::solve(const double* rhs1, double* x1) {
    if (!have_factor) throw std::runtime_error("tf_solve: matrix not factorised");
    if (delegated) { delegate_solve(rhs1, x1); return; }
    solve_once(rhs1, x1);
    polish(rhs1, x1);
}

void tf_solver::transfer_to(tf_solver* dst, const double* src_planes, double* dst_planes, int ncomp) {
    ensure_staging((size_t)ncomp * nsys * N);
    perm(1 , src_planes, staging.p, ncomp);
    dst->perm(0 , staging.p, dst_planes, ncomp);
}

void tf_solver::delegate_factor(double c) {
    tf_solver* fb = ensure_fallback();
    fb_touched = true;
    fb->mode = mode;
    copy(fb->parsca.p, parsca.p, parsca.n * sizeof(double));
    copy(fb->dx.p, dx.p, (size_t)nsys * sizeof(double));
    ++fb->par_ver;
    if (spec.parvec_mask) transfer_to(fb, parvec.p, fb->parvec.p, spec.npar);
    if (spec.nnz > 0) transfer_to(fb, Jv.p, fb->Jv.p, spec.nnz);
    fb->have_jac = true;
    fb->have_factor = false;
    fb->factor(c);
    fb_c = c; fb_ver = par_ver; fb_valid = true;
    delegated = true;
    fact_needs_refine = true;
}

void tf_solver::delegate_solve(const double* rhs1, double* x1) {
    if (!(fb_valid && fb_c == factor_c && fb_ver == par_ver)) delegate_factor(factor_c);
    tf_solver* fb = fallback;
    fb_touched = true;
    fb->mode = mode;
    transfer_to(fb, rhs1, fb->Wrhs.p, spec.nvar);
    fb->solve(fb->Wrhs.p, fb->Wstage.p);
    fb->transfer_to(this, fb->Wstage.p, x1, spec.nvar);
    last_omega = fb->last_omega;
    if (fb->unstable) { fb->unstable = false; unstable = true; }
}

void tf_solver::polish(const double* rhs1, double* x1) {
    if (refine > 0) {
        for (int it = 0; it < refine; ++it) refine_sweep(rhs1, x1);
    } else if (refine == -1) {
        if (!fact_checked) {
            last_omega = backward_error(rhs1, x1);
            fact_checked = true;
            sweeps_needed = 0;
            if (!(last_omega <= refine_trigger)) {
                double prev = last_omega;
                while (sweeps_needed < 6 && !(last_omega <= 1e-13)) {
                    refine_sweep(rhs1, x1);
                    ++sweeps_needed;
                    last_omega = backward_error(rhs1, x1);
                    if (!(last_omega < 0.5 * prev)) break;
                    prev = last_omega;
                }
            }
            fact_needs_refine = sweeps_needed > 0;
            if (berr_adaptive)
                berr_cur = (sweeps_needed == 0 && last_omega <= 0.01 * refine_trigger)
                    ? std::min(2 * berr_cur, std::max(berr_max, berr_every)) : berr_every;
            bool replan = false;
            if (sweeps_needed > 0 && !(last_omega <= 1e-12) && can_replan()) replan = true;
            else if (!(last_omega <= 1e-6)) unstable = true;
            if (Checked* e = checked_like(factor_c)) { e->c = factor_c; e->sweeps = sweeps_needed; e->at = n_factor; e->replan = replan; }
            else {
                if (checked.size() >= 4) checked.erase(checked.begin());
                checked.push_back(Checked{factor_c, sweeps_needed, n_factor, replan});
            }
            if (replan) {
                ++n_replans;
                tfb::memset0(status, sizeof(int), stream);
                delegate_factor(factor_c);
                delegate_solve(rhs1, x1);
            }
        } else {
            for (int it = 0; it < sweeps_needed; ++it) refine_sweep(rhs1, x1);
        }
    }
}

void tf_solver::check_status(const int* have_flag, const double* have_worst) {
    int flag = 0;
    if (have_flag) flag = *have_flag;
    else tfb::d2h(&flag, status, sizeof(int), stream);
    if (monitored) {
        double worst = 0.0;
        if (have_worst) worst = *have_worst;
        else tfb::d2h(&worst, red.p + 4, sizeof(double), stream);
        tfb::memset0(red.p + 4, sizeof(double), stream);
        monitored = false;
        if (worst > refine_trigger || worst != worst) {
            checked.clear();
            berr_cur = berr_every;
            monitor_omega = worst;
            if (!(worst <= 1e-6)) { last_omega = worst; unstable = true; }
        }
    }
    if (flag != 0) {
        tfb::memset0(status, sizeof(int), stream);
        throw std::runtime_error("banded solver: singular or non-finite pivot block");
    }
    if (fallback && fb_touched) { fb_touched = false; fallback->check_status(); }
    if (unstable) {
        unstable = false;
        throw std::runtime_error("banded solver: the block elimination lost accuracy (backward error " +
                                 std::to_string(last_omega) + " after refinement); no pivoting across blocks");
    }
}
```

Before: 2332 steps/s.

## Fuse adjacent CR backward levels and last two CR factor levels into single kernels

Adds a tfk_cr_bwd2 kernel that runs two consecutive cyclic-reduction backward levels in one launch, using shared memory to pass separator values so the coarser level's solution need not be stored to global memory. It also adds tfk_cr_factor_last2, where the last block per system to finish (detected with an atomic counter) factors the final CR level. The backward fusion is on by default, while the factor fusion is gated off by default behind an environment variable. The aim is to cut kernel launches and global round trips on the small coarse levels, at the cost of redundant coarse-level work per block and agent-scope loads and stores.

```diff
diff --git a/include/triflow_hip.h b/include/triflow_hip.h
--- a/include/triflow_hip.h
+++ b/include/triflow_hip.h
@@ -48,6 +48,7 @@
 void tf_solver_destroy(tf_solver* solver);
 int tf_solver_describe(tf_solver* solver, int32_t* nlevels, int32_t* chunks ,
                        int32_t max_levels, int64_t* device_bytes);
+int tf_solver_fused_forms(tf_solver* solver, int32_t* factor_last2, int32_t* bwd2);
 
 int tf_set_state(tf_solver*, int32_t slot, int32_t first_var, int32_t nvars, const double* host);
 int tf_get_state(tf_solver*, int32_t slot, int32_t first_var, int32_t nvars, double* host);
diff --git a/triflow_amd/_capi.py b/triflow_amd/_capi.py
--- a/triflow_amd/_capi.py
+++ b/triflow_amd/_capi.py
@@ -40,6 +40,7 @@
                                    C.POINTER(SolverOpts), C.POINTER(C.c_void_p)]),
     "tf_solver_destroy": (None, [C.c_void_p]),
     "tf_solver_describe": (C.c_int, [C.c_void_p, c_int32_p, c_int32_p, C.c_int32, c_int64_p]),
+    "tf_solver_fused_forms": (C.c_int, [C.c_void_p, c_int32_p, c_int32_p]),
     "tf_set_state": (C.c_int, [C.c_void_p, C.c_int32, C.c_int32, C.c_int32, c_double_p]),
     "tf_get_state": (C.c_int, [C.c_void_p, C.c_int32, C.c_int32, C.c_int32, c_double_p]),
     "tf_set_state_flat": (C.c_int, [C.c_void_p, C.c_int32, c_double_p]),
@@ -224,7 +225,10 @@
         nl, nbytes = C.c_int32(0), C.c_int64(0)
         chunks = (C.c_int32 * 32)()
         self.lib.call("tf_solver_describe", self.handle, C.byref(nl), chunks, 32, C.byref(nbytes))
-        return dict(levels=nl.value, chunks=list(chunks[:nl.value]), device_bytes=nbytes.value)
+        f2, b2 = C.c_int32(0), C.c_int32(0)
+        self.lib.call("tf_solver_fused_forms", self.handle, C.byref(f2), C.byref(b2))
+        fused = [name for name, on in (("tfk_cr_factor_last2", f2.value), ("tfk_cr_bwd2", b2.value)) if on]
+        return dict(levels=nl.value, chunks=list(chunks[:nl.value]), device_bytes=nbytes.value, fused=fused)
 
     def set_state(self, slot, arrays, first=0):
         a = _f64(arrays).reshape(-1, self.nsys, self.N)
diff --git a/triflow_amd/csrc/tf_args.h b/triflow_amd/csrc/tf_args.h
--- a/triflow_amd/csrc/tf_args.h
+++ b/triflow_amd/csrc/tf_args.h
@@ -199,6 +199,11 @@
     unsigned* counter;
 };
 
+struct TfFactor2Args {
+    TfLevelArgs lv[2];
+    unsigned* counter;
+};
+
 struct TfTopArgs {
     int nsys;
     const double* A;
@@ -299,11 +304,17 @@
     "tfk_l1_solve_cr", "tfk_l1_fwd2_backsub_cr", "tfk_sweep_f_stage_rhs_mon", \
     "tfk_probe_partial", "tfk_probe_final" }
 #define TF_KERNEL_NAMES_RECORD { "tfk_record" }
+enum TfKernelMore { TFK_CR_FACTOR_LAST2 = TFK_COUNT, TFK_CR_BWD2, TFK_TOTAL };
+#define TF_KERNEL_NAMES_MORE { "tfk_cr_factor_last2", "tfk_cr_bwd2" }
 static inline const char* tf_kernel_entry(int kernel) {
     static const char* const base[] = TF_KERNEL_NAMES;
     static const char* const rec[] = TF_KERNEL_NAMES_RECORD;
+    static const char* const more[] = TF_KERNEL_NAMES_MORE;
     static_assert(sizeof(base) / sizeof(base[0]) == TFK_RECORD, "TF_KERNEL_NAMES and TfKernel differ");
     static_assert(sizeof(rec) / sizeof(rec[0]) == TFK_COUNT - TFK_RECORD, "TF_KERNEL_NAMES_RECORD and TfKernel differ");
-    if (kernel < 0 || kernel >= TFK_COUNT) return "";
+    static_assert(sizeof(more) / sizeof(more[0]) == (int)TFK_TOTAL - (int)TFK_COUNT, "TF_KERNEL_NAMES_MORE and TfKernelMore differ");
+    static_assert((int)TFK_TOTAL <= 64, "the timing and alternate-build masks are 64 bits wide");
+    if (kernel < 0 || kernel >= (int)TFK_TOTAL) return "";
+    if (kernel >= (int)TFK_COUNT) return more[kernel - (int)TFK_COUNT];
     return kernel < TFK_RECORD ? base[kernel] : rec[kernel - TFK_RECORD];
 }
diff --git a/triflow_amd/csrc/tf_backend_hip.cpp b/triflow_amd/csrc/tf_backend_hip.cpp
--- a/triflow_amd/csrc/tf_backend_hip.cpp
+++ b/triflow_amd/csrc/tf_backend_hip.cpp
@@ -21,7 +21,7 @@
 }
 #define TF_HIP(call) check((call), #call)
 
-struct Module { hipModule_t mod; hipFunction_t fn[TFK_COUNT]; hipModule_t alt = nullptr; };
+struct Module { hipModule_t mod; hipFunction_t fn[TFK_TOTAL]; hipModule_t alt = nullptr; };
 struct Stream { hipStream_t s; };
 struct Event { hipEvent_t e; };
 
@@ -160,7 +160,7 @@
         delete m;
         check(err, "hipModuleLoadData (is the code object built for this GPU, gfx950?)");
     }
-    for (int k = 0; k < TFK_COUNT; ++k) {
+    for (int k = 0; k < TFK_TOTAL; ++k) {
         err = hipModuleGetFunction(&m->fn[k], m->mod, tf_kernel_entry(k));
         if (err != hipSuccess) {
             (void)hipModuleUnload(m->mod);
@@ -178,7 +178,7 @@
             if (fread(&img[0], 1, n, f) == (size_t)n) {
                 hipModule_t am;
                 if (hipModuleLoadData(&am, img.data()) == hipSuccess)
-                    for (int k = 0; k < TFK_COUNT; ++k)
+                    for (int k = 0; k < TFK_TOTAL; ++k)
                         if ((mask >> k) & 1ul) (void)hipModuleGetFunction(&m->fn[k], am, tf_kernel_entry(k));
             }
         }
@@ -190,7 +190,7 @@
     if (!m || !mask) return;
     if (m->alt) throw std::runtime_error("module_add_alternate: one alternate build per model");
     check(hipModuleLoadData(&m->alt, image), "hipModuleLoadData (alternate build)");
-    for (int k = 0; k < TFK_COUNT; ++k)
+    for (int k = 0; k < TFK_TOTAL; ++k)
         if ((mask >> k) & 1ull) {
             if (hipModuleGetFunction(&m->fn[k], m->alt, tf_kernel_entry(k)) != hipSuccess)
                 throw std::runtime_error(std::string("kernel missing from the alternate code object: ") + tf_kernel_entry(k));
diff --git a/triflow_amd/csrc/tf_coop_hip.h b/triflow_amd/csrc/tf_coop_hip.h
--- a/triflow_amd/csrc/tf_coop_hip.h
+++ b/triflow_amd/csrc/tf_coop_hip.h
@@ -648,7 +648,7 @@
     if (g < BB && grp == 1 && io.has_xprev) return io.xn_prev[g];
     return 0.0;
 }
-template <int BB, bool USE_EF = false, bool PREX = false>
+template <int BB, bool USE_EF = false, bool PREX = false, bool STORE_X = true>
 __device__ __forceinline__ void tfk_cr_bwd_run(const TfLevelArgs& a, const TfCrChunk<BB>& ch, int tid,
                                                TfCrSolveLds<BB>& sh, const TfCrIo<BB>& io,
                                                const TfCrBwdRows<BB>& rows, const double* ef = nullptr, double xsep = 0.0) {
@@ -662,7 +662,7 @@
     if (row_on && grp == 0) {
         const double xs = PREX ? xsep : io.xn_own[g];
         sX[pe][g] = xs;
-        x0[pe * BB] = xs;
+        if (STORE_X) x0[pe * BB] = xs;
     }
     if (row_on && grp == 1) sX[0][g] = PREX ? xsep : (io.has_xprev ? io.xn_prev[g] : 0.0);
     tf_wave_sync();
@@ -690,7 +690,7 @@
                     }
                 }
                 sX[k][g] = xk;
-                x0[k * BB] = xk;
+                if (STORE_X) x0[k * BB] = xk;
             }
             tf_wave_sync();
         }
@@ -711,6 +711,30 @@
     TfCrBwdRows<BB> rows;
     tfk_cr_bwd_load<BB>(a, ch, (int)threadIdx.x, io, rows, true);
     tfk_cr_bwd_run<BB>(a, ch, (int)threadIdx.x, sh, io, rows);
+}
+
+template <int BB>
+__device__ __forceinline__ void tfk_cr_bwd2_coop(const TfTailArgs& t) {
+    constexpr int G = TfCr<BB>::G;
+    __shared__ TfCrSolveLds<BB> sh;
+    const TfLevelArgs& la = t.lv[0];
+    const TfLevelArgs& lb = t.lv[1];
+    const int tid = (int)threadIdx.x, grp = tid / G, g = tid % G;
+    const TfCrChunk<BB> ch(la.L, (int)blockIdx.x);
+    int q, i;
+    tf_locate(lb.L, ch.p, q, i);
+    const TfCrChunk<BB> chb(lb.L, ch.e * lb.L.P + q);
+    const TfCrIo<BB> io(la, ch), iob(lb, chb);
+    TfCrBwdRows<BB> rows, rowsb;
+    tfk_cr_bwd_load<BB>(lb, chb, tid, iob, rowsb, true);
+    const double xb = tfk_cr_bwd_sep<BB>(tid, iob);
+    tfk_cr_bwd_load<BB>(la, ch, tid, io, rows, true);
+    if (i == 0) tfk_cr_bwd_run<BB, false, true, true>(lb, chb, tid, sh, iob, rowsb, nullptr, xb);
+    else tfk_cr_bwd_run<BB, false, true, false>(lb, chb, tid, sh, iob, rowsb, nullptr, xb);
+    double xsep = 0.0;
+    if (g < BB && grp == 0) xsep = sh.sY[i + 1][g];
+    if (g < BB && grp == 1 && io.has_xprev) xsep = sh.sY[i][g];
+    tfk_cr_bwd_run<BB, false, true>(la, ch, tid, sh, io, rows, nullptr, xsep);
 }
 
 #define TF_CR_TAIL_WAVES 8
diff --git a/triflow_amd/csrc/tf_cr3_hip.h b/triflow_amd/csrc/tf_cr3_hip.h
--- a/triflow_amd/csrc/tf_cr3_hip.h
+++ b/triflow_amd/csrc/tf_cr3_hip.h
@@ -37,8 +37,8 @@
     if constexpr (K + 1 < BB) tf_gj3_step<BB, K + 1>(val, c, grow);
 }
 
-template <int BB>
-__device__ __forceinline__ void tfk_cr_factor_v4(const TfLevelArgs& a) {
+template <int BB, bool XWG = false>
+__device__ __forceinline__ void tfk_cr_factor_v4(const TfLevelArgs& a, int chunk) {
     typedef TfCr3<BB> C;
     constexpr int NPOS = C::NPOS, B2 = BB * BB, REC = 4 * B2, NT_MIN = 256;
     constexpr int RS = C::RS, PS = C::PS, NC = C::NC;
@@ -47,7 +47,7 @@
     constexpr int NQ = (2 * B2 + 63) / 64;
     const int NT = blockDim.x, nw = NT >> 6;
     const TfLayout& L = a.L;
-    const TfCrChunk<BB> ch(L, (int)blockIdx.x);
+    const TfCrChunk<BB> ch(L, chunk);
     const int tid = threadIdx.x, w = __builtin_amdgcn_readfirstlane(tid >> 6), lane = tid & 63;
     constexpr bool DUP = C::DUP;
     const int half = DUP ? lane >> 5 : 0, c = DUP ? lane & 31 : lane;
@@ -57,6 +57,8 @@
     __shared__ double sRow[NPOS * PS];
     __shared__ unsigned sPerm[NPOS + 1];
     auto row = [&](int pos, int r) { return sRow + pos * PS + r * RS; };
+    auto ldx = [](const double* p) { if constexpr (XWG) return TF_LD_AGENT(p); else return *p; };
+    auto stx = [](double* p, double v) { if constexpr (XWG) TF_ST_AGENT(p, v); else *p = v; };
     unsigned* const perm = a.perm + ch.nbase + ch.start;
     if (tid < len) sPerm[tid + 1] = perm[tid];
     unsigned* const perm_top = a.perm + (int64_t)L.nsys * L.N + ch.e;
@@ -98,14 +100,14 @@
         for (int it = 0; it < NIT; ++it) {
             const int i = it * NT + tid;
             const int nd = i / (3 * B2), rem = i - nd * 3 * B2, blk = rem / B2, rc = rem - blk * B2;
-            v[it] = i < n3 ? src[nd * REC + blk * B2 + rc] : 0.0;
-            v2[it] = (i < n3 && blk == 1) ? src[nd * REC + 3 * B2 + rc] : 0.0;
+            v[it] = i < n3 ? ldx(src + nd * REC + blk * B2 + rc) : 0.0;
+            v2[it] = (i < n3 && blk == 1) ? ldx(src + nd * REC + 3 * B2 + rc) : 0.0;
         }
         const double* prev = a.Ablk + (ch.nbase + ch.gprev) * REC + 2 * B2;
         double p0 = 0.0, y0 = 0.0;
-        if (tid < B2 && ch.has_prev) p0 = prev[tid];
+        if (tid < B2 && ch.has_prev) p0 = ldx(prev + tid);
         const double* ys = a.rhs + (ch.nbase + ch.start) * 2 * BB;
-        if (with_rhs && tid < len * BB) y0 = ys[(tid / BB) * 2 * BB + tid % BB] + ys[(tid / BB) * 2 * BB + BB + tid % BB];
+        if (with_rhs && tid < len * BB) y0 = ldx(ys + (tid / BB) * 2 * BB + tid % BB) + ldx(ys + (tid / BB) * 2 * BB + BB + tid % BB);
         for (int i = tid; i < (len + 1) * BB * (RS - 3 * BB); i += NT) {
             const int pr = i / (RS - 3 * BB), o = i - pr * (RS - 3 * BB);
             sRow[(pr / BB) * PS + (pr % BB) * RS + 3 * BB + o] = 0.0;
@@ -255,9 +257,9 @@
         double* rec = a.Anext + ((int64_t)ch.e * a.Lnext.N + nn) * REC;
         double* rr = a.rhsnext + ((int64_t)ch.e * a.Lnext.N + nn) * 2 * BB;
         const double* rs = row(side == 0 ? pe : 0, r);
-        if (o < BB) rec[(side == 0 ? 0 : 2) * B2 + r * BB + o] = rs[(side == 0 ? oL : oU) + o];
-        else if (o < 2 * BB) rec[(side == 0 ? 1 : 3) * B2 + r * BB + o - BB] = rs[oDL + o - BB] + rs[oDR + o - BB];
-        else if (with_rhs) rr[(side == 0 ? 0 : BB) + r] = rs[oYL] + rs[oYR];
+        if (o < BB) stx(rec + (side == 0 ? 0 : 2) * B2 + r * BB + o, rs[(side == 0 ? oL : oU) + o]);
+        else if (o < 2 * BB) stx(rec + (side == 0 ? 1 : 3) * B2 + r * BB + o - BB, rs[oDL + o - BB] + rs[oDR + o - BB]);
+        else if (with_rhs) stx(rr + (side == 0 ? 0 : BB) + r, rs[oYL] + rs[oYR]);
     }
     TF_STAMP(a, 20);
     if (a.fold_top) {
diff --git a/triflow_amd/csrc/tf_entry_hip.h b/triflow_amd/csrc/tf_entry_hip.h
--- a/triflow_amd/csrc/tf_entry_hip.h
+++ b/triflow_amd/csrc/tf_entry_hip.h
@@ -368,7 +368,7 @@
 __global__ void __attribute__((amdgpu_waves_per_eu(TF_CR_FACTOR_WAVES))) __launch_bounds__(TF_CR_FACTOR_BLOCK)
 tfk_cr_factor(TfLevelArgs a) {
     if constexpr (TF_B2 <= 2) tfk_crs_factor<TF_B2, 256>(a, (int)blockIdx.x, (int)threadIdx.x);
-    else if constexpr (TF_B2 <= 8) tfk_cr_factor_v4<TF_B2>(a);
+    else if constexpr (TF_B2 <= 8) tfk_cr_factor_v4<TF_B2>(a, (int)blockIdx.x);
 }
 __global__ void __launch_bounds__(TF_CR_BLOCK) tfk_cr_fwd(TfLevelArgs a) {
     if constexpr (TF_B2 <= 2) tfk_crs_fwd<TF_B2, 256>(a, (int)blockIdx.x, (int)threadIdx.x);
@@ -377,6 +377,27 @@
 __global__ void __launch_bounds__(TF_CR_BLOCK) tfk_cr_bwd(TfLevelArgs a) {
     if constexpr (TF_B2 <= 2) tfk_crs_bwd<TF_B2, 256>(a, (int)blockIdx.x, (int)threadIdx.x);
     else if constexpr (TF_B2 <= 8) tfk_cr_bwd_coop<TF_B2>(a);
+}
+__global__ void __launch_bounds__(64) tfk_cr_bwd2(TfTailArgs t) {
+    if constexpr (TF_B2 >= 3 && TF_B2 <= 6) tfk_cr_bwd2_coop<TF_B2>(t);
+}
+__global__ void __attribute__((amdgpu_waves_per_eu(2))) __launch_bounds__(TF_CR_FACTOR_BLOCK)
+tfk_cr_factor_last2(TfFactor2Args t) {
+    if constexpr (TF_B2 >= 3 && TF_B2 <= 6) {
+        __shared__ int last;
+        const int e = (int)blockIdx.x / t.lv[0].L.P;
+        tfk_cr_factor_v4<TF_B2, true>(t.lv[0], (int)blockIdx.x);
+        asm volatile("s_waitcnt vmcnt(0)" ::: "memory");
+        __syncthreads();
+        if (threadIdx.x == 0) {
+            const unsigned seen = __hip_atomic_fetch_add(t.counter + e, 1u, __ATOMIC_RELAXED, __HIP_MEMORY_SCOPE_AGENT);
+            const int is_last = seen == (unsigned)t.lv[0].L.P - 1u;
+            if (is_last) __hip_atomic_store(t.counter + e, 0u, __ATOMIC_RELAXED, __HIP_MEMORY_SCOPE_AGENT);
+            last = is_last;
+        }
+        __syncthreads();
+        if (last) tfk_cr_factor_v4<TF_B2, true>(t.lv[1], e);
+    }
 }
 __device__ __forceinline__ void tf_own4(const TfLayout& L2, int blk, int& e, int& q0, int& nq, int& c0, int& cnt) {
     const int qps = (L2.P + 3) / 4;
diff --git a/triflow_amd/csrc/tf_rt_diag.cpp b/triflow_amd/csrc/tf_rt_diag.cpp
--- a/triflow_amd/csrc/tf_rt_diag.cpp
+++ b/triflow_amd/csrc/tf_rt_diag.cpp
@@ -41,7 +41,7 @@
 int tf_solver_kernel_block(tf_solver* s, int32_t kernel, int32_t* block) {
     TF_API_BEGIN
     require(s && block, "null argument");
-    require(kernel >= 0 && kernel < TFK_COUNT, "no such kernel");
+    require(kernel >= 0 && kernel < TFK_TOTAL, "no such kernel");
     *block = (int32_t)tfb::kernel_block(s->model->module, kernel);
     TF_API_END
 }
@@ -65,13 +65,13 @@
     TF_API_BEGIN
     require(s, "null solver");
     s->collect_timing();
-    for (int k = 0; k < TFK_COUNT; ++k) { s->time_ms[k] = 0; s->time_n[k] = 0; }
+    for (int k = 0; k < TFK_TOTAL; ++k) { s->time_ms[k] = 0; s->time_n[k] = 0; }
     TF_API_END
 }
 int tf_timing_get(tf_solver* s, int32_t kernel, double* total_ms, int64_t* launches) {
     TF_API_BEGIN
     require(s, "null solver");
-    require(kernel >= 0 && kernel < TFK_COUNT, "tf_timing_get: kernel index");
+    require(kernel >= 0 && kernel < TFK_TOTAL, "tf_timing_get: kernel index");
     s->collect_timing();
     if (total_ms) *total_ms = s->time_ms[kernel];
     if (launches) *launches = s->time_n[kernel];
diff --git a/triflow_amd/csrc/tf_rt_plan.cpp b/triflow_amd/csrc/tf_rt_plan.cpp
--- a/triflow_amd/csrc/tf_rt_plan.cpp
+++ b/triflow_amd/csrc/tf_rt_plan.cpp
@@ -19,7 +19,7 @@
     TF_API_END
 }
 
-int tf_kernel_count(void) { return TFK_COUNT; }
+int tf_kernel_count(void) { return TFK_TOTAL; }
 const char* tf_kernel_name(int32_t kernel) {
     return tf_kernel_entry(kernel);
 }
@@ -72,6 +72,8 @@
     if (const char* v = getenv("TRIFLOW_FUSE_STAGE")) s->fuse_stage = atoi(v) != 0;
     if (const char* v = getenv("TRIFLOW_S_FUSE")) s->s_fuse = atoi(v) != 0;
     if (const char* v = getenv("TRIFLOW_L1CR_FUSE")) s->l1cr_fuse = atoi(v) != 0;
+    if (const char* v = getenv("TRIFLOW_CR_FACTOR_FUSE")) s->cr_factor_fuse = atoi(v) != 0;
+    if (const char* v = getenv("TRIFLOW_CR_BWD_FUSE")) s->cr_bwd_fuse = atoi(v) != 0;
     if (const char* v = getenv("TRIFLOW_L1_FUSE_BACKSUB")) s->l1_fuse_backsub = atoi(v) != 0;
     if (const char* v = getenv("TRIFLOW_L1_FUSE_ASM")) s->l1_fuse_asm = atoi(v) != 0;
     if (const char* v = getenv("TRIFLOW_FUSE_UPDATE")) s->upd_fuse = atoi(v) != 0;
@@ -140,7 +142,7 @@
     for (int i = 0; i < TF_MAX_TERMS; ++i) s->K[i].alloc(i < 6 ? (size_t)sp.nvar * plane : 1, tot);
     s->red.alloc(8, tot);
     s->status = (int*)tfb::dev_alloc(sizeof(int));
-    if (b2 <= 2) s->sfuse_counter = (unsigned*)tfb::dev_alloc((size_t)nsys * sizeof(unsigned));
+    if (b2 <= 6) s->sfuse_counter = (unsigned*)tfb::dev_alloc((size_t)nsys * sizeof(unsigned));
     for (size_t l = 0; l < s->levels.size(); ++l) s->levels[l]->alloc(l, nsys, s->l1_respike, tot);
     s->top.alloc_top(b2, nsys, tot);
     s->topAinv.alloc((size_t)b2 * b2 * nsys, tot);
@@ -191,4 +193,15 @@
     if (device_bytes) *device_bytes = s->bytes;
     TF_API_END
 }
-}
+
+int tf_solver_fused_forms(tf_solver* s, int32_t* factor_last2, int32_t* bwd2) {
+    TF_API_BEGIN
+    require(s, "null solver");
+    if (factor_last2) *factor_last2 = s->factor2_ok() ? 1 : 0;
+    if (bwd2) {
+        const size_t n = s->levels.size();
+        *bwd2 = n >= 3 && s->fold_top() && s->bwd2_ok(n - 2, s->l2_in_l1_ok(1)) ? 1 : 0;
+    }
+    TF_API_END
+}
+}
diff --git a/triflow_amd/csrc/tf_solver.h b/triflow_amd/csrc/tf_solver.h
--- a/triflow_amd/csrc/tf_solver.h
+++ b/triflow_amd/csrc/tf_solver.h
@@ -264,8 +264,8 @@
     struct Stamp { int kernel; tfb::Event *a, *b; };
     std::vector<Stamp> stamps;
     std::vector<tfb::Event*> event_pool;
-    double time_ms[TFK_COUNT] = {0};
-    int64_t time_n[TFK_COUNT] = {0};
+    double time_ms[TFK_TOTAL] = {0};
+    int64_t time_n[TFK_TOTAL] = {0};
 
     ~tf_solver() {
         for (auto& st : stamps) { tfb::event_destroy(st.a); tfb::event_destroy(st.b); }
@@ -396,6 +396,11 @@
     TfScalarArgs scalar_args(const double* rhs1, double* x1);
     bool cr_tail = true;
     bool tail_ok() const;
+    bool cr_factor_fuse = false;
+    bool cr_bwd_fuse = true;
+    bool factor2_ok() const;
+    bool l2_in_l1_ok(int skip);
+    bool bwd2_ok(size_t l, bool l2_in_l1) const;
     void solve_once(const double* rhs1, double* x1);
     void refine_sweep(const double* rhs1, double* x1);
     double backward_error(const double* rhs1, const double* x1);
diff --git a/triflow_amd/csrc/tf_solver_linear.cpp b/triflow_amd/csrc/tf_solver_linear.cpp
--- a/triflow_amd/csrc/tf_solver_linear.cpp
+++ b/triflow_amd/csrc/tf_solver_linear.cpp
@@ -63,6 +63,16 @@
         if (l == 0) launch(fused ? TFK_L1_FACTOR_RHS : TFK_L1_FACTOR, gx, 2, l1_factor_block(), &a, sizeof(a));
         else if (levels[l]->cr) {
             a.cr_rhs = fused ? 1 : 0;
+            if (l + 2 == levels.size() && factor2_ok()) {
+                TfFactor2Args t;
+                t.lv[0] = a;
+                t.lv[1] = level_args(l + 1, rhs1, x1);
+                if (!fused) t.lv[1].rhs = nullptr;
+                t.lv[1].cr_rhs = a.cr_rhs;
+                t.counter = sfuse_counter;
+                launch(TFK_CR_FACTOR_LAST2, (unsigned)a.L.Ptot, 1, cr_factor_block(a.L.Ptot), &t, sizeof(t));
+                break;
+            }
             launch(TFK_CR_FACTOR, (unsigned)a.L.Ptot, 1, cr_factor_block(a.L.Ptot), &a, sizeof(a));
             continue;
         } else {
@@ -117,12 +127,7 @@
         launch(TFK_S_BWD, (unsigned)t.lv[1].L.Ptot, 1, 512, &t, sizeof(t));
         return;
     }
-    bool l2_in_l1 = false;
-    if (l1cr_ok() && levels.size() - (size_t)skip >= 2) {
-        TfLevelArgs a0 = level_args(0, rhs1, x1);
-        const unsigned lds0 = l1_twist_lds(a0);
-        l2_in_l1 = lds0 > 0 && lds0 <= 64u * 1024u;
-    }
+    const bool l2_in_l1 = l2_in_l1_ok(skip);
     for (size_t l = levels.size() - (size_t)skip; l-- > 0;) {
         if (l == 1 && l2_in_l1) continue;
         TfLevelArgs a = level_args(l, rhs1, x1);
@@ -149,6 +154,13 @@
             if (l1_respike) launch(TFK_L1_FWD2, cdiv(a.L.Ptot, 64), gy, 64, &a, sizeof(a));
             launch(l1_respike ? TFK_L1_BACKSUB_U : TFK_L1_BACKSUB, cdiv(a.L.Ptot, 64), gy, 64, &a, sizeof(a));
         }
+        else if (bwd2_ok(l, l2_in_l1)) {
+            TfTailArgs t;
+            t.lv[0] = level_args(l - 1, rhs1, x1);
+            t.lv[1] = a;
+            launch(TFK_CR_BWD2, (unsigned)t.lv[0].L.Ptot, 1, cr_block(), &t, sizeof(t));
+            --l;
+        }
         else if (levels[l]->cr) launch(TFK_CR_BWD, (unsigned)a.L.Ptot, 1, cr_block(), &a, sizeof(a));
         else launch(TFK_BT_BACKSUB, cdiv((int64_t)a.L.Ptot * tfb::coop_group(levels[l]->B), 64), 1, 64, &a, sizeof(a));
     }
@@ -176,6 +188,25 @@
     const size_t n = levels.size();
     return cr_tail && tfb::is_device_build() && n >= 3 && top.B >= 3 && top.B <= 6 && levels[n - 1]->cr && levels[n - 2]->cr &&
            levels[n - 1]->L.P == 1 && levels[n - 2]->L.P <= 8;
+}
+
+bool tf_solver::l2_in_l1_ok(int skip) {
+    if (!(l1cr_ok() && levels.size() - (size_t)skip >= 2)) return false;
+    TfLevelArgs a0 = level_args(0, nullptr, nullptr);
+    const unsigned lds0 = l1_twist_lds(a0);
+    return lds0 > 0 && lds0 <= 64u * 1024u;
+}
+
+bool tf_solver::factor2_ok() const {
+    const size_t n = levels.size();
+    return cr_factor_fuse && tfb::is_device_build() && !tiny && sfuse_counter && n >= 3 && top.B >= 3 && top.B <= 6 &&
+           levels[n - 1]->cr && levels[n - 2]->cr && levels[n - 1]->L.P == 1 && fold_top() &&
+           cr_factor_block(levels[n - 2]->L.Ptot) == cr_factor_block(levels[n - 1]->L.Ptot);
+}
+
+bool tf_solver::bwd2_ok(size_t l, bool) const {
+    return cr_bwd_fuse && tfb::is_device_build() && !tiny && top.B >= 3 && top.B <= 6 && l >= 3 && l < levels.size() &&
+           levels[l]->cr && levels[l - 1]->cr;
 }
 
 void tf_solver::solve_once(const double* rhs1, double* x1) {
```

Result: no change. 2325 steps/s (median of 2 runs) (-0.3%).
